# OpenMendel/MendelIHT.jl

Measured on NVIDIA B200. Metric: iht_iterations_per_sec, higher is better.
Workload: dtype f64 (sweep: f32 LUT partials per slab of 640 samples (512 without the ternary copy), f64 across slabs; top-k candidates re-scored in f64)

## Files before the change

### include/ihtb200.h

```cpp
#ifndef IHTB200_H
#define IHTB200_H

#include <stdint.h>

#ifdef __cplusplus
extern "C" {
#endif

#define IHTB_OK          0
#define IHTB_EINVAL     -1
#define IHTB_EDIM       -2
#define IHTB_EDOMAIN    -3
#define IHTB_ENUMERIC   -4
#define IHTB_ECUDA      -5
#define IHTB_ENOMEM     -6
#define IHTB_EUNSUPPORTED -7

enum { IHTB_NORMAL = 0, IHTB_BERNOULLI = 1, IHTB_POISSON = 2, IHTB_NEGBIN = 3 };
enum { IHTB_LINK_IDENTITY = 0, IHTB_LINK_LOGIT = 1, IHTB_LINK_LOG = 2, IHTB_LINK_PROBIT = 3,
       IHTB_LINK_CLOGLOG = 4, IHTB_LINK_CAUCHIT = 5, IHTB_LINK_SQRT = 6, IHTB_LINK_INVERSE = 7,
       IHTB_LINK_INVSQ = 8 };
enum { IHTB_SWEEP_FAST = 0, IHTB_SWEEP_EXACT = 1, IHTB_SWEEP_PAIR = 2 };

typedef struct ihtb_geno ihtb_geno;
typedef struct ihtb_fit ihtb_fit;
typedef struct ihtb_mvfit ihtb_mvfit;
typedef struct ihtb_comm ihtb_comm;

typedef struct ihtb_cfg {
    int32_t dist;
    int32_t link;
    int64_t k;
    double  nb_r;
    double  tol;
    int32_t max_iter;
    int32_t min_iter;
    int32_t max_step;
    int32_t sweep_mode;
    int32_t est_r;
    int32_t debias;
} ihtb_cfg;

typedef struct ihtb_result {
    double  time;
    double  logl;
    int64_t iter;
    double  sigma_g;
    int64_t n_sweeps;
    int64_t n_backtracks;
    double  sweep_seconds;
    int64_t n_launches;
    int64_t n_steps;
} ihtb_result;

typedef struct ihtb_iter_trace {
    double  logl;
    double  tol;
    double  eta;
    int32_t backtracks;
    int32_t n_candidates;
} ihtb_iter_trace;

int32_t ihtb_version(void);
int32_t ihtb_last_error(char* buf, int64_t cap);
int32_t ihtb_device_count(int32_t* count);
int32_t ihtb_set_device(int32_t device);
int32_t ihtb_launch_count(int64_t* count);

int32_t ihtb_geno_create(const uint8_t* bed_cols, int64_t n, int64_t p, int64_t col_stride_bytes,
                         int32_t center, int32_t scale, int32_t impute, ihtb_geno** out);
int32_t ihtb_geno_create_empty(int64_t n, int64_t p, int32_t center, int32_t scale, int32_t impute, ihtb_geno** out);
int32_t ihtb_geno_load_columns(ihtb_geno* g, const uint8_t* bed_cols, int64_t col_stride_bytes, int64_t j_first,
                               int64_t ncols);
int32_t ihtb_geno_finalize(ihtb_geno* g);
int32_t ihtb_geno_create_synthetic(int64_t n, int64_t p_local, int64_t j0, uint64_t seed, double missing_rate,
                                   ihtb_geno** out);
int32_t ihtb_synth_host(int64_t n, int64_t ncols, int64_t j0, uint64_t seed, double missing_rate, uint8_t* out);
int32_t ihtb_geno_dims(const ihtb_geno* g, int64_t* n, int64_t* p);
int32_t ihtb_geno_stats(const ihtb_geno* g, double* mu, double* sigma_inv, int64_t* n_missing);
int32_t ihtb_geno_counts(const ihtb_geno* g, int64_t* counts_4_by_p);
int32_t ihtb_geno_maf(const ihtb_geno* g, double* maf);
int32_t ihtb_geno_decode(const ihtb_geno* g, int64_t i0, int64_t i1, int64_t j0, int64_t j1, double* out_colmajor);
int32_t ihtb_geno_packed(const ihtb_geno* g, int64_t j0, int64_t j1, uint8_t* out);
int32_t ihtb_xt_v(const ihtb_geno* g, const double* V, int64_t m, double* out, int32_t sweep_mode);
int32_t ihtb_x_support(const ihtb_geno* g, const int64_t* idx, int64_t k, const double* coef, int64_t m, double* out);
int32_t ihtb_sweep_bench(const ihtb_geno* g, int32_t sweep_mode, int32_t warmup, int32_t reps, double* ms_kernel,
                         double* ms_total);
int32_t ihtb_geno_sweep_stream_bytes(const ihtb_geno* g, int64_t* bytes, int32_t* ternary);
int32_t ihtb_geno_ternary_tiles(const ihtb_geno* g, uint8_t* out, int64_t out_bytes);
int32_t ihtb_gather_bench(const ihtb_geno* g, int64_t ncols, int32_t reps, double* ms_per_call, double* max_rel_diff);
int32_t ihtb_geno_destroy(ihtb_geno* g);

enum { IHTB_DENSE_F64 = 0, IHTB_DENSE_F32 = 1 };
int32_t ihtb_geno_create_dense(const void* x, int32_t dtype, int64_t n, int64_t p, int64_t ld, int32_t standardize,
                               ihtb_geno** out);
int32_t ihtb_geno_create_dense_empty(int64_t n, int64_t p, int32_t dtype, int32_t standardize, ihtb_geno** out);
int32_t ihtb_geno_load_dense_columns(ihtb_geno* g, const void* x, int64_t ld, int64_t j_first, int64_t ncols);

int32_t ihtb_fit_create(const ihtb_geno* g, const double* y, const double* z, int64_t q, const uint8_t* zkeep,
                        const ihtb_cfg* cfg, ihtb_fit** out);
int32_t ihtb_fit_create_sharded(const ihtb_geno* g, ihtb_comm* comm, int64_t p_global, const double* y,
                                const double* z, int64_t q, const uint8_t* zkeep, const ihtb_cfg* cfg, ihtb_fit** out);
int32_t ihtb_fit_set_weights(ihtb_fit* f, const double* weight);
int32_t ihtb_fit_set_groups(ihtb_fit* f, const int32_t* group, int32_t J, const int64_t* ks, int64_t n_groups);
int32_t ihtb_fit_set_k(ihtb_fit* f, int64_t k);
int32_t ihtb_fit_init(ihtb_fit* f, const uint8_t* train_mask);
int32_t ihtb_fit_init_beta(ihtb_fit* f, const uint8_t* train_mask);
int32_t ihtb_fit_run(ihtb_fit* f, ihtb_result* result, ihtb_iter_trace* trace, int64_t trace_cap);
int32_t ihtb_fit_get(const ihtb_fit* f, double* beta, double* c, double* mu, double* xb);
int32_t ihtb_fit_get_sparse(const ihtb_fit* f, int64_t* idx, double* val, int64_t cap, int64_t* nnz);
int32_t ihtb_fit_predict(ihtb_fit* f, const uint8_t* test_mask, double* deviance);
int32_t ihtb_fit_timer(ihtb_fit* f, int32_t which, double* ms);
int32_t ihtb_fit_phase_times(const ihtb_fit* f, double* out4);
int32_t ihtb_fit_destroy(ihtb_fit* f);

int32_t ihtb_mvfit_create(const ihtb_geno* g, const double* Y, int64_t r, const double* z, int64_t q,
                          const ihtb_cfg* cfg, ihtb_mvfit** out);
int32_t ihtb_mvfit_create_sharded(const ihtb_geno* g, ihtb_comm* comm, int64_t p_global, const double* Y, int64_t r,
                                  const double* z, int64_t q, const ihtb_cfg* cfg, ihtb_mvfit** out);
int32_t ihtb_mvfit_set_k(ihtb_mvfit* f, int64_t k);
int32_t ihtb_mvfit_init(ihtb_mvfit* f, const uint8_t* train_mask);
int32_t ihtb_mvfit_init_beta(ihtb_mvfit* f, const uint8_t* train_mask);
int32_t ihtb_mvfit_run(ihtb_mvfit* f, ihtb_result* result, ihtb_iter_trace* trace, int64_t trace_cap);
int32_t ihtb_mvfit_get(const ihtb_mvfit* f, double* beta, double* c, double* Sigma, double* sigma_g);
int32_t ihtb_mvfit_predict(ihtb_mvfit* f, const uint8_t* test_mask, double* mse);
int32_t ihtb_mvfit_destroy(ihtb_mvfit* f);

int32_t ihtb_cv_run(const ihtb_geno* g, const double* y, const double* z, int64_t q, const uint8_t* zkeep,
                    const ihtb_cfg* cfg, const int32_t* folds, int32_t nfolds, const int64_t* path, int64_t npath,
                    const double* weight, double* mses, int64_t* iters);

enum { IHTB_MULTI_SHARD = 0, IHTB_MULTI_REPLICATE = 1 };
typedef struct ihtb_mgeno ihtb_mgeno;
typedef struct ihtb_mfit ihtb_mfit;
int32_t ihtb_mgeno_create(const uint8_t* bed_cols, int64_t n, int64_t p, int64_t col_stride_bytes, int32_t center,
                          int32_t scale, int32_t impute, int32_t ngpu, const int32_t* devices, int32_t mode,
                          ihtb_mgeno** out);
int32_t ihtb_mgeno_create_synthetic(int64_t n, int64_t p, uint64_t seed, double missing_rate, int32_t ngpu,
                                    const int32_t* devices, int32_t mode, ihtb_mgeno** out);
int32_t ihtb_mgeno_info(const ihtb_mgeno* g, int32_t* ngpu, int32_t* mode, int64_t* n, int64_t* p);
int32_t ihtb_mgeno_part(const ihtb_mgeno* g, int32_t i, ihtb_geno** part, int32_t* device, int64_t* j0);
int32_t ihtb_mgeno_destroy(ihtb_mgeno* g);
int32_t ihtb_mfit_create(const ihtb_mgeno* g, const double* y, const double* z, int64_t q, const uint8_t* zkeep,
                         const ihtb_cfg* cfg, ihtb_mfit** out);
int32_t ihtb_mfit_set_weights(ihtb_mfit* f, const double* weight);
int32_t ihtb_mfit_set_groups(ihtb_mfit* f, const int32_t* group, int32_t J, const int64_t* ks, int64_t n_groups);
int32_t ihtb_mfit_set_k(ihtb_mfit* f, int64_t k);
int32_t ihtb_mfit_init(ihtb_mfit* f, const uint8_t* train_mask, int32_t init_beta);
int32_t ihtb_mfit_run(ihtb_mfit* f, ihtb_result* result, ihtb_iter_trace* trace, int64_t trace_cap);
int32_t ihtb_mfit_get(const ihtb_mfit* f, double* beta, double* c, double* mu, double* xb);
int32_t ihtb_mfit_get_sparse(const ihtb_mfit* f, int64_t* idx, double* val, int64_t cap, int64_t* nnz);
int32_t ihtb_mfit_predict(ihtb_mfit* f, const uint8_t* test_mask, double* deviance);
int32_t ihtb_mfit_timer(ihtb_mfit* f, int32_t which, double* ms);
int32_t ihtb_mfit_destroy(ihtb_mfit* f);
typedef struct ihtb_mmvfit ihtb_mmvfit;
int32_t ihtb_mmvfit_create(const ihtb_mgeno* g, const double* Y, int64_t r, const double* z, int64_t q,
                           const ihtb_cfg* cfg, ihtb_mmvfit** out);
int32_t ihtb_mmvfit_set_k(ihtb_mmvfit* f, int64_t k);
int32_t ihtb_mmvfit_init(ihtb_mmvfit* f, const uint8_t* train_mask, int32_t init_beta);
int32_t ihtb_mmvfit_run(ihtb_mmvfit* f, ihtb_result* result, ihtb_iter_trace* trace, int64_t trace_cap);
int32_t ihtb_mmvfit_get(const ihtb_mmvfit* f, double* beta, double* c, double* Sigma, double* sigma_g);
int32_t ihtb_mmvfit_predict(ihtb_mmvfit* f, const uint8_t* test_mask, double* mse);
int32_t ihtb_mmvfit_destroy(ihtb_mmvfit* f);
int32_t ihtb_mcv_run(const ihtb_mgeno* g, const double* y, const double* z, int64_t q, const uint8_t* zkeep,
                     const ihtb_cfg* cfg, const int32_t* folds, int32_t nfolds, const int64_t* path, int64_t npath,
                     const double* weight, double* mses, int64_t* iters, double* busy_seconds);

int32_t ihtb_comm_unique_id(const char* nccl_lib_path, uint8_t* out128);
int32_t ihtb_comm_create(const char* nccl_lib_path, const uint8_t* id128, int32_t rank, int32_t nranks, ihtb_comm** out);
int32_t ihtb_comm_destroy(ihtb_comm* c);
int32_t ihtb_comm_stats(const ihtb_comm* c, int64_t* peer_memory_collectives, int64_t* nccl_calls);
int32_t ihtb_comm_allreduce_bench(ihtb_comm* c, int64_t n, int32_t reps, int32_t use_p2p, double* us_per_op);
int32_t ihtb_geno_set_offset(ihtb_geno* g, int64_t j0);

#ifdef __cplusplus
}
#endif
#endif
```

### mendeliht.jl_b200/__init__.py

```python
from . import _lib, synth
from ._lib import (SWEEP_EXACT, SWEEP_FAST, SWEEP_PAIR, CudaError, DimensionMismatch, IHTBError, NumericError, device_count,
                   launch_count, load)
from .api import (BERNOULLI, NEGBIN, NORMAL, POISSON, B200DenseLinAlg, B200MultiSnpLinAlg, B200SnpLinAlg, IHTResult, IHTVariable, mIHTResult, mIHTVariable,
                  is_multivariate, allocate_fold_and_k,
                  canonicallink, cross_validate, cv_iht, cv_run, fit_iht, iht, maf_weights, meanloss, parse_covariates)

__all__ = ["B200SnpLinAlg", "B200DenseLinAlg", "B200MultiSnpLinAlg", "IHTResult", "IHTVariable", "fit_iht", "cv_iht", "cv_run", "allocate_fold_and_k", "meanloss",
           "canonicallink", "maf_weights", "iht", "cross_validate", "parse_covariates", "NORMAL", "BERNOULLI", "POISSON", "NEGBIN", "SWEEP_FAST", "SWEEP_EXACT", "SWEEP_PAIR", "load",
           "device_count", "launch_count", "IHTBError", "DimensionMismatch", "NumericError", "CudaError", "synth"]
```

### mendeliht.jl_b200/_lib.py

```python
from __future__ import annotations

import ctypes as C
import os

import numpy as np

HERE = os.path.dirname(os.path.abspath(__file__))
LIB_PATH = os.path.join(HERE, "libihtb200.so")

IHTB_OK, IHTB_EINVAL, IHTB_EDIM, IHTB_EDOMAIN, IHTB_ENUMERIC, IHTB_ECUDA, IHTB_ENOMEM, IHTB_EUNSUPPORTED = (
    0, -1, -2, -3, -4, -5, -6, -7)
SWEEP_FAST, SWEEP_EXACT, SWEEP_PAIR = 0, 1, 2
DENSE_F64, DENSE_F32 = 0, 1


class IHTBError(RuntimeError):
    def __init__(self, code, msg):
        super().__init__(msg)
        self.code = code


class DimensionMismatch(IHTBError, ValueError):
    pass


class NumericError(IHTBError, FloatingPointError):
    pass


class CudaError(IHTBError):
    pass


_EXC = {IHTB_EINVAL: IHTBError, IHTB_EDIM: DimensionMismatch, IHTB_EDOMAIN: IHTBError, IHTB_ENUMERIC: NumericError,
        IHTB_ECUDA: CudaError, IHTB_ENOMEM: IHTBError, IHTB_EUNSUPPORTED: IHTBError}


class Cfg(C.Structure):
    _fields_ = [("dist", C.c_int32), ("link", C.c_int32), ("k", C.c_int64), ("nb_r", C.c_double),
                ("tol", C.c_double), ("max_iter", C.c_int32), ("min_iter", C.c_int32), ("max_step", C.c_int32),
                ("sweep_mode", C.c_int32), ("est_r", C.c_int32), ("debias", C.c_int32)]


class Result(C.Structure):
    _fields_ = [("time", C.c_double), ("logl", C.c_double), ("iter", C.c_int64), ("sigma_g", C.c_double),
                ("n_sweeps", C.c_int64), ("n_backtracks", C.c_int64), ("sweep_seconds", C.c_double),
                ("n_launches", C.c_int64), ("n_steps", C.c_int64)]


class IterTrace(C.Structure):
    _fields_ = [("logl", C.c_double), ("tol", C.c_double), ("eta", C.c_double), ("backtracks", C.c_int32),
                ("n_candidates", C.c_int32)]


_p = C.c_void_p
_pp = C.POINTER(C.c_void_p)
_f64 = C.POINTER(C.c_double)
_i64 = C.POINTER(C.c_int64)
_u8 = C.POINTER(C.c_uint8)

SIGNATURES = {
    "ihtb_version": [],
    "ihtb_last_error": [C.c_char_p, C.c_int64],
    "ihtb_device_count": [C.POINTER(C.c_int32)],
    "ihtb_set_device": [C.c_int32],
    "ihtb_launch_count": [_i64],
    "ihtb_geno_create": [_u8, C.c_int64, C.c_int64, C.c_int64, C.c_int32, C.c_int32, C.c_int32, _pp],
    "ihtb_geno_create_empty": [C.c_int64, C.c_int64, C.c_int32, C.c_int32, C.c_int32, _pp],
    "ihtb_geno_load_columns": [_p, _u8, C.c_int64, C.c_int64, C.c_int64],
    "ihtb_geno_finalize": [_p],
    "ihtb_geno_counts": [_p, _i64],
    "ihtb_geno_maf": [_p, _f64],
    "ihtb_geno_create_synthetic": [C.c_int64, C.c_int64, C.c_int64, C.c_uint64, C.c_double, _pp],
    "ihtb_synth_host": [C.c_int64, C.c_int64, C.c_int64, C.c_uint64, C.c_double, _u8],
    "ihtb_geno_dims": [_p, _i64, _i64],
    "ihtb_geno_stats": [_p, _f64, _f64, _i64],
    "ihtb_geno_decode": [_p, C.c_int64, C.c_int64, C.c_int64, C.c_int64, _f64],
    "ihtb_geno_packed": [_p, C.c_int64, C.c_int64, _u8],
    "ihtb_xt_v": [_p, _f64, C.c_int64, _f64, C.c_int32],
    "ihtb_x_support": [_p, _i64, C.c_int64, _f64, C.c_int64, _f64],
    "ihtb_sweep_bench": [_p, C.c_int32, C.c_int32, C.c_int32, _f64, _f64],
    "ihtb_geno_sweep_stream_bytes": [_p, C.POINTER(C.c_int64), C.POINTER(C.c_int32)],
    "ihtb_gather_bench": [_p, C.c_int64, C.c_int32, _f64, _f64],
    "ihtb_geno_ternary_tiles": [_p, _u8, C.c_int64],
    "ihtb_geno_destroy": [_p],
    "ihtb_geno_create_dense": [_p, C.c_int32, C.c_int64, C.c_int64, C.c_int64, C.c_int32, _pp],
    "ihtb_geno_create_dense_empty": [C.c_int64, C.c_int64, C.c_int32, C.c_int32, _pp],
    "ihtb_geno_load_dense_columns": [_p, _p, C.c_int64, C.c_int64, C.c_int64],
    "ihtb_fit_create": [_p, _f64, _f64, C.c_int64, _u8, C.POINTER(Cfg), _pp],
    "ihtb_fit_create_sharded": [_p, _p, C.c_int64, _f64, _f64, C.c_int64, _u8, C.POINTER(Cfg), _pp],
    "ihtb_fit_set_weights": [_p, _f64],
    "ihtb_fit_set_groups": [_p, C.POINTER(C.c_int32), C.c_int32, _i64, C.c_int64],
    "ihtb_fit_set_k": [_p, C.c_int64],
    "ihtb_fit_init": [_p, _u8],
    "ihtb_fit_init_beta": [_p, _u8],
    "ihtb_fit_run": [_p, C.POINTER(Result), C.POINTER(IterTrace), C.c_int64],
    "ihtb_fit_get": [_p, _f64, _f64, _f64, _f64],
    "ihtb_fit_get_sparse": [_p, C.POINTER(C.c_int64), _f64, C.c_int64, C.POINTER(C.c_int64)],
    "ihtb_fit_predict": [_p, _u8, _f64],
    "ihtb_fit_timer": [_p, C.c_int32, _f64],
    "ihtb_fit_phase_times": [_p, _f64],
    "ihtb_fit_destroy": [_p],
    "ihtb_cv_run": [_p, _f64, _f64, C.c_int64, _u8, C.POINTER(Cfg), C.POINTER(C.c_int32), C.c_int32, _i64, C.c_int64,
                    _f64, _f64, _i64],
    "ihtb_mvfit_create": [_p, _f64, C.c_int64, _f64, C.c_int64, C.POINTER(Cfg), _pp],
    "ihtb_mvfit_create_sharded": [_p, _p, C.c_int64, _f64, C.c_int64, _f64, C.c_int64, C.POINTER(Cfg), _pp],
    "ihtb_mvfit_set_k": [_p, C.c_int64],
    "ihtb_mvfit_init": [_p, _u8],
    "ihtb_mvfit_init_beta": [_p, _u8],
    "ihtb_mvfit_run": [_p, C.POINTER(Result), C.POINTER(IterTrace), C.c_int64],
    "ihtb_mvfit_get": [_p, _f64, _f64, _f64, _f64],
    "ihtb_mvfit_predict": [_p, _u8, _f64],
    "ihtb_mvfit_destroy": [_p],
    "ihtb_comm_unique_id": [C.c_char_p, _u8],
    "ihtb_comm_create": [C.c_char_p, _u8, C.c_int32, C.c_int32, _pp],
    "ihtb_comm_destroy": [_p],
    "ihtb_comm_stats": [_p, _i64, _i64],
    "ihtb_comm_allreduce_bench": [_p, C.c_int64, C.c_int32, C.c_int32, _f64],
    "ihtb_geno_set_offset": [_p, C.c_int64],
    "ihtb_mgeno_create": [_u8, C.c_int64, C.c_int64, C.c_int64, C.c_int32, C.c_int32, C.c_int32, C.c_int32,
                          C.POINTER(C.c_int32), C.c_int32, _pp],
    "ihtb_mgeno_create_synthetic": [C.c_int64, C.c_int64, C.c_uint64, C.c_double, C.c_int32, C.POINTER(C.c_int32),
                                    C.c_int32, _pp],
    "ihtb_mgeno_info": [_p, C.POINTER(C.c_int32), C.POINTER(C.c_int32), _i64, _i64],
    "ihtb_mgeno_part": [_p, C.c_int32, _pp, C.POINTER(C.c_int32), _i64],
    "ihtb_mgeno_destroy": [_p],
    "ihtb_mfit_create": [_p, _f64, _f64, C.c_int64, _u8, C.POINTER(Cfg), _pp],
    "ihtb_mfit_set_weights": [_p, _f64],
    "ihtb_mfit_set_groups": [_p, C.POINTER(C.c_int32), C.c_int32, _i64, C.c_int64],
    "ihtb_mfit_set_k": [_p, C.c_int64],
    "ihtb_mfit_init": [_p, _u8, C.c_int32],
    "ihtb_mfit_run": [_p, C.POINTER(Result), C.POINTER(IterTrace), C.c_int64],
    "ihtb_mfit_get": [_p, _f64, _f64, _f64, _f64],
    "ihtb_mfit_get_sparse": [_p, C.POINTER(C.c_int64), _f64, C.c_int64, C.POINTER(C.c_int64)],
    "ihtb_mfit_predict": [_p, _u8, _f64],
    "ihtb_mfit_timer": [_p, C.c_int32, _f64],
    "ihtb_mfit_destroy": [_p],
    "ihtb_mmvfit_create": [_p, _f64, C.c_int64, _f64, C.c_int64, C.POINTER(Cfg), _pp],
    "ihtb_mmvfit_set_k": [_p, C.c_int64],
    "ihtb_mmvfit_init": [_p, _u8, C.c_int32],
    "ihtb_mmvfit_run": [_p, C.POINTER(Result), C.POINTER(IterTrace), C.c_int64],
    "ihtb_mmvfit_get": [_p, _f64, _f64, _f64, _f64],
    "ihtb_mmvfit_predict": [_p, _u8, _f64],
    "ihtb_mmvfit_destroy": [_p],
    "ihtb_mcv_run": [_p, _f64, _f64, C.c_int64, _u8, C.POINTER(Cfg), C.POINTER(C.c_int32), C.c_int32, _i64, C.c_int64,
                     _f64, _f64, _i64, _f64],
}

_lib = None


def load() -> C.CDLL:
    global _lib
    if _lib is None:
        if not os.path.exists(LIB_PATH):
            raise ImportError(
                f"{LIB_PATH} is missing: the CUDA extension has not been built. "
                "Run `python -c 'import __graft_entry__ as g; g.build()'` (needs nvcc). "
                "mendeliht.jl_b200 has no CPU fallback.")
        lib = C.CDLL(LIB_PATH)
        for name, args in SIGNATURES.items():
            fn = getattr(lib, name)
            fn.argtypes = args
            fn.restype = C.c_int32
        _lib = lib
    return _lib


def last_error() -> str:
    buf = C.create_string_buffer(1024)
    load().ihtb_last_error(buf, 1024)
    return buf.value.decode("utf-8", "replace")


def check(status: int) -> None:
    if status != IHTB_OK:
        raise _EXC.get(status, IHTBError)(status, last_error())


def f64(a) -> np.ndarray:
    return np.ascontiguousarray(a, dtype=np.float64)


def ptr(a: np.ndarray, ctype):
    return a.ctypes.data_as(C.POINTER(ctype)) if a is not None else None


def device_count() -> int:
    n = C.c_int32(0)
    load().ihtb_device_count(C.byref(n))
    return int(n.value)


def launch_count() -> int:
    n = C.c_int64(0)
    check(load().ihtb_launch_count(C.byref(n)))
    return int(n.value)
```

### mendeliht.jl_b200/csrc/common.cuh

```cuda
#pragma once
#include <cuda_runtime.h>
#include <stdint.h>
#include <stdio.h>
#include <string>
#include <vector>
#include <stdexcept>
#include "../../include/ihtb200.h"

namespace ihtb {

struct Error : std::runtime_error {
    int code;
    Error(int c, const std::string& m) : std::runtime_error(m), code(c) {}
};
void set_last_error(const std::string& m);
const std::string& last_error();
struct LaunchCounter {
    int64_t v = 0;
    LaunchCounter& operator++(int) { __atomic_fetch_add(&v, 1, __ATOMIC_RELAXED); return *this; }
    operator int64_t() const { return __atomic_load_n(&v, __ATOMIC_RELAXED); }
};
LaunchCounter& launch_counter();
bool debug_sync();

#define IHTB_CUDA(call)                                                                      \
    do {                                                                                     \
        cudaError_t e__ = (call);                                                            \
        if (e__ != cudaSuccess)                                                              \
            throw ::ihtb::Error(IHTB_ECUDA, std::string(#call) + ": " + cudaGetErrorString(e__)); \
    } while (0)

#define IHTB_CHECK(cond, code, msg)                                  \
    do {                                                             \
        if (!(cond)) throw ::ihtb::Error((code), (msg));             \
    } while (0)

#define IHTB_LAUNCH(kernel, grid, block, smem, stream, ...)          \
    do {                                                             \
        kernel<<<(grid), (block), (smem), (stream)>>>(__VA_ARGS__);  \
        ::ihtb::launch_counter()++;                                  \
        IHTB_CUDA(cudaGetLastError());                               \
        if (::ihtb::debug_sync()) {                                  \
            cudaError_t e2__ = cudaStreamSynchronize(stream);        \
            if (e2__ != cudaSuccess)                                 \
                throw ::ihtb::Error(IHTB_ECUDA, std::string("kernel " #kernel " failed: ") + cudaGetErrorString(e2__)); \
        }                                                            \
    } while (0)

template <typename F>
static inline int32_t guard(F&& f) {
    try {
        f();
        return IHTB_OK;
    } catch (const Error& e) {
        set_last_error(e.what());
        return e.code;
    } catch (const std::bad_alloc&) {
        set_last_error("out of host memory");
        return IHTB_ENOMEM;
    } catch (const std::exception& e) {
        set_last_error(e.what());
        return IHTB_EINVAL;
    }
}

template <typename T>
struct DBuf {
    T* p = nullptr;
    size_t n = 0;
    DBuf() = default;
    explicit DBuf(size_t count) { alloc(count); }
    DBuf(const DBuf&) = delete;
    DBuf& operator=(const DBuf&) = delete;
    ~DBuf() { release(); }
    void alloc(size_t count) {
        release();
        n = count;
        if (count) {
            cudaError_t e = cudaMalloc((void**)&p, count * sizeof(T));
            if (e != cudaSuccess) {
                p = nullptr; n = 0;
                throw Error(IHTB_ENOMEM, std::string("cudaMalloc of ") + std::to_string(count * sizeof(T)) +
                                             " bytes failed: " + cudaGetErrorString(e));
            }
        }
    }
    void release() {
        if (p) cudaFree(p);
        p = nullptr; n = 0;
    }
    void zero(cudaStream_t s) { if (n) IHTB_CUDA(cudaMemsetAsync(p, 0, n * sizeof(T), s)); }
};

template <typename T>
struct HBuf {
    T* p = nullptr;
    size_t n = 0;
    HBuf() = default;
    HBuf(const HBuf&) = delete;
    HBuf& operator=(const HBuf&) = delete;
    ~HBuf() { if (p) cudaFreeHost(p); }
    void alloc(size_t count) {
        if (p) cudaFreeHost(p);
        p = nullptr; n = count;
        if (count) IHTB_CUDA(cudaMallocHost((void**)&p, count * sizeof(T)));
    }
};

static inline int64_t ceil_div(int64_t a, int64_t b) { return (a + b - 1) / b; }

bool smem_attr_needed(const void* kernel, int device);
template <typename K>
static inline void ensure_dynamic_smem(K kernel, int bytes) {
    int dev = 0;
    IHTB_CUDA(cudaGetDevice(&dev));
    if (!smem_attr_needed(reinterpret_cast<const void*>(kernel), dev)) return;
    IHTB_CUDA(cudaFuncSetAttribute(kernel, cudaFuncAttributeMaxDynamicSharedMemorySize, bytes));
}

struct TopkFuse;
ihtb_geno* dense_new_handle(int64_t n, int64_t p, int dtype, int standardize);
void dense_upload(ihtb_geno* g, const void* x, int64_t ld_host, int64_t j_dst, int64_t ncols);
void dense_finalize(ihtb_geno* g);
int64_t dense_stream_bytes(const ihtb_geno* g);
void dense_decode_block(const ihtb_geno* g, int64_t i0, int64_t i1, int64_t j0, int64_t j1, double* d_out);
void dense_xt_v(const ihtb_geno* g, const double* dV, int64_t m, double* dOut, cudaStream_t s, DBuf<double>* part,
                const TopkFuse* tf);
void dense_sweep_kernel_only(const ihtb_geno* g, const double* dV, DBuf<double>* part, cudaStream_t s);
void dense_x_support(const ihtb_geno* g, const int64_t* d_idx, int64_t k, const double* d_coef, int64_t m,
                     double* d_out, cudaStream_t s);
void dense_xt_gather2(const ihtb_geno* g, const int64_t* d_cols_a, int64_t n_a, const int64_t* d_cols_b, int64_t n_b,
                      const double* d_v, int64_t m, double* d_out, cudaStream_t s);
void dense_init_beta_moments(const ihtb_geno* g, const double* d_w, const double* d_wy, double* d_sx, double* d_sxx,
                             double* d_sxy, cudaStream_t s);
void dense_decode_cols(const ihtb_geno* g, const int64_t* d_cols, int64_t k, double* d_out, cudaStream_t s);
const double* geno_bound_scale(const ihtb_geno* g);
double geno_bound_coef(const ihtb_geno* g, double plink_coef);

}

enum { GENO_PLINK = 0, GENO_DENSE = 1 };

struct ihtb_geno {
    int kind = 0;
    int device = 0;
    int64_t n = 0;
    int64_t p = 0;
    int64_t j0 = 0;
    int64_t nbytes = 0;
    int64_t stride = 0;
    int64_t cs_j = 0, cs_s = 0;
    int quad = 0;
    int64_t p4 = 0;
    int center = 1, scale = 1, impute = 1;
    int sm_count = 148;
    ihtb::DBuf<uint8_t> bed;
    ihtb::DBuf<uint8_t> tern;
    int64_t tern_slabs = 0;
    ihtb::DBuf<double> mu, sinv;
    ihtb::DBuf<double> sgn;
    ihtb::DBuf<int32_t> nmiss;
    ihtb::DBuf<int64_t> miss_ptr;
    ihtb::DBuf<int32_t> miss_idx;
    int64_t total_missing = 0;
    bool ready = false;
    int dtype = 0;
    int standardize = 0;
    int64_t ld = 0;
    ihtb::DBuf<uint8_t> dense;
    ihtb::DBuf<double> dscale;
    double dcoef = 0.0;
};
static inline bool geno_is_dense(const ihtb_geno* g) { return g->kind == GENO_DENSE; }

static inline void geno_require_ready(const ihtb_geno* g) {
    IHTB_CHECK(g && g->ready, IHTB_EINVAL, "genotype handle is not finalized (ihtb_geno_finalize)");
}

struct GenoView {
    const uint8_t* bed;
    int64_t cs_j, cs_s, nbytes, stride, n, p;
    int quad;
    const double* mu;
    const double* sinv;
    const int32_t* nmiss;
    int impute;
};
static inline GenoView geno_view(const ihtb_geno* g) {
    return GenoView{g->bed.p, g->cs_j, g->cs_s, g->nbytes, g->stride, g->n, g->p, g->quad, g->mu.p, g->sinv.p,
                    g->nmiss.p, g->impute};
}
__device__ __forceinline__ const uint8_t* gv_ptr(const GenoView& g, int64_t j, int64_t b) {
    if (g.quad)
        return g.bed + (b >> 7) * g.cs_s + (j >> 2) * 512 + ((b & 127) >> 2) * 16 + (j & 3) * 4 + (b & 3);
    return g.bed + j * g.cs_j + (b >> 7) * g.cs_s + (b & 127);
}

namespace ihtb {

__device__ __forceinline__ double warp_sum(double v) {
#pragma unroll
    for (int o = 16; o > 0; o >>= 1) v += __shfl_xor_sync(0xffffffffu, v, o);
    return v;
}
__device__ __forceinline__ float warp_sum(float v) {
#pragma unroll
    for (int o = 16; o > 0; o >>= 1) v += __shfl_xor_sync(0xffffffffu, v, o);
    return v;
}
__device__ __forceinline__ int warp_sum(int v) {
#pragma unroll
    for (int o = 16; o > 0; o >>= 1) v += __shfl_xor_sync(0xffffffffu, v, o);
    return v;
}

__device__ __forceinline__ double block_sum(double v, double* sh) {
    v = warp_sum(v);
    int lane = threadIdx.x & 31, w = threadIdx.x >> 5;
    __syncthreads();
    if (lane == 0) sh[w] = v;
    __syncthreads();
    int nw = (blockDim.x + 31) >> 5;
    v = (threadIdx.x < nw) ? sh[threadIdx.x] : 0.0;
    if (w == 0) v = warp_sum(v);
    return v;
}

void sweep_xt_v(const ihtb_geno* g, const double* dV, int64_t m, double* dOut, int mode, cudaStream_t s,
                double* sweep_seconds);
void x_support(const ihtb_geno* g, const int64_t* d_idx_local, int64_t k, const double* d_coef, int64_t m,
               double* d_out, cudaStream_t s);
void xt_gather(const ihtb_geno* g, const int64_t* d_cols_local, int64_t ncols, const double* d_v, int64_t m,
               const double* d_vsum , double* d_out , cudaStream_t s);
void xt_gather2(const ihtb_geno* g, const int64_t* d_cols_a, int64_t n_a, const int64_t* d_cols_b, int64_t n_b,
                const double* d_v, int64_t m, const double* d_vsum, double* d_out, cudaStream_t s, bool blocked = false);

struct TopkFuse;
void dense_xt_v(const ihtb_geno* g, const double* dV, int64_t m, double* dOut, cudaStream_t s, void* scratch_any,
                const TopkFuse* tf);
void dense_x_support(const ihtb_geno* g, const int64_t* d_idx, int64_t k, const double* d_coef, int64_t m,
                     double* d_out, cudaStream_t s);
void dense_xt_gather2(const ihtb_geno* g, const int64_t* d_cols_a, int64_t n_a, const int64_t* d_cols_b, int64_t n_b,
                      const double* d_v, int64_t m, double* d_out, cudaStream_t s);
void dense_init_beta_moments(const ihtb_geno* g, const double* d_w, const double* d_wy, double* d_sx, double* d_sxx,
                             double* d_sxy, cudaStream_t s, void* scratch_any);
void dense_decode_cols(const ihtb_geno* g, const int64_t* d_cols, int64_t k, double* d_out, cudaStream_t s);
const double* geno_bound_scale(const ihtb_geno* g);
double geno_bound_coef(const ihtb_geno* g, double plink_coef);

}
```

### mendeliht.jl_b200/csrc/fit.cu

```cuda
#include "glm.cuh"
#include "topk.cuh"
#include "comm.cuh"
#include "debias.cuh"
#include "groups.cuh"
#include "pairer.cuh"
#include <algorithm>
#include <chrono>
#include <cmath>
#include <memory>
#include <mutex>
#include <string.h>
#include <unordered_map>

namespace ihtb {
void sweep_xt_v_with_means(const ihtb_geno* g, const double* dV, const double* vbar_host, int64_t m, double* dOut,
                           int mode, cudaStream_t s, void* scratch_any, float* sweep_ms, double* d_l2 = nullptr,
                           const TopkFuse* tf = nullptr);
void* sweep_scratch_create();
void sweep_scratch_destroy(void* p);
void sweep_class_sums(const ihtb_geno* g, const double* d_v, double* d_w1, double* d_w2, double* d_wm, cudaStream_t s,
                      void* scratch_any);
}

using namespace ihtb;

static const double kFastBound = 1.0 / 262144.0;
static const double kExactBound = 1e-13;
static const double kPairBound = 3.1 / 2048.0;

struct ihtb_fit {
    const ihtb_geno* g = nullptr;
    int device = 0;
    int64_t n = 0, p = 0, q = 0;
    ihtb_comm* comm = nullptr;
    int64_t j0 = 0, p_global = 0;
    std::vector<int64_t> shard_j0;
    DBuf<int64_t> d_selall, d_pack, d_packall;
    HBuf<int64_t> h_selall, h_packall;
    int capx = 512;
    ihtb_cfg cfg{};
    cudaStream_t s = nullptr;
    std::vector<uint8_t> zkeep;
    int zkeepn = 0;
    int cap = 4096;

    DBuf<unsigned> d_done;
    DBuf<double> d_y, d_z, d_w, d_xb, d_zc, d_mu, d_r, d_xs, d_dfa, d_part, d_scal, d_small, d_coef, d_gout,
        d_vbar;
    DBuf<uint8_t> d_mask;
    DBuf<uint32_t> d_keyL, d_keyU;
    DBuf<int> d_hist;
    DBuf<int64_t> d_sel;
    DBuf<int64_t> d_idx, d_cols;
    HBuf<double> h_scal, h_gout;
    HBuf<int64_t> h_sel;
    void* sweep_scratch = nullptr;
    cudaEvent_t ev0 = nullptr, ev1 = nullptr, tm0 = nullptr, tm1 = nullptr;
    bool sweep_pending = false;
    struct FusedStep {
        std::vector<int64_t> uni_loc;
        size_t maxsupp = 0;
        int M = 0;
        int winner = -1;
    };
    FusedStep* fz = nullptr;
    DBuf<double> d_pick;
    HBuf<double> h_pick;
    SweepPairer* pairer = nullptr;
    int pair_slot = 0;
    double sweep_coef = kFastBound;
    GlmCtx glm{};
    TopkCtx tk{};

    std::vector<int64_t> idx, idx0, best_idx;
    std::vector<double> b, b0, best_b;
    std::vector<double> c, c0, best_c, df2, h_y, h_mu;
    std::vector<uint8_t> idc, idc0;
    std::unordered_map<int64_t, double> df_exact;
    std::vector<double> wt;
    DBuf<double> d_wt;
    double w_at(int64_t j) const { return wt.empty() ? 1.0 : wt[(size_t)j]; }
    void set_weights(const double* w) {
        if (!w) { wt.clear(); tk.wt = nullptr; return; }
        for (int64_t j = 0; j < p_global; ++j)
            IHTB_CHECK(w[j] > 0.0 && std::isfinite(w[j]), IHTB_EDOMAIN, "weights must be positive and finite");
        wt.assign(w, w + p_global);
        if (d_wt.n < (size_t)p) d_wt.alloc((size_t)p);
        IHTB_CUDA(cudaMemcpyAsync(d_wt.p, wt.data() + j0, (size_t)p * sizeof(double), cudaMemcpyHostToDevice, s));
        sync();
        tk.wt = d_wt.p;
    }
    std::vector<int64_t> cand_cache;
    bool df_sparse = false;
    std::vector<int64_t> dfs_idx;
    std::vector<double> dfs_val;
    double rbar = 0.0, bound = 0.0, sum_w = 0.0, sum_wy = 0.0, last_dev = 0.0, denom_next = 0.0;
    bool denom_ready = false;
    bool inited = false;

    int64_t n_sweeps = 0, n_backtracks = 0, n_cand_iter = 0, n_pair_overflow = 0;
    int last_count = 0;
    double sweep_ms_total = 0.0;
    double pve = 0.0;

    ~ihtb_fit() {
        if (sweep_scratch) sweep_scratch_destroy(sweep_scratch);
        if (ev0) cudaEventDestroy(ev0);
        if (ev1) cudaEventDestroy(ev1);
        if (tm0) cudaEventDestroy(tm0);
        if (tm1) cudaEventDestroy(tm1);
        if (s) cudaStreamDestroy(s);
    }

    void sync() { IHTB_CUDA(cudaStreamSynchronize(s)); }
    void readback_scal(int nv) {
        IHTB_CUDA(cudaMemcpyAsync(h_scal.p, d_scal.p, nv * sizeof(double), cudaMemcpyDeviceToHost, s));
        sync();
    }
    template <typename T>
    void upload(T* dst, const T* src, size_t count) {
        if (count) IHTB_CUDA(cudaMemcpyAsync(dst, src, count * sizeof(T), cudaMemcpyHostToDevice, s));
    }

    bool is_local(int64_t j) const { return j >= j0 && j < j0 + p; }
    int nranks() const { return comm ? comm->nranks : 1; }

    void support_matvec(const std::vector<int64_t>& cols, const std::vector<double>& coef, double* d_out) {
        std::vector<int64_t> ii; std::vector<double> vv;
        for (size_t t = 0; t < cols.size(); ++t)
            if (coef[t] != 0.0 && is_local(cols[t])) { ii.push_back(cols[t] - j0); vv.push_back(coef[t]); }
        if (!ii.empty()) {
            upload(d_idx.p, ii.data(), ii.size());
            upload(d_coef.p, vv.data(), vv.size());
        }
        support_matvec_dev(ii.empty() ? nullptr : d_idx.p, (int64_t)ii.size(), d_coef.p, d_out);
    }

    void support_matvec_dev(const int64_t* d_idx_loc, int64_t k_loc, const double* d_coef_loc, double* d_out) {
        support_matvec_dev_m(d_idx_loc, k_loc, d_coef_loc, 1, d_out);
    }
    void support_matvec_dev_m(const int64_t* d_idx_loc, int64_t k_loc, const double* d_coef_loc, int m, double* d_out) {
        const size_t cnt = (size_t)n * (size_t)m;
        if (!comm) {
            if (k_loc > 0) x_support(g, d_idx_loc, k_loc, d_coef_loc, m, d_out, s);
            else IHTB_CUDA(cudaMemsetAsync(d_out, 0, cnt * sizeof(double), s));
            return;
        }
        if (m == 1 && p2p_pushall_ok(comm, cnt)) {
            if (k_loc > 0) x_support_push(g, d_idx_loc, k_loc, d_coef_loc, comm, s);
            else p2p_push(comm, nullptr, cnt, s);
            p2p_reduce(comm, d_out, cnt, s);
            return;
        }
        if (p2p_mapped(comm) && cnt <= comm->red_cap) {
            double* part = p2p_partial_ptr(comm);
            if (k_loc > 0) x_support(g, d_idx_loc, k_loc, d_coef_loc, m, part, s);
            else IHTB_CUDA(cudaMemsetAsync(part, 0, cnt * sizeof(double), s));
            p2p_allreduce_2phase(comm, cnt, d_out, s);
            return;
        }
        if (k_loc > 0) x_support(g, d_idx_loc, k_loc, d_coef_loc, m, d_out, s);
        else IHTB_CUDA(cudaMemsetAsync(d_out, 0, cnt * sizeof(double), s));
        comm_allreduce_sum_f64(comm, d_out, cnt, s);
    }

    void update_xb() { support_matvec(idx, b, d_xb.p); }

    double glm_update(int add_zc) {
        upload(d_small.p, c.data(), (size_t)q);
        glm_mu(glm, d_small.p, add_zc, s);
        readback_scal(3);
        double dev = h_scal.p[0], lp = h_scal.p[1], sw = h_scal.p[2];
        last_dev = dev;
        if (cfg.dist == IHTB_NORMAL) {
            double phi = dev / (double)n;
            double sigma = std::sqrt(phi);
            return -0.5 * (dev / phi) - sw * (0.5 * std::log(2.0 * M_PI) + std::log(sigma));
        }
        return lp;
    }

    static double digamma(double x) {
        double r = 0.0;
        while (x < 6.0) { r -= 1.0 / x; x += 1.0; }
        double f = 1.0 / (x * x);
        return r + std::log(x) - 0.5 / x -
               f * (1.0 / 12 - f * (1.0 / 120 - f * (1.0 / 252 - f * (1.0 / 240 - f * (1.0 / 132)))));
    }
    static double trigamma(double x) {
        double r = 0.0;
        while (x < 6.0) { r += 1.0 / (x * x); x += 1.0; }
        double f = 1.0 / (x * x);
        return r + 1.0 / x + f / 2 + f / x * (1.0 / 6 - f * (1.0 / 30 - f * (1.0 / 42 - f * (1.0 / 30))));
    }
    void fetch_mu() {
        h_mu.resize((size_t)n);
        IHTB_CUDA(cudaMemcpyAsync(h_mu.data(), d_mu.p, n * sizeof(double), cudaMemcpyDeviceToHost, s));
        sync();
    }
    double nb_logl(double r) {
        glm.nb_r = r;
        return glm_update(1);
    }
    void mle_for_r() {
        fetch_mu();
        const std::vector<double>& y = h_y;
        double r = glm.nb_r;
        if (cfg.est_r == 1) {
            double num = 0.0, den = 0.0;
            for (int64_t i = 0; i < n; ++i) {
                for (int64_t j = 0; j <= (int64_t)y[i] - 1; ++j) num += r / (r + (double)j);
                den += std::log(r / (r + h_mu[i]));
            }
            glm.nb_r = -num / den;
            return;
        }
        auto d1 = [&](double rr) {
            double a = 0.0;
            for (int64_t i = 0; i < n; ++i)
                a += -(y[i] + rr) / (h_mu[i] + rr) - std::log(h_mu[i] + rr) + 1.0 + std::log(rr) + digamma(rr + y[i]) -
                     digamma(rr);
            return a;
        };
        auto d2 = [&](double rr) {
            double a = 0.0;
            for (int64_t i = 0; i < n; ++i)
                a += (y[i] + rr) / ((h_mu[i] + rr) * (h_mu[i] + rr)) - 2.0 / (h_mu[i] + rr) + 1.0 / rr +
                     trigamma(rr + y[i]) - trigamma(rr);
            return a;
        };
        double new_r = 1.0, stepsize = 1.0;
        for (int it = 0; it < 100; ++it) {
            double dx = d1(r), dx2 = d2(r);
            double increment = dx2 < 0 ? dx / dx2 : dx;
            new_r = r - stepsize * increment;
            double old_logl = nb_logl(r);
            for (int j = 0; j < 20; ++j) {
                if (new_r <= 0) {
                    stepsize /= 2; new_r = r - stepsize * increment;
                } else {
                    double new_logl = nb_logl(new_r);
                    if (old_logl >= new_logl) { stepsize /= 2; new_r = r - stepsize * increment; }
                    else break;
                }
            }
            if (std::fabs(r - new_r) <= 1e-6) { glm.nb_r = new_r; return; }
            r = new_r;
        }
        glm.nb_r = r;
    }
    double mu_r_logl() {
        double l = glm_update(1);
        if (cfg.est_r != 0) {
            mle_for_r();
            l = glm_update(1);
        }
        return l;
    }

    void exact_df(const std::vector<int64_t>& cols, bool exchange = true) {
        std::vector<int64_t> need;
        for (int64_t j : cols)
            if (!df_exact.count(j) && (exchange || is_local(j))) need.push_back(j);
        if (need.empty()) { if (!exchange) sync(); return; }
        IHTB_CHECK((int64_t)need.size() <= (int64_t)d_cols.n, IHTB_ENUMERIC, "too many columns to re-score");
        std::vector<int64_t> loc(need.size());
        for (size_t t = 0; t < need.size(); ++t) loc[t] = is_local(need[t]) ? need[t] - j0 : -1;
        upload(d_cols.p, loc.data(), loc.size());
        xt_gather2(g, d_cols.p, (int64_t)need.size(), nullptr, 0, d_r.p, 1, d_vbar.p, d_gout.p, s,
                   false);
        if (exchange) comm_allreduce_sum_f64(comm, d_gout.p, need.size(), s);
        IHTB_CUDA(cudaMemcpyAsync(h_gout.p, d_gout.p, need.size() * sizeof(double), cudaMemcpyDeviceToHost, s));
        sync();
        for (size_t t = 0; t < need.size(); ++t) df_exact[need[t]] = h_gout.p[t];
        n_cand_iter += (int64_t)need.size();
    }

    void score_and_sweep() {
        glm_score(glm, s, d_vbar.p);
        IHTB_CUDA(cudaMemcpyAsync(h_scal.p, d_scal.p, (2 + q) * sizeof(double), cudaMemcpyDeviceToHost, s));
        IHTB_CUDA(cudaEventRecord(ev0, s));
        sweep_coef = geno_bound_coef(g, cfg.sweep_mode == IHTB_SWEEP_FAST ? kFastBound : kExactBound);
        const double t_sw = now();
        if (pairer && cfg.sweep_mode == IHTB_SWEEP_FAST) {
            IHTB_CHECK(!grouped() && !comm, IHTB_EUNSUPPORTED, "paired sweeps serve plain single-device fits only");
            if (pairer->sweep(pair_slot, g, d_r.p, d_vbar.p, d_dfa.p, s, sweep_scratch)) {
                sweep_coef = kPairBound;
                IHTB_CUDA(cudaMemcpyAsync(h_scal.p + 3 + q, pairer->d_l2 + pair_slot, sizeof(double), cudaMemcpyDeviceToHost, s));
            }
        } else if (cfg.k > 0 && !(grouped() && !init_plain)) {
            const TopkFuse tf = topk_absdf_fuse_begin(tk, geno_bound_scale(g), d_scal.p, sweep_coef);
            sweep_xt_v_with_means(g, d_r.p, d_vbar.p, 1, d_dfa.p, cfg.sweep_mode, s, sweep_scratch, nullptr, nullptr, &tf);
        } else {
            sweep_xt_v_with_means(g, d_r.p, d_vbar.p, 1, d_dfa.p, cfg.sweep_mode, s, sweep_scratch, nullptr);
        }
        IHTB_CUDA(cudaEventRecord(ev1, s));
        ++n_sweeps;
        const double t_sel = now();
        dbg[0] += t_sel - t_sw;
        select_rescore(false);
        dbg[1] += now() - t_sel;
    }

    void select_rescore(bool rerun) {
        if (grouped() && !init_plain) {
            select_groups(rerun);
            if (!rerun) finish_sweep_scalars(sweep_coef);
            return;
        }
        df_exact.clear(); cand_cache.clear();
        df_sparse = false;
        const double coef = sweep_coef;
        std::vector<std::pair<int64_t, double>> cvals;
        const bool fused = fz != nullptr && !rerun;
        std::vector<int64_t> supp_loc;
        if (fused) supp_loc = fz->uni_loc;
        else
            for (int64_t j : idx)
                if (is_local(j)) supp_loc.push_back(j - j0);
        const int nsupp = (int)supp_loc.size();
        const int64_t* d_supp = fused ? d_idx.p : d_cols.p;
        int glaunch = 0;
        if (cfg.k > 0) {
            const int64_t ksel = cfg.k + (int64_t)(fused ? fz->maxsupp : idx.size());
            const bool paired = coef == kPairBound;
            if (tk.fused_hist) topk_candidates_absdf_finish(tk, ksel, s);
            else
                topk_candidates_absdf(tk, d_dfa.p, paired ? g->sgn.p : geno_bound_scale(g), rerun ? nullptr : d_scal.p, coef, ksel, s,
                                      bound, (paired && !rerun) ? pairer->d_l2 + pair_slot : nullptr);
            const int64_t want = sweep_coef == kPairBound ? std::max<int64_t>(ksel + 1024, last_count + last_count / 4 + 256)
                                                          : ksel + 64;
            glaunch = (int)std::min<int64_t>(comm ? capx / 2 : cap, want);
        }
        if (nsupp && !fused) upload(d_cols.p, supp_loc.data(), supp_loc.size());
        xt_gather2(g, tk.cand, glaunch, d_supp, nsupp, d_r.p, 1, d_vbar.p, d_gout.p, s);
        denom_ready = false;
        if (!rerun) {
            if (fused) {
                glm_winner_coef(d_pick.p, d_coefM.p, nsupp, d_gout.p + glaunch, d_coef.p, d_cM.p, q, d_small.p + q, s);
                support_matvec_dev(d_supp, nsupp, d_coef.p, d_xs.p);
                IHTB_CUDA(cudaMemcpyAsync(h_pick.p, d_pick.p, (size_t)(1 + fz->M) * sizeof(double), cudaMemcpyDeviceToHost, s));
                IHTB_CUDA(cudaMemcpyAsync(h_scalM.p, d_scalM.p, (size_t)(3 * fz->M) * sizeof(double), cudaMemcpyDeviceToHost, s));
            } else {
                support_matvec_dev(d_supp, nsupp, d_gout.p + glaunch, d_xs.p);
                std::vector<double> mask((size_t)q);
                for (int64_t l = 0; l < q; ++l) mask[l] = idc[l] ? 1.0 : 0.0;
                upload(d_small.p + q, mask.data(), (size_t)q);
            }
            glm_stepsize(glm, d_scal.p + 2, d_xs.p, s, d_small.p + q, d_scal.p + 2 + q);
            IHTB_CUDA(cudaMemcpyAsync(h_scal.p + 2 + q, d_scal.p + 2 + q, sizeof(double), cudaMemcpyDeviceToHost, s));
            denom_ready = true;
        }
        if (!comm) {
            IHTB_CUDA(cudaMemcpyAsync(h_sel.p, d_sel.p, (2 + glaunch) * sizeof(int64_t), cudaMemcpyDeviceToHost, s));
            IHTB_CUDA(cudaMemcpyAsync(h_gout.p, d_gout.p, (glaunch + nsupp) * sizeof(double), cudaMemcpyDeviceToHost, s));
            sync();
            const double t_host = now();
            struct Acc { double& a; double t0; ~Acc() { a += now() - t0; } } acc_host{dbg[2], t_host};
            if (fused) adopt_winner();
            const TopkState* st = reinterpret_cast<const TopkState*>(h_sel.p);
            const int count = cfg.k > 0 ? st->count : 0;
            dbg[3] += (double)std::min(count, glaunch);
            if (count > cap && coef == kPairBound && !rerun) {
                ++n_pair_overflow;
                sweep_coef = kFastBound;
                sweep_xt_v_with_means(g, d_r.p, d_vbar.p, 1, d_dfa.p, IHTB_SWEEP_FAST, s, sweep_scratch, nullptr);
                IHTB_CUDA(cudaEventRecord(ev1, s));
                select_rescore(false);
                return;
            }
            IHTB_CHECK(count <= cap, IHTB_ENUMERIC,
                       "degenerate projection: more than " + std::to_string(cap) +
                           " entries lie within the sweep error bound of the k-th largest |gradient|");
            last_count = count;
            cvals.reserve((size_t)count);
            for (int t = 0; t < std::min(count, glaunch); ++t) cvals.push_back({h_sel.p[2 + t], h_gout.p[t]});
            for (int t = 0; t < nsupp; ++t) df_exact[supp_loc[t] + j0] = h_gout.p[glaunch + t];
            if (count > glaunch) {
                IHTB_CUDA(cudaMemcpyAsync(h_sel.p, d_sel.p, (2 + count) * sizeof(int64_t), cudaMemcpyDeviceToHost, s));
                sync();
                std::vector<int64_t> rest(h_sel.p + 2 + glaunch, h_sel.p + 2 + count);
                exact_df(rest);
                for (int64_t j : rest) cvals.push_back({j, df_exact.at(j)});
            }
        } else {
            const int nr = nranks();
            const size_t blk = 2 + 2 * (size_t)capx;
            IHTB_CHECK(nsupp <= capx / 2, IHTB_ENUMERIC, "support too large for the sharded candidate exchange");
            pack_sweep_candidates(d_pack.p, reinterpret_cast<const TopkState*>(d_sel.p), tk.cand, glaunch, d_gout.p,
                                  d_supp, nsupp, d_gout.p + glaunch, j0, capx, s);
            comm_allgather_i64(comm, d_pack.p, d_packall.p, blk, s);
            IHTB_CUDA(cudaMemcpyAsync(h_packall.p, d_packall.p, nr * blk * sizeof(int64_t), cudaMemcpyDeviceToHost, s));
            sync();
            if (fused) adopt_winner();
            for (int r = 0; r < nr; ++r) {
                const int64_t* b_ = h_packall.p + (size_t)r * blk;
                IHTB_CHECK(b_[0] <= glaunch, IHTB_ENUMERIC,
                           "degenerate projection: too many local candidates within the sweep error bound");
                const int half = capx / 2;
                auto take = [&](int t, bool is_cand) {
                    const int64_t j = b_[2 + t];
                    if (j < 0) return;
                    double v;
                    memcpy(&v, &b_[2 + capx + t], sizeof(double));
                    if (is_cand) cvals.push_back({j, v});
                    else df_exact[j] = v;
                };
                for (int t = 0; t < (int)b_[0]; ++t) take(t, true);
                for (int t = 0; t < (int)b_[1]; ++t) take(half + t, false);
            }
        }
        std::sort(cvals.begin(), cvals.end());
        cvals.erase(std::unique(cvals.begin(), cvals.end(), [](const std::pair<int64_t, double>& x, const std::pair<int64_t, double>& y) {
                        return x.first == y.first; }), cvals.end());
        n_cand_iter += (int64_t)cvals.size();
        std::vector<char> keep(cvals.size(), 1);
        if ((int64_t)cvals.size() > cfg.k) {
            std::vector<std::pair<double, size_t>> outside;
            outside.reserve(cvals.size());
            for (size_t t = 0; t < cvals.size(); ++t)
                if (!std::binary_search(idx.begin(), idx.end(), cvals[t].first))
                    outside.push_back({std::fabs(cvals[t].second) * w_at(cvals[t].first), t});
            if ((int64_t)outside.size() > cfg.k) {
                std::nth_element(outside.begin(), outside.begin() + (cfg.k - 1), outside.end(),
                                 [](const std::pair<double, size_t>& x, const std::pair<double, size_t>& y) {
                                     return x.first > y.first;
                                 });
                const double thr = outside[(size_t)cfg.k - 1].first * (1.0 - 1e-12);
                std::fill(keep.begin(), keep.end(), 0);
                for (const auto& e : outside)
                    if (e.first >= thr) keep[e.second] = 1;
            }
        }
        for (size_t t = 0; t < cvals.size(); ++t)
            if (keep[t]) {
                cand_cache.push_back(cvals[t].first);
                df_exact[cvals[t].first] = cvals[t].second;
            }
        if (rerun) return;
        finish_sweep_scalars(coef);
    }

    void finish_sweep_scalars(double coef) {
        float ms = 0.f;
        IHTB_CUDA(cudaEventElapsedTime(&ms, ev0, ev1));
        sweep_ms_total += ms;
        double rsum = h_scal.p[0], rl1 = h_scal.p[1];
        for (int64_t l = 0; l < q; ++l) df2[l] = h_scal.p[2 + l];
        denom_next = h_scal.p[2 + q];
        rbar = rsum / (double)n;
        bound = coef == kPairBound ? coef * h_scal.p[3 + q]
                                   : coef * (rl1 + std::fabs(rsum));
    }

    double df_at(int64_t j) const {
        if (df_sparse) {
            auto it = std::lower_bound(dfs_idx.begin(), dfs_idx.end(), j);
            return (it != dfs_idx.end() && *it == j) ? dfs_val[it - dfs_idx.begin()] : 0.0;
        }
        return df_exact.at(j);
    }

    double stepsize() {
        std::vector<double> coef(idx.size());
        double numer = 0.0;
        for (size_t t = 0; t < idx.size(); ++t) { coef[t] = df_at(idx[t]); numer += coef[t] * coef[t]; }
        if (denom_ready && !df_sparse) {
            denom_ready = false;
            for (int64_t l = 0; l < q; ++l)
                if (idc[l]) numer += df2[l] * df2[l];
            double eta = numer / denom_next;
            if (std::isinf(eta) || std::isnan(eta)) eta = 1e-8;
            return eta;
        }
        denom_ready = false;
        support_matvec(idx, coef, d_xs.p);
        std::vector<double> d2((size_t)q);
        for (int64_t l = 0; l < q; ++l) {
            d2[l] = idc[l] ? df2[l] : 0.0;
            if (idc[l]) numer += df2[l] * df2[l];
        }
        upload(d_small.p + q, d2.data(), (size_t)q);
        glm_stepsize(glm, d_small.p + q, d_xs.p, s);
        readback_scal(1);
        double denom = h_scal.p[0];
        double eta = numer / denom;
        if (std::isinf(eta) || std::isnan(eta)) eta = 1e-8;
        return eta;
    }

    static double b_lookup(const std::vector<int64_t>& ii, const std::vector<double>& vv, int64_t j) {
        auto it = std::lower_bound(ii.begin(), ii.end(), j);
        return (it != ii.end() && *it == j) ? vv[it - ii.begin()] : 0.0;
    }

    void gradstep(double eta) {
        if (grouped()) { gradstep_group(eta); return; }
        std::vector<int64_t> cand;
        cand = df_sparse ? dfs_idx : cand_cache;
        cand.insert(cand.end(), idx0.begin(), idx0.end());
        std::sort(cand.begin(), cand.end());
        cand.erase(std::unique(cand.begin(), cand.end()), cand.end());

        struct Item { double a; int64_t pos; double v; };
        std::vector<Item> items;
        items.reserve(cand.size() + (size_t)q);
        for (int64_t j : cand) {
            double v = b_lookup(idx0, b0, j) + eta * df_at(j);
            if (!wt.empty()) {
                const double w = wt[(size_t)j], a = v * w;
                items.push_back({std::fabs(a), j, a / w});
            } else {
                items.push_back({std::fabs(v), j, v});
            }
        }
        for (int64_t l = 0; l < q; ++l) {
            c[l] = c0[l] + eta * df2[l];
            if (!zkeep[l]) items.push_back({std::fabs(c[l]), p_global + l, c[l]});
        }
        int64_t k = cfg.k;
        std::sort(items.begin(), items.end(), [](const Item& x, const Item& y) {
            return x.a > y.a || (x.a == y.a && x.pos < y.pos);
        });
        idx.clear(); b.clear();
        const double thr = project_threshold(items, k);
        std::vector<std::pair<int64_t, double>> keep;
        for (size_t t = 0; t < items.size(); ++t) {
            const bool kept = items[t].a >= thr;
            if (items[t].pos >= p_global) {
                if (!kept) c[items[t].pos - p_global] = 0.0;
            } else if (kept && items[t].v != 0.0) {
                keep.push_back({items[t].pos, items[t].v});
            }
        }
        for (int64_t l = 0; l < q; ++l) idc[l] = c[l] != 0.0;
        choose_prune(keep);
        std::sort(keep.begin(), keep.end());
        for (auto& kv : keep) { idx.push_back(kv.first); b.push_back(kv.second); }
    }

    template <typename ItemT>
    static double project_threshold(const std::vector<ItemT>& sorted_items, int64_t k) {
        if (k <= 0) return INFINITY;
        return (int64_t)sorted_items.size() >= k ? sorted_items[(size_t)k - 1].a : 0.0;
    }
    void choose_prune(std::vector<std::pair<int64_t, double>>& keep) const {
        int64_t nonzero = (int64_t)keep.size() - zkeepn;
        for (int64_t l = 0; l < q; ++l) nonzero += idc[l] ? 1 : 0;
        const int64_t limit = cfg.k + zkeepn;
        if (nonzero <= limit) return;
        std::vector<std::pair<int64_t, double>> byabs = keep;
        std::sort(byabs.begin(), byabs.end(), [](const std::pair<int64_t, double>& x, const std::pair<int64_t, double>& y) {
            return std::fabs(x.second) < std::fabs(y.second) || (std::fabs(x.second) == std::fabs(y.second) && x.first > y.first);
        });
        const size_t excess = std::min<size_t>((size_t)(nonzero - limit), byabs.size());
        for (size_t t = 0; t < excess; ++t) keep.erase(std::find(keep.begin(), keep.end(), byabs[t]));
    }

    std::unique_ptr<GroupCtx> grpctx;
    bool init_plain = false;
    bool grouped() const { return (bool)grpctx; }
    void set_groups(const int32_t* group1, int J, const int64_t* ks, int64_t n_groups) {
        if (!group1) { grpctx.reset(); return; }
        IHTB_CHECK(J >= 0, IHTB_EINVAL, "Value of J (max number of groups) must be nonnegative!");
        std::unique_ptr<GroupCtx> gc(new GroupCtx());
        std::vector<double> h_sinv((size_t)p);
        IHTB_CUDA(cudaMemcpy(h_sinv.data(), geno_bound_scale(g), (size_t)p * sizeof(double), cudaMemcpyDeviceToHost));
        gc->build(p, j0, p_global, group1, J, ks, n_groups, cfg.k, h_sinv.data());
        grpctx = std::move(gc);
    }

    void select_groups(bool rerun) {
        GroupCtx& gc = *grpctx;
        df_exact.clear(); cand_cache.clear();
        df_sparse = false; denom_ready = false;
        const double coef = sweep_coef;
        group_topk(gc, d_dfa.p, geno_bound_scale(g), rerun ? nullptr : d_scal.p, coef, bound, cfg.k, s);
        const size_t G = (size_t)gc.G, nT = 2 * G + 1;
        const int nr = nranks();
        std::vector<double> TL(G), TU(G);
        bool overflow = false;
        if (comm) {
            if (gc.d_Tall.n < nT * (size_t)nr) { gc.d_Tall.alloc(nT * (size_t)nr); gc.h_Tall.alloc(nT * (size_t)nr); }
            comm_allgather_i64(comm, reinterpret_cast<const int64_t*>(gc.d_gT.p), gc.d_Tall.p, nT, s);
            IHTB_CUDA(cudaMemcpyAsync(gc.h_Tall.p, gc.d_Tall.p, nT * (size_t)nr * sizeof(int64_t), cudaMemcpyDeviceToHost, s));
            sync();
            std::fill(TL.begin(), TL.end(), 0.0); std::fill(TU.begin(), TU.end(), 0.0);
            for (int rk = 0; rk < nr; ++rk) {
                const double* T = reinterpret_cast<const double*>(gc.h_Tall.p) + (size_t)rk * nT;
                for (size_t gi = 0; gi < G; ++gi) { TL[gi] = std::max(TL[gi], T[gi]); TU[gi] += T[G + gi]; }
                overflow = overflow || T[2 * G] != 0.0;
            }
        } else {
            IHTB_CUDA(cudaMemcpyAsync(gc.h_gT.p, gc.d_gT.p, nT * sizeof(double), cudaMemcpyDeviceToHost, s));
            sync();
            for (size_t gi = 0; gi < G; ++gi) { TL[gi] = gc.h_gT.p[gi]; TU[gi] = gc.h_gT.p[G + gi]; }
            overflow = gc.h_gT.p[2 * G] != 0.0;
        }
        IHTB_CHECK(!overflow, IHTB_ENUMERIC,
                   "degenerate group projection: too many entries of one group lie within the sweep error bound of its "
                   "2k-th largest |gradient|");
        std::vector<char> has(G, 0);
        for (int64_t j : idx) has[(size_t)gc.grp[(size_t)j]] = 1;
        std::vector<int32_t> chosen;
        std::vector<double> lows;
        for (size_t gi = 0; gi < G; ++gi) {
            if (has[gi]) chosen.push_back((int32_t)gi);
            else lows.push_back(TL[gi]);
        }
        if (gc.J > 0 && !lows.empty()) {
            const size_t need = std::min<size_t>((size_t)gc.J, lows.size());
            std::nth_element(lows.begin(), lows.begin() + (need - 1), lows.end(), std::greater<double>());
            const double thr = lows[need - 1];
            for (size_t gi = 0; gi < G; ++gi)
                if (!has[gi] && TU[gi] >= thr) chosen.push_back((int32_t)gi);
        }
        IHTB_CHECK(chosen.size() <= 65536, IHTB_ENUMERIC, "degenerate group projection: too many groups tie at the J-th norm");
        std::sort(chosen.begin(), chosen.end());
        const int nc = (int)chosen.size();
        const int64_t nsupp = (int64_t)idx.size();
        const int64_t list_slots = (int64_t)nc * gc.lcap, slots = list_slots + nsupp;
        if (slots == 0) return;
        gc.ensure_chosen(std::max(nc, 1));
        if (gc.d_oidx.n < (size_t)slots) {
            gc.d_oidx.alloc((size_t)slots); gc.d_oval.alloc((size_t)slots);
            gc.h_oidx.alloc((size_t)slots); gc.h_oval.alloc((size_t)slots);
        }
        if (nc) {
            IHTB_CUDA(cudaMemcpyAsync(gc.d_chosen.p, chosen.data(), (size_t)nc * sizeof(int32_t), cudaMemcpyHostToDevice, s));
            group_take(gc, nc, s);
        }
        std::vector<int64_t> supp_loc((size_t)nsupp);
        for (int64_t t = 0; t < nsupp; ++t) supp_loc[(size_t)t] = is_local(idx[(size_t)t]) ? idx[(size_t)t] - j0 : -1;
        upload(gc.d_oidx.p + list_slots, supp_loc.data(), (size_t)nsupp);
        xt_gather(g, gc.d_oidx.p, slots, d_r.p, 1, d_vbar.p, gc.d_oval.p, s);
        auto take = [&](int64_t t, int64_t j, double v) {
            if (j < 0) return;
            df_exact[j] = v;
            if (t < list_slots) cand_cache.push_back(j);
        };
        if (comm) {
            const size_t blk = 2 * (size_t)slots;
            if (gc.d_blk.n < blk) gc.d_blk.alloc(blk);
            if (gc.d_blkall.n < blk * (size_t)nr) { gc.d_blkall.alloc(blk * (size_t)nr); gc.h_blkall.alloc(blk * (size_t)nr); }
            group_pack(gc.d_oidx.p, gc.d_oval.p, slots, j0, gc.d_blk.p, s);
            comm_allgather_i64(comm, gc.d_blk.p, gc.d_blkall.p, blk, s);
            IHTB_CUDA(cudaMemcpyAsync(gc.h_blkall.p, gc.d_blkall.p, blk * (size_t)nr * sizeof(int64_t), cudaMemcpyDeviceToHost, s));
            sync();
            for (int rk = 0; rk < nr; ++rk) {
                const int64_t* b_ = gc.h_blkall.p + (size_t)rk * blk;
                for (int64_t t = 0; t < slots; ++t) {
                    double v;
                    memcpy(&v, &b_[slots + t], sizeof(double));
                    take(t, b_[t], v);
                }
            }
        } else {
            IHTB_CUDA(cudaMemcpyAsync(gc.h_oidx.p, gc.d_oidx.p, (size_t)slots * sizeof(int64_t), cudaMemcpyDeviceToHost, s));
            IHTB_CUDA(cudaMemcpyAsync(gc.h_oval.p, gc.d_oval.p, (size_t)slots * sizeof(double), cudaMemcpyDeviceToHost, s));
            sync();
            for (int64_t t = 0; t < slots; ++t) take(t, gc.h_oidx.p[t], gc.h_oval.p[t]);
        }
        std::sort(cand_cache.begin(), cand_cache.end());
        cand_cache.erase(std::unique(cand_cache.begin(), cand_cache.end()), cand_cache.end());
        n_cand_iter += (int64_t)cand_cache.size();
    }

    struct GItem { double a; int64_t j; double v; int g; };
    std::vector<std::pair<int64_t, double>> project_groups(std::vector<GItem>& items) const {
        const GroupCtx& gc = *grpctx;
        std::sort(items.begin(), items.end(), [](const GItem& x, const GItem& y) { return x.a > y.a || (x.a == y.a && x.j < y.j); });
        std::unordered_map<int, std::pair<int64_t, double>> acc;
        for (const GItem& it : items) {
            auto& e = acc[it.g];
            if (e.first < gc.k_of(it.g, cfg.k)) { e.second += it.v * it.v; ++e.first; }
        }
        std::vector<std::pair<double, int>> order;
        for (const auto& kv : acc) order.push_back({kv.second.second, kv.first});
        std::sort(order.begin(), order.end(), [](const std::pair<double, int>& x, const std::pair<double, int>& y) {
            return x.first > y.first || (x.first == y.first && x.second < y.second);
        });
        std::unordered_map<int, int> rank;
        for (size_t i = 0; i < order.size(); ++i) rank[order[i].second] = (int)i + 1;
        std::unordered_map<int, int64_t> cnt;
        std::vector<std::pair<int64_t, double>> keep;
        for (const GItem& it : items) {
            int64_t& c_ = cnt[it.g];
            if (rank[it.g] > gc.J || c_ >= gc.k_of(it.g, cfg.k)) continue;
            ++c_;
            if (it.v != 0.0) keep.push_back({it.j, it.v});
        }
        std::sort(keep.begin(), keep.end());
        return keep;
    }

    void gradstep_group(double eta) {
        const GroupCtx& gc = *grpctx;
        std::vector<int64_t> cand = df_sparse ? dfs_idx : cand_cache;
        cand.insert(cand.end(), idx0.begin(), idx0.end());
        std::sort(cand.begin(), cand.end());
        cand.erase(std::unique(cand.begin(), cand.end()), cand.end());
        std::vector<GItem> items;
        items.reserve(cand.size());
        for (int64_t j : cand) {
            const double v = b_lookup(idx0, b0, j) + eta * df_at(j);
            items.push_back({std::fabs(v), j, v, gc.grp[(size_t)j]});
        }
        for (int64_t l = 0; l < q; ++l) c[l] = c0[l] + eta * df2[l];
        auto keep = project_groups(items);
        for (int64_t l = 0; l < q; ++l) idc[l] = c[l] != 0.0;
        if (!gc.ks_vector) {
            int64_t nonzero = (int64_t)keep.size() - zkeepn;
            for (int64_t l = 0; l < q; ++l) nonzero += idc[l] ? 1 : 0;
            const int64_t limit = (int64_t)(gc.J == 0 ? 1 : gc.J) * (cfg.k + zkeepn);
            if (nonzero > limit) {
                std::vector<std::pair<int64_t, double>> byabs = keep;
                std::sort(byabs.begin(), byabs.end(), [](const std::pair<int64_t, double>& x, const std::pair<int64_t, double>& y) {
                    return std::fabs(x.second) < std::fabs(y.second) || (std::fabs(x.second) == std::fabs(y.second) && x.first > y.first);
                });
                const size_t excess = std::min<size_t>((size_t)(nonzero - limit), byabs.size());
                for (size_t t = 0; t < excess; ++t)
                    keep.erase(std::find(keep.begin(), keep.end(), byabs[t]));
            }
        }
        idx.clear(); b.clear();
        for (auto& kv : keep) { idx.push_back(kv.first); b.push_back(kv.second); }
    }

    DebiasWs debias_ws;
    void debias() {
        if (idx.empty()) return;
        std::vector<int64_t> loc(idx.size());
        for (size_t t = 0; t < idx.size(); ++t) loc[t] = is_local(idx[t]) ? idx[t] - j0 : -1;
        upload(d_cols.p, loc.data(), loc.size());
        debias_irls(g, d_y.p, cfg.dist, cfg.link, glm.nb_r, d_cols.p, (int)idx.size(), b.data(), debias_ws, s, comm);
        ++n_debias;
    }
    int64_t n_debias = 0;

    double save_prev(double cur, double best) {
        idx0 = idx; b0 = b; c0 = c; idc0 = idc;
        if (cur > best) { best_idx = idx; best_b = b; best_c = c; }
        return std::max(cur, best);
    }

    double check_convergence() const {
        double the_norm = 0.0, b0max = 0.0;
        size_t i = 0, j = 0;
        while (i < idx.size() || j < idx0.size()) {
            double x = 0.0, y = 0.0;
            if (j >= idx0.size() || (i < idx.size() && idx[i] < idx0[j])) x = b[i++];
            else if (i >= idx.size() || idx0[j] < idx[i]) y = b0[j++];
            else { x = b[i++]; y = b0[j++]; }
            the_norm = std::max(the_norm, std::fabs(x - y));
            b0max = std::max(b0max, std::fabs(y));
        }
        for (int64_t l = 0; l < q; ++l) {
            the_norm = std::max(the_norm, std::fabs(c[l] - c0[l]));
            b0max = std::max(b0max, std::fabs(c0[l]));
        }
        return the_norm / (b0max + 1.0);
    }

    void save_best_model() {
        idx.clear(); b.clear();
        for (size_t t = 0; t < best_idx.size(); ++t)
            if (best_b[t] != 0.0) { idx.push_back(best_idx[t]); b.push_back(best_b[t]); }
        c = best_c;
        for (int64_t l = 0; l < q; ++l) idc[l] = c[l] != 0.0;
        update_xb();
        glm_update(0);
    }

    void compute_pve() {
        glm_sum2(glm, d_mu.p, d_y.p, s);
        readback_scal(2);
        double mm = h_scal.p[0] / (double)n, my = h_scal.p[1] / (double)n;
        glm_ssq2(glm, d_mu.p, mm, d_y.p, my, s);
        readback_scal(2);
        pve = h_scal.p[0] / h_scal.p[1];
    }

    void do_init_beta() {
        IHTB_CHECK(cfg.dist == IHTB_NORMAL, IHTB_EINVAL, "Intializing beta values only work for Gaussian phenotypes! Sorry!");
        DBuf<double> cls((size_t)(7 * p));
        double *W1 = cls.p, *W2 = W1 + p, *Wm = W2 + p, *Y1 = Wm + p, *Y2 = Y1 + p, *Ym = Y2 + p, *bd = Ym + p;
        init_beta_products(glm, d_xs.p, s);
        if (geno_is_dense(g)) {
            dense_init_beta_moments(g, d_w.p, d_xs.p, W1, W2, Wm, s);
            n_sweeps += 1;
            init_beta_solve_moments(glm, p, W1, W2, Wm, sum_w, sum_wy, bd, s);
        } else {
            sweep_class_sums(g, d_w.p, W1, W2, Wm, s, sweep_scratch);
            sweep_class_sums(g, d_xs.p, Y1, Y2, Ym, s, sweep_scratch);
            n_sweeps += 2;
            init_beta_solve(glm, p, W1, W2, Wm, Y1, Y2, Ym, sum_w, sum_wy, g->mu.p, g->sinv.p, g->impute, bd, s);
        }
        if (comm) comm_allreduce_sum_f64(comm, d_scal.p, 1, s);
        readback_scal(1);
        double c0sum = h_scal.p[0];
        std::fill(c.begin(), c.end(), 0.0);
        if (q > 1) {
            init_beta_cov_sums(glm, s);
            readback_scal(3 * ((int)q - 1));
            for (int64_t l = 1; l < q; ++l) {
                double sx = h_scal.p[3 * (l - 1)], sxx = h_scal.p[3 * (l - 1) + 1], sxy = h_scal.p[3 * (l - 1) + 2];
                double icpt = sum_wy, slope = sxy;
                double u11 = std::sqrt(sum_w), u12 = sx / u11, dd = sxx - u12 * u12;
                if (sum_w > 0 && dd > 0) {
                    double u22 = std::sqrt(dd), t1 = sum_wy / u11, t2 = (sxy - u12 * t1) / u22;
                    slope = t2 / u22; icpt = (t1 - u12 * slope) / u11;
                }
                c0sum += icpt;
                c[l] = std::min(std::max(slope, -2.0), 2.0);
            }
        }
        c[0] = std::min(std::max(c0sum / (double)(p_global + q - 1), -2.0), 2.0);
        std::vector<int64_t> cand;
        if (cfg.k > 0) {
            topk_candidates(tk, bd, nullptr, g->sinv.p, 1.0, 0.0, cfg.k, s);
            IHTB_CUDA(cudaMemcpyAsync(h_sel.p, d_sel.p, (2 + cap) * sizeof(int64_t), cudaMemcpyDeviceToHost, s));
            sync();
            const TopkState* st = reinterpret_cast<const TopkState*>(h_sel.p);
            IHTB_CHECK(st->count <= cap, IHTB_ENUMERIC, "degenerate projection of the initial beta (too many ties)");
            cand.assign(h_sel.p + 2, h_sel.p + 2 + st->count);
            std::sort(cand.begin(), cand.end());
        }
        std::vector<double> vals(cand.size());
        if (!cand.empty()) {
            upload(d_cols.p, cand.data(), cand.size());
            take_values(bd, d_cols.p, (int64_t)cand.size(), d_gout.p, s);
            IHTB_CUDA(cudaMemcpyAsync(vals.data(), d_gout.p, cand.size() * sizeof(double), cudaMemcpyDeviceToHost, s));
            sync();
        }
        if (comm) {
            const size_t blk = 2 + 2 * (size_t)capx;
            IHTB_CHECK((int64_t)cand.size() <= capx, IHTB_ENUMERIC, "degenerate projection of the initial beta (too many ties)");
            std::vector<int64_t> mine(blk, 0);
            mine[0] = (int64_t)cand.size();
            for (size_t t = 0; t < cand.size(); ++t) {
                mine[2 + t] = cand[t] + j0;
                memcpy(&mine[2 + capx + t], &vals[t], sizeof(double));
            }
            upload(d_pack.p, mine.data(), blk);
            comm_allgather_i64(comm, d_pack.p, d_packall.p, blk, s);
            const int nr = nranks();
            IHTB_CUDA(cudaMemcpyAsync(h_packall.p, d_packall.p, nr * blk * sizeof(int64_t), cudaMemcpyDeviceToHost, s));
            sync();
            cand.clear(); vals.clear();
            for (int rk = 0; rk < nr; ++rk) {
                const int64_t* b_ = h_packall.p + (size_t)rk * blk;
                for (int64_t t = 0; t < b_[0]; ++t) {
                    double v;
                    memcpy(&v, &b_[2 + capx + t], sizeof(double));
                    cand.push_back(b_[2 + t]);
                    vals.push_back(v);
                }
            }
        }
        struct Item { double a; int64_t pos; double v; };
        std::vector<Item> items;
        for (size_t t = 0; t < cand.size(); ++t) {
            const double w = w_at(cand[t]), a = vals[t] * w;
            items.push_back({std::fabs(a), cand[t], wt.empty() ? vals[t] : a / w});
        }
        for (int64_t l = 0; l < q; ++l)
            if (!zkeep[l]) items.push_back({std::fabs(c[l]), p_global + l, c[l]});
        std::sort(items.begin(), items.end(), [](const Item& x, const Item& y) {
            return x.a > y.a || (x.a == y.a && x.pos < y.pos);
        });
        const double thr = project_threshold(items, cfg.k);
        std::vector<std::pair<int64_t, double>> keep;
        for (size_t t = 0; t < items.size(); ++t) {
            const bool kept = items[t].a >= thr;
            if (items[t].pos >= p_global) {
                if (!kept) c[items[t].pos - p_global] = 0.0;
            } else if (kept && items[t].v != 0.0) {
                keep.push_back({items[t].pos, items[t].v});
            }
        }
        std::sort(keep.begin(), keep.end());
        idx.clear(); b.clear();
        for (auto& kv : keep) { idx.push_back(kv.first); b.push_back(kv.second); }
        for (int64_t l = 0; l < q; ++l) idc[l] = c[l] != 0.0;
        select_rescore(true);
    }

    void init(const uint8_t* train_mask, bool init_beta = false) {
        idx.clear(); b.clear(); idx0.clear(); b0.clear(); best_idx.clear(); best_b.clear();
        c.assign((size_t)q, 0.0); c0 = c; best_c = c; df2.assign((size_t)q, 0.0);
        idc.assign(zkeep.begin(), zkeep.end()); idc0 = idc;
        df_exact.clear(); dfs_idx.clear(); dfs_val.clear(); df_sparse = false;
        last_bt = kMaxBatch;
        d_xb.zero(s);
        const uint8_t* dm = nullptr;
        if (train_mask) {
            upload(d_mask.p, train_mask, (size_t)n);
            dm = d_mask.p;
        }
        glm_set_weights(glm, dm, s);
        readback_scal(2);
        sum_w = h_scal.p[0];
        sum_wy = h_scal.p[1];
        double ybar = h_scal.p[1] / sum_w;
        for (int it = 0; it < 20; ++it) {
            double g1 = glm_linkinv(cfg.link, c[0]);
            double g2 = glm_mueta(cfg.link, c[0]);
            double step = (g1 - ybar) / g2;
            step = std::min(std::max(step, -1.0), 1.0);
            c[0] = c[0] - step;
            if (std::fabs(g1 - ybar) < 1e-10) break;
        }
        glm_update(1);
        init_plain = grouped() && !grpctx->ks_vector && !init_beta;
        score_and_sweep();
        init_plain = false;
        if (grouped() && grpctx->ks_vector && !init_beta) {
            std::vector<GItem> items;
            for (int64_t j : cand_cache) { double v = df_exact.at(j); items.push_back({std::fabs(v), j, v, grpctx->grp[(size_t)j]}); }
            auto keep = project_groups(items);
            for (auto& kv : keep) { dfs_idx.push_back(kv.first); dfs_val.push_back(kv.second); }
            df_sparse = true;
            idx.clear(); b.clear();
            for (int64_t l = 0; l < q; ++l) idc[l] = 1;
            inited = true;
            return;
        }
        if (init_beta) {
            do_init_beta();
            inited = true;
            return;
        }
        std::vector<int64_t> cand = cand_cache;
        struct Item { double a; int64_t pos; double v; };
        std::vector<Item> items;
        for (int64_t j : cand) {
            double v = df_exact.at(j);
            const double w = w_at(j), a = v * w;
            items.push_back({std::fabs(a), j, wt.empty() ? v : a / w});
        }
        for (int64_t l = 0; l < q; ++l)
            if (!zkeep[l]) items.push_back({std::fabs(df2[l]), p_global + l, df2[l]});
        std::sort(items.begin(), items.end(), [](const Item& x, const Item& y) {
            return x.a > y.a || (x.a == y.a && x.pos < y.pos);
        });
        const double thr = project_threshold(items, cfg.k);
        std::vector<std::pair<int64_t, double>> keep;
        for (size_t t = 0; t < items.size(); ++t) {
            const bool kept = items[t].a >= thr;
            if (items[t].pos >= p_global) {
                if (!kept) df2[items[t].pos - p_global] = 0.0;
            } else if (kept && items[t].v != 0.0) {
                keep.push_back({items[t].pos, items[t].v});
            }
        }
        std::sort(keep.begin(), keep.end());
        for (auto& kv : keep) { dfs_idx.push_back(kv.first); dfs_val.push_back(kv.second); }
        df_sparse = true;
        for (int64_t l = 0; l < q; ++l) idc[l] = zkeep[l];
        choose_prune(keep);
        std::sort(keep.begin(), keep.end());
        idx.clear();
        for (auto& kv : keep) idx.push_back(kv.first);
        b.assign(idx.size(), 0.0);
        inited = true;
    }

    double phase[4] = {0, 0, 0, 0};
    double dbg[6] = {0, 0, 0, 0, 0, 0};
    static double now() {
        return std::chrono::duration<double>(std::chrono::steady_clock::now().time_since_epoch()).count();
    }
    static constexpr int kMaxBatch = 4;
    static constexpr int64_t kAdaptiveBatchN = 131072;
    int last_bt = kMaxBatch;
    DBuf<double> d_xbM, d_zcM, d_muM, d_partM, d_scalM, d_cM, d_coefM;
    HBuf<double> h_scalM;
    bool batch_ok() const {
        static const bool off = [] { const char* e = getenv("IHTB_NO_BATCH"); return e && *e == '1'; }();
        return !off && cfg.est_r == 0 && cfg.max_step >= 1 && cfg.max_step + 1 <= kMaxBatch;
    }
    struct StepModel { double eta; std::vector<int64_t> idx; std::vector<double> b, c; std::vector<uint8_t> idc; };
    std::vector<StepModel> step_models;
    void ensure_batch_buffers() {
        if (d_xbM.n < (size_t)(kMaxBatch * n)) {
            d_xbM.alloc((size_t)(kMaxBatch * n)); d_zcM.alloc((size_t)(kMaxBatch * n)); d_muM.alloc((size_t)(kMaxBatch * n));
            d_partM.alloc((size_t)kMaxBatch * GLM_MAX_BLOCKS * 3); d_scalM.alloc(kMaxBatch * 3); h_scalM.alloc(kMaxBatch * 3);
            d_cM.alloc((size_t)(kMaxBatch * q)); d_coefM.alloc((size_t)kMaxBatch * (size_t)cap);
            d_pick.alloc(1 + kMaxBatch); h_pick.alloc(1 + kMaxBatch);
        }
    }
    struct StepPlan { int M; int m0; std::vector<int64_t> uni, loc; size_t UL; };
    StepPlan plan_step(double eta0, int m0 = 0, int m1 = -1) {
        const int Mtot = cfg.max_step + 1;
        if (m1 < 0) m1 = Mtot;
        if (m0 == 0) step_models.assign((size_t)Mtot, StepModel{});
        for (int m = m0; m < m1; ++m) {
            double e = eta0;
            for (int i = 0; i < m; ++i) e /= 2;
            if (m) { idx = idx0; b = b0; c = c0; }
            gradstep(e);
            step_models[(size_t)m] = StepModel{e, idx, b, c, idc};
        }
        const int M = m1 - m0;
        StepPlan pl; pl.M = M; pl.m0 = m0;
        for (int m = m0; m < m1; ++m) {
            const StepModel& md = step_models[(size_t)m];
            pl.uni.insert(pl.uni.end(), md.idx.begin(), md.idx.end());
        }
        std::sort(pl.uni.begin(), pl.uni.end());
        pl.uni.erase(std::unique(pl.uni.begin(), pl.uni.end()), pl.uni.end());
        const size_t U = pl.uni.size();
        IHTB_CHECK(U * (size_t)M <= d_coefM.n && U <= d_idx.n, IHTB_ENUMERIC, "support union too large for the batched step");
        std::vector<size_t> keep_pos;
        for (size_t t = 0; t < U; ++t)
            if (is_local(pl.uni[t])) { pl.loc.push_back(pl.uni[t] - j0); keep_pos.push_back(t); }
        pl.UL = pl.loc.size();
        std::vector<double> coefL(pl.UL * (size_t)M, 0.0), cM((size_t)(M * q));
        for (int m = 0; m < M; ++m) {
            const StepModel& md = step_models[(size_t)(m0 + m)];
            size_t u = 0;
            for (size_t t = 0; t < md.idx.size(); ++t) {
                if (!is_local(md.idx[t])) continue;
                const int64_t lj = md.idx[t] - j0;
                while (pl.loc[u] != lj) ++u;
                coefL[u + (size_t)m * pl.UL] = md.b[t];
            }
            for (int64_t l = 0; l < q; ++l) cM[(size_t)(m * q + l)] = md.c[(size_t)l];
        }
        if (pl.UL) {
            upload(d_idx.p, pl.loc.data(), pl.UL);
            upload(d_coefM.p, coefL.data(), coefL.size());
        }
        upload(d_cM.p, cM.data(), cM.size());
        return pl;
    }
    void adopt_model(int m) {
        const StepModel& win = step_models[(size_t)m];
        idx = win.idx; b = win.b; c = win.c; idc = win.idc;
    }
    double logl_from_sums(const double* s3) const {
        if (cfg.dist == IHTB_NORMAL) {
            const double dev = s3[0], sw = s3[2], phi = dev / (double)n, sigma = std::sqrt(phi);
            return -0.5 * (dev / phi) - sw * (0.5 * std::log(2.0 * M_PI) + std::log(sigma));
        }
        return s3[1];
    }

    void one_step_batched(double old_logl, double& eta, int& eta_step, double& new_logl) {
        ensure_batch_buffers();
        double t0 = now();
        const double eta0 = stepsize();
        double t1 = now(); phase[0] += t1 - t0;
        const int Mtot = cfg.max_step + 1;
        int first = Mtot;
        if (n >= kAdaptiveBatchN) first = std::min(Mtot, last_bt + 1 + (last_bt > 0 ? 1 : 0));
        const StepPlan pl = plan_step(eta0, 0, first);
        double t2 = now(); phase[1] += t2 - t1;
        finish_batched(pl, eta0, t2, old_logl, eta, eta_step, new_logl);
    }
    void finish_batched(const StepPlan& pl, double eta0, double t2, double old_logl, double& eta, int& eta_step,
                        double& new_logl) {
        const int Mtot = cfg.max_step + 1;
        auto eval = [&](const StepPlan& P) {
            const size_t off = (size_t)P.m0 * (size_t)n;
            support_matvec_dev_m(P.UL ? d_idx.p : nullptr, (int64_t)P.UL, d_coefM.p, P.M, d_xbM.p + off);
            glm_mu_batched(glm, d_cM.p, P.M, d_xbM.p + off, d_zcM.p + off, d_muM.p + off, d_partM.p, d_scalM.p + 3 * P.m0, s);
            IHTB_CUDA(cudaMemcpyAsync(h_scalM.p + 3 * P.m0, d_scalM.p + 3 * P.m0, (size_t)(3 * P.M) * sizeof(double),
                                      cudaMemcpyDeviceToHost, s));
            sync();
        };
        int have = pl.M;
        eval(pl);
        int sidx = 0;
        new_logl = logl_from_sums(h_scalM.p);
        while (old_logl > new_logl && sidx < cfg.max_step) {
            ++sidx;
            if (sidx >= have) { eval(plan_step(eta0, have, Mtot)); have = Mtot; }
            new_logl = logl_from_sums(h_scalM.p + 3 * sidx);
            ++n_backtracks;
        }
        last_bt = sidx;
        adopt_model(sidx);
        eta = step_models[(size_t)sidx].eta; eta_step = sidx;
        last_dev = h_scalM.p[3 * sidx];
        const size_t nb = (size_t)n * sizeof(double);
        IHTB_CUDA(cudaMemcpyAsync(d_xb.p, d_xbM.p + (size_t)sidx * n, nb, cudaMemcpyDeviceToDevice, s));
        IHTB_CUDA(cudaMemcpyAsync(d_zc.p, d_zcM.p + (size_t)sidx * n, nb, cudaMemcpyDeviceToDevice, s));
        IHTB_CUDA(cudaMemcpyAsync(d_mu.p, d_muM.p + (size_t)sidx * n, nb, cudaMemcpyDeviceToDevice, s));
        double t3 = now(); phase[2] += t3 - t2;
        score_and_sweep();
        phase[3] += now() - t3;
        IHTB_CHECK(!std::isnan(new_logl), IHTB_ENUMERIC, "Loglikelihood function is NaN, aborting...");
        IHTB_CHECK(!std::isinf(new_logl), IHTB_ENUMERIC, "Loglikelihood function is Inf, aborting...");
    }

    bool fuse_ok() const {
        const char* e = getenv("IHTB_FUSE");
        return e && *e == '1' && !grouped() && denom_ready && !df_sparse;
    }
    void adopt_winner() {
        fz->winner = (int)h_pick.p[0];
        adopt_model(fz->winner);
    }
    void one_step_fused(double old_logl, double& eta, int& eta_step, double& new_logl) {
        ensure_batch_buffers();
        double t0 = now();
        const double eta0 = stepsize();
        double t1 = now(); phase[0] += t1 - t0;
        const StepPlan pl = plan_step(eta0);
        const int M = pl.M;
        double t2 = now(); phase[1] += t2 - t1;
        if (comm && pl.UL > (size_t)capx / 2) {
            finish_batched(pl, eta0, t2, old_logl, eta, eta_step, new_logl);
            return;
        }
        support_matvec_dev_m(pl.UL ? d_idx.p : nullptr, (int64_t)pl.UL, d_coefM.p, M, d_xbM.p);
        glm_mu_batched(glm, d_cM.p, M, d_xbM.p, d_zcM.p, d_muM.p, d_partM.p, d_scalM.p, s);
        glm_pick_model(glm, d_scalM.p, M, old_logl, cfg.max_step, d_pick.p, d_xbM.p, d_zcM.p, d_muM.p, s);
        FusedStep ctx;
        ctx.uni_loc = pl.loc; ctx.M = M;
        for (const StepModel& md : step_models) ctx.maxsupp = std::max(ctx.maxsupp, md.idx.size());
        double t3 = now(); phase[2] += t3 - t2;
        fz = &ctx;
        try {
            score_and_sweep();
        } catch (...) {
            fz = nullptr;
            throw;
        }
        fz = nullptr;
        phase[3] += now() - t3;
        const int w = ctx.winner;
        n_backtracks += w;
        eta = step_models[(size_t)w].eta; eta_step = w;
        new_logl = h_pick.p[1 + w];
        last_dev = h_scalM.p[3 * w];
        IHTB_CHECK(!std::isnan(new_logl), IHTB_ENUMERIC, "Loglikelihood function is NaN, aborting...");
        IHTB_CHECK(!std::isinf(new_logl), IHTB_ENUMERIC, "Loglikelihood function is Inf, aborting...");
    }

    void one_step(double old_logl, double& eta, int& eta_step, double& new_logl) {
        if (batch_ok()) {
            if (fuse_ok()) one_step_fused(old_logl, eta, eta_step, new_logl);
            else one_step_batched(old_logl, eta, eta_step, new_logl);
            return;
        }
        double t0 = now();
        eta = stepsize();
        double t1 = now(); phase[0] += t1 - t0;
        gradstep(eta);
        double t2 = now(); phase[1] += t2 - t1;
        update_xb();
        new_logl = mu_r_logl();
        double t3 = now(); phase[2] += t3 - t2;
        eta_step = 0;
        while (old_logl > new_logl && eta_step < cfg.max_step) {
            eta /= 2;
            idx = idx0; b = b0; c = c0;
            double u0 = now();
            gradstep(eta);
            double u1 = now(); phase[1] += u1 - u0;
            update_xb();
            new_logl = mu_r_logl();
            phase[2] += now() - u1;
            ++eta_step;
            ++n_backtracks;
        }
        double t4 = now();
        score_and_sweep();
        phase[3] += now() - t4;
        IHTB_CHECK(!std::isnan(new_logl), IHTB_ENUMERIC, "Loglikelihood function is NaN, aborting...");
        IHTB_CHECK(!std::isinf(new_logl), IHTB_ENUMERIC, "Loglikelihood function is Inf, aborting...");
    }

    void run(ihtb_result* res, ihtb_iter_trace* trace, int64_t trace_cap) {
        IHTB_CHECK(inited, IHTB_EINVAL, "ihtb_fit_init must be called before ihtb_fit_run");
        auto t0 = std::chrono::steady_clock::now();
        int64_t launches0 = launch_counter();
        int64_t mm_iter = 0, n_steps = 0;
        double next_logl = -INFINITY, best_logl = -INFINITY;
        n_backtracks = 0;
        int64_t sweeps0 = n_sweeps;
        double sweep_ms0 = sweep_ms_total;
        for (int64_t iter = 1; iter <= cfg.max_iter; ++iter) {
            if (iter >= cfg.max_iter) {
                best_logl = save_prev(next_logl, best_logl);
                save_best_model();
                mm_iter = iter;
                break;
            }
            best_logl = save_prev(next_logl, best_logl);
            double eta; int eta_step;
            n_cand_iter = 0;
            one_step(next_logl, eta, eta_step, next_logl);
            ++n_steps;
            if (cfg.debias && iter >= 5 && idx == idx0) debias();
            double scaled_norm = check_convergence();
            if (trace && iter - 1 < trace_cap)
                trace[iter - 1] = ihtb_iter_trace{next_logl, scaled_norm, eta, eta_step, (int32_t)n_cand_iter};
            if (iter >= cfg.min_iter && scaled_norm < cfg.tol) {
                best_logl = save_prev(next_logl, best_logl);
                save_best_model();
                mm_iter = iter;
                break;
            }
        }
        compute_pve();
        IHTB_CHECK(!p2p_failed(comm), IHTB_ECUDA, "peer-memory all-reduce timed out waiting for another rank");
        inited = false;
        if (res) {
            res->time = std::chrono::duration<double>(std::chrono::steady_clock::now() - t0).count();
            res->logl = best_logl;
            res->iter = mm_iter;
            res->sigma_g = pve;
            res->n_sweeps = n_sweeps - sweeps0 + 1;
            res->n_backtracks = n_backtracks;
            res->sweep_seconds = (sweep_ms_total - sweep_ms0) * 1e-3;
            res->n_launches = launch_counter() - launches0;
            res->n_steps = n_steps;
        }
    }
};

extern "C" {

static std::mutex g_cache_mu;
static std::vector<ihtb_fit*> g_cache;
static const size_t kCacheMax = 16;

static ihtb_fit* cache_take(int device, int64_t n, int64_t p, int64_t q, int cap) {
    std::lock_guard<std::mutex> lk(g_cache_mu);
    for (size_t i = 0; i < g_cache.size(); ++i) {
        ihtb_fit* f = g_cache[i];
        if (f->device == device && f->n == n && f->p == p && f->q == q && f->cap == cap) {
            g_cache.erase(g_cache.begin() + i);
            return f;
        }
    }
    return nullptr;
}

void ihtb_internal_fit_cache_clear(int device) {
    std::vector<ihtb_fit*> drop;
    {
        std::lock_guard<std::mutex> lk(g_cache_mu);
        for (size_t i = 0; i < g_cache.size();) {
            if (device < 0 || g_cache[i]->device == device) { drop.push_back(g_cache[i]); g_cache.erase(g_cache.begin() + i); }
            else ++i;
        }
    }
    for (ihtb_fit* f : drop) { cudaSetDevice(f->device); delete f; }
}

static thread_local int t_min_cap = 0;
void ihtb_internal_next_fit_min_cap(int cap) { t_min_cap = cap; }

static ihtb_fit* fit_allocate(const ihtb_geno* g, int64_t q, int cap) {
    std::unique_ptr<ihtb_fit> f(new ihtb_fit());
    int64_t n = g->n, p = g->p;
    f->device = g->device; f->n = n; f->p = p; f->q = q; f->cap = cap;
    IHTB_CUDA(cudaStreamCreateWithFlags(&f->s, cudaStreamNonBlocking));
    IHTB_CUDA(cudaEventCreate(&f->ev0));
    IHTB_CUDA(cudaEventCreate(&f->ev1));
    f->d_y.alloc(n); f->d_z.alloc(n * q); f->d_w.alloc(n); f->d_xb.alloc(n); f->d_zc.alloc(n); f->d_mu.alloc(n);
    f->d_r.alloc(n); f->d_xs.alloc(n + 2 * (size_t)cap + 64); f->d_dfa.alloc(p); f->d_mask.alloc(n);
    f->d_part.alloc((size_t)GLM_MAX_BLOCKS * (2 + q)); f->d_scal.alloc(2 + q + 8); f->d_small.alloc(2 * q);
    size_t cols_cap = 2 * (size_t)cap + 64;
    f->d_coef.alloc(cols_cap); f->d_gout.alloc(cols_cap); f->d_vbar.alloc(1);
    f->d_idx.alloc(cols_cap); f->d_cols.alloc(cols_cap);
    f->d_keyL.alloc(p); f->d_keyU.alloc(p); f->d_hist.alloc(2 * 3 * 2048); f->d_sel.alloc(2 + cap);
    f->h_scal.alloc(2 + q + 8); f->h_gout.alloc(cols_cap); f->h_sel.alloc(2 + cap);
    f->sweep_scratch = sweep_scratch_create();
    f->d_hist.zero(f->s);
    return f.release();
}

int32_t ihtb_fit_create_sharded(const ihtb_geno* g, ihtb_comm* comm, int64_t p_global, const double* y,
                                const double* z, int64_t q, const uint8_t* zkeep, const ihtb_cfg* cfg, ihtb_fit** out);

int32_t ihtb_fit_create(const ihtb_geno* g, const double* y, const double* z, int64_t q, const uint8_t* zkeep,
                        const ihtb_cfg* cfg, ihtb_fit** out) {
    return ihtb_fit_create_sharded(g, nullptr, g ? g->p : 0, y, z, q, zkeep, cfg, out);
}

int32_t ihtb_fit_create_sharded(const ihtb_geno* g, ihtb_comm* comm, int64_t p_global, const double* y,
                                const double* z, int64_t q, const uint8_t* zkeep, const ihtb_cfg* cfg, ihtb_fit** out) {
    return guard([&] {
        IHTB_CHECK(g && y && z && cfg && out, IHTB_EINVAL, "NULL argument");
        IHTB_CHECK(p_global >= g->p, IHTB_EDIM, "p_global is smaller than the local shard");
        geno_require_ready(g);
        IHTB_CHECK(!(geno_is_dense(g) && comm && comm->nranks > 1), IHTB_EUNSUPPORTED,
                   "SNP-sharded fits need PLINK handles: a dense matrix is fitted on one device");
        IHTB_CHECK(q >= 1, IHTB_EDIM, "z must have at least the intercept column");
        IHTB_CHECK(cfg->k >= 0, IHTB_EINVAL, "Value of k (max predictors per group) must be nonnegative!");
        IHTB_CHECK(cfg->max_iter >= 0, IHTB_EINVAL, "Value of max_iter must be nonnegative!");
        IHTB_CHECK(cfg->max_step >= 0, IHTB_EINVAL, "Value of max_step must be nonnegative!");
        IHTB_CHECK(cfg->tol > 2.220446049250313e-16, IHTB_EINVAL, "Value of global tol must exceed machine precision!");
        IHTB_CHECK(cfg->dist >= IHTB_NORMAL && cfg->dist <= IHTB_NEGBIN, IHTB_EINVAL, "unknown distribution");
        IHTB_CHECK(cfg->link >= IHTB_LINK_IDENTITY && cfg->link <= IHTB_LINK_INVSQ, IHTB_EINVAL, "unknown link");
        IHTB_CHECK(cfg->sweep_mode == IHTB_SWEEP_FAST || cfg->sweep_mode == IHTB_SWEEP_EXACT, IHTB_EINVAL,
                   "bad sweep_mode");
        IHTB_CHECK(cfg->k <= p_global, IHTB_EINVAL, "k cannot exceed the number of SNPs");
        IHTB_CUDA(cudaSetDevice(g->device));
        int cap = (int)std::max<int64_t>(4096, 4 * cfg->k + 1024);
        if (t_min_cap > cap) cap = t_min_cap;
        t_min_cap = 0;
        std::unique_ptr<ihtb_fit> f(cache_take(g->device, g->n, g->p, q, cap));
        if (!f) f.reset(fit_allocate(g, q, cap));
        int64_t n = g->n, p = g->p;
        f->g = g; f->cfg = *cfg;
        f->comm = (comm && comm->nranks > 1) ? comm : nullptr;
        f->j0 = f->comm ? g->j0 : 0;
        f->p_global = f->comm ? p_global : g->p;
        f->shard_j0.clear();
        if (f->comm) {
            const int nr = comm->nranks;
            p2p_setup(comm, (size_t)ihtb_fit::kMaxBatch * (size_t)n,
                      (size_t)(2 + 2 * std::max<int64_t>(1024, 2 * (2 * cfg->k + 64 + 64))), f->s);
            if (f->d_selall.n < (size_t)nr * (2 + cap)) {
                f->d_selall.alloc((size_t)nr * (2 + cap));
                f->h_selall.alloc((size_t)nr * (2 + cap));
            }
            f->capx = (int)std::max<int64_t>(1024, 2 * (2 * cfg->k + 64 + 64));
            const size_t blk = 2 + 2 * (size_t)f->capx;
            if (f->d_packall.n < (size_t)nr * blk) {
                f->d_pack.alloc(blk);
                f->d_packall.alloc((size_t)nr * blk);
                f->h_packall.alloc((size_t)nr * blk);
            }
            int64_t mine = g->j0;
            IHTB_CUDA(cudaMemcpyAsync(f->d_sel.p, &mine, sizeof(int64_t), cudaMemcpyHostToDevice, f->s));
            comm_allgather_i64(comm, f->d_sel.p, f->d_selall.p, 1, f->s);
            f->shard_j0.resize(nr);
            IHTB_CUDA(cudaMemcpyAsync(f->shard_j0.data(), f->d_selall.p, nr * sizeof(int64_t), cudaMemcpyDeviceToHost,
                                      f->s));
            IHTB_CUDA(cudaStreamSynchronize(f->s));

        }
        f->zkeep.assign((size_t)q, 1);
        if (zkeep) for (int64_t l = 0; l < q; ++l) f->zkeep[l] = zkeep[l] ? 1 : 0;
        f->zkeepn = 0;
        for (auto v : f->zkeep) f->zkeepn += v;
        f->d_hist.zero(f->s);
        f->inited = false; f->sweep_pending = false; f->denom_ready = false;
        f->n_sweeps = 0; f->n_backtracks = 0; f->sweep_ms_total = 0.0;
        for (int i = 0; i < 4; ++i) f->phase[i] = 0.0;
        IHTB_CHECK(cfg->est_r == 0 || cfg->dist == IHTB_NEGBIN, IHTB_EINVAL,
                   "Only negative binomial regression currently supports nuisance parameter estimation");
        IHTB_CHECK(cfg->est_r >= 0 && cfg->est_r <= 2, IHTB_EINVAL, "Only support method is Newton or MM");
        if (cfg->est_r != 0) f->h_y.assign(y, y + n); else f->h_y.clear();
        IHTB_CUDA(cudaMemcpyAsync(f->d_y.p, y, n * sizeof(double), cudaMemcpyHostToDevice, f->s));
        IHTB_CUDA(cudaMemcpyAsync(f->d_z.p, z, n * q * sizeof(double), cudaMemcpyHostToDevice, f->s));
        f->d_xb.zero(f->s); f->d_zc.zero(f->s);
        f->glm = GlmCtx{n, q, f->d_z.p, f->d_y.p, f->d_w.p, f->d_xb.p, f->d_zc.p, f->d_mu.p, f->d_r.p, f->d_part.p,
                        f->d_scal.p, cfg->dist, cfg->link, cfg->nb_r};
        if (f->d_done.n < 8) { f->d_done.alloc(8); }
        IHTB_CUDA(cudaMemsetAsync(f->d_done.p, 0, 8 * sizeof(unsigned), f->s));
        f->glm.done = f->d_done.p;
        f->tk = TopkCtx{p, f->d_keyL.p, f->d_keyU.p, f->d_hist.p, reinterpret_cast<TopkState*>(f->d_sel.p),
                        f->d_sel.p + 2, f->cap};
        f->wt.clear();
        f->grpctx.reset();
        f->init_plain = false;
        f->sync();
        *out = f.release();
    });
}

int32_t ihtb_fit_set_weights(ihtb_fit* f, const double* weight) {
    return guard([&] {
        IHTB_CHECK(f, IHTB_EINVAL, "NULL fit handle");
        IHTB_CUDA(cudaSetDevice(f->g->device));
        f->set_weights(weight);
    });
}

int32_t ihtb_fit_set_groups(ihtb_fit* f, const int32_t* group, int32_t J, const int64_t* ks, int64_t n_groups) {
    return guard([&] {
        IHTB_CHECK(f, IHTB_EINVAL, "NULL fit handle");
        IHTB_CUDA(cudaSetDevice(f->g->device));
        f->set_groups(group, J, ks, n_groups);
    });
}

int32_t ihtb_fit_set_k(ihtb_fit* f, int64_t k) {
    return guard([&] {
        IHTB_CHECK(f, IHTB_EINVAL, "NULL fit handle");
        IHTB_CHECK(k >= 0 && k <= f->p, IHTB_EINVAL, "Sparsity level cannot be larger than total number of variables");
        IHTB_CHECK(4 * k + 1024 <= f->cap, IHTB_EINVAL,
                   "k exceeds the candidate capacity this fit handle was created with (create it with the largest k)");
        IHTB_CHECK(!f->grouped() || f->grpctx->ks_vector || k <= f->grpctx->kcap, IHTB_EINVAL,
                   "k exceeds the group candidate capacity (create the fit with the largest k of the path)");
        f->cfg.k = k;
    });
}

int32_t ihtb_fit_init(ihtb_fit* f, const uint8_t* train_mask) {
    return guard([&] {
        IHTB_CHECK(f, IHTB_EINVAL, "NULL fit handle");
        IHTB_CUDA(cudaSetDevice(f->g->device));
        f->init(train_mask);
    });
}

int32_t ihtb_fit_init_beta(ihtb_fit* f, const uint8_t* train_mask) {
    return guard([&] {
        IHTB_CHECK(f, IHTB_EINVAL, "NULL fit handle");
        IHTB_CUDA(cudaSetDevice(f->g->device));
        f->init(train_mask, true);
    });
}

int32_t ihtb_fit_run(ihtb_fit* f, ihtb_result* result, ihtb_iter_trace* trace, int64_t trace_cap) {
    return guard([&] {
        IHTB_CHECK(f, IHTB_EINVAL, "NULL fit handle");
        IHTB_CUDA(cudaSetDevice(f->g->device));
        f->run(result, trace, trace_cap);
    });
}

int32_t ihtb_fit_get(const ihtb_fit* f, double* beta, double* c, double* mu, double* xb) {
    return guard([&] {
        IHTB_CHECK(f, IHTB_EINVAL, "NULL fit handle");
        IHTB_CUDA(cudaSetDevice(f->g->device));
        if (beta) {
            std::fill(beta, beta + f->p_global, 0.0);
            for (size_t t = 0; t < f->best_idx.size(); ++t) beta[f->best_idx[t]] = f->best_b[t];
        }
        if (c) std::copy(f->best_c.begin(), f->best_c.end(), c);
        if (mu) IHTB_CUDA(cudaMemcpy(mu, f->d_mu.p, f->n * sizeof(double), cudaMemcpyDeviceToHost));
        if (xb) IHTB_CUDA(cudaMemcpy(xb, f->d_xb.p, f->n * sizeof(double), cudaMemcpyDeviceToHost));
    });
}

int32_t ihtb_fit_get_sparse(const ihtb_fit* f, int64_t* idx, double* val, int64_t cap, int64_t* nnz) {
    return guard([&] {
        IHTB_CHECK(f && nnz, IHTB_EINVAL, "NULL argument");
        *nnz = (int64_t)f->best_idx.size();
        for (size_t t = 0; t < f->best_idx.size() && (int64_t)t < cap; ++t) {
            if (idx) idx[t] = f->best_idx[t];
            if (val) val[t] = f->best_b[t];
        }
    });
}

int32_t ihtb_fit_predict(ihtb_fit* f, const uint8_t* test_mask, double* deviance) {
    return guard([&] {
        IHTB_CHECK(f && deviance, IHTB_EINVAL, "NULL argument");
        IHTB_CUDA(cudaSetDevice(f->g->device));
        const uint8_t* dm = nullptr;
        if (test_mask) {
            f->upload(f->d_mask.p, test_mask, (size_t)f->n);
            dm = f->d_mask.p;
        }
        glm_set_weights(f->glm, dm, f->s);
        f->update_xb();
        f->glm_update(1);
        *deviance = f->last_dev;
    });
}

int32_t ihtb_fit_timer(ihtb_fit* f, int32_t which, double* ms) {
    return guard([&] {
        IHTB_CHECK(f, IHTB_EINVAL, "NULL fit handle");
        IHTB_CUDA(cudaSetDevice(f->g->device));
        if (!f->tm0) { IHTB_CUDA(cudaEventCreate(&f->tm0)); IHTB_CUDA(cudaEventCreate(&f->tm1)); }
        if (which == 0) {
            IHTB_CUDA(cudaStreamSynchronize(f->s));
            IHTB_CUDA(cudaEventRecord(f->tm0, f->s));
        } else {
            IHTB_CUDA(cudaEventRecord(f->tm1, f->s));
            IHTB_CUDA(cudaEventSynchronize(f->tm1));
            float t = 0.f;
            IHTB_CUDA(cudaEventElapsedTime(&t, f->tm0, f->tm1));
            if (ms) *ms = t;
        }
    });
}

int32_t ihtb_fit_phase_times(const ihtb_fit* f, double* out4) {
    return guard([&] {
        IHTB_CHECK(f && out4, IHTB_EINVAL, "NULL argument");
        for (int i = 0; i < 4; ++i) out4[i] = f->phase[i];
    });
}

void ihtb_internal_fit_debug(const ihtb_fit* f, double* out8) {
    for (int i = 0; i < 6; ++i) out8[i] = f->dbg[i];
    out8[6] = f->sweep_ms_total * 1e-3;
    out8[7] = (double)f->n_sweeps;
}

void ihtb_internal_fit_set_pairer(ihtb_fit* f, void* pairer, int slot) {
    f->pairer = reinterpret_cast<ihtb::SweepPairer*>(pairer);
    f->pair_slot = slot;
}

int32_t ihtb_fit_destroy(ihtb_fit* f) {
    return guard([&] {
        if (!f) return;
        cudaSetDevice(f->device);
        cudaStreamSynchronize(f->s);
        f->g = nullptr;
        f->pairer = nullptr;
        {
            std::lock_guard<std::mutex> lk(g_cache_mu);
            if (g_cache.size() < kCacheMax) { g_cache.push_back(f); return; }
        }
        delete f;
    });
}

}
```

### mendeliht.jl_b200/csrc/geno.cu

```cuda
#include "common.cuh"
#include "synth.cuh"
#include <mutex>
#include <thread>
#include <stdlib.h>
#include <string.h>

extern "C" void ihtb_internal_fit_cache_clear(int device);

namespace ihtb {

static thread_local std::string t_last_error;
void set_last_error(const std::string& m) { t_last_error = m; }
const std::string& last_error() { return t_last_error; }
LaunchCounter& launch_counter() {
    static LaunchCounter c;
    return c;
}
bool smem_attr_needed(const void* kernel, int device) {
    static std::mutex mu;
    static std::vector<std::pair<const void*, int>> done;
    std::lock_guard<std::mutex> lk(mu);
    for (const auto& e : done)
        if (e.first == kernel && e.second == device) return false;
    done.push_back({kernel, device});
    return true;
}
bool debug_sync() {
    static int v = -1;
    if (v < 0) { const char* e = getenv("IHTB_DEBUG_SYNC"); v = (e && *e == '1') ? 1 : 0; }
    return v == 1;
}


__global__ void k_mask_tail(GenoView g, int n_rem) {
    int64_t j = blockIdx.x * (int64_t)blockDim.x + threadIdx.x;
    if (j >= g.p) return;
    uint8_t mask = (uint8_t)((1u << (2 * n_rem)) - 1u);
    *const_cast<uint8_t*>(gv_ptr(g, j, g.nbytes - 1)) &= mask;
}

__global__ void k_repack(const uint8_t* __restrict__ staging, int64_t pitch, int64_t j0, int64_t ncols, GenoView g) {
    int64_t vec_per_col = (g.nbytes + 15) >> 4;
    int64_t t = blockIdx.x * (int64_t)blockDim.x + threadIdx.x;
    if (t >= ncols * vec_per_col) return;
    int64_t c = t / vec_per_col, v = t % vec_per_col;
    const uint8_t* src = staging + c * pitch + 16 * v;
    uint8_t tmp[16];
#pragma unroll
    for (int k = 0; k < 16; ++k) tmp[k] = (16 * v + k < g.nbytes) ? src[k] : (uint8_t)0;
    uint32_t q[4];
    memcpy(q, tmp, 16);
#pragma unroll
    for (int k = 0; k < 4; ++k)
        *reinterpret_cast<uint32_t*>(const_cast<uint8_t*>(gv_ptr(g, j0 + c, 16 * v + 4 * k))) = q[k];
}

__global__ void k_export(GenoView g, int64_t j0, int64_t ncols, uint8_t* __restrict__ out) {
    int64_t t = blockIdx.x * (int64_t)blockDim.x + threadIdx.x;
    if (t >= ncols * g.nbytes) return;
    int64_t c = t / g.nbytes, b = t % g.nbytes;
    out[t] = *gv_ptr(g, j0 + c, b);
}

__global__ void k_col_stats(GenoView g, int scale, double* __restrict__ mu, double* __restrict__ sinv,
                            int32_t* __restrict__ nmiss, double* __restrict__ sgn) {
    int64_t j = (blockIdx.x * (int64_t)blockDim.x + threadIdx.x) >> 5;
    int lane = threadIdx.x & 31;
    if (j >= g.p) return;
    const int64_t n = g.n;
    int64_t nvec = g.stride >> 4;
    int c1 = 0, c2 = 0, cm = 0;
    for (int64_t v = lane; v < nvec; v += 32) {
        uint32_t w[4];
#pragma unroll
        for (int t = 0; t < 4; ++t) w[t] = *reinterpret_cast<const uint32_t*>(gv_ptr(g, j, 16 * v + 4 * t));
#pragma unroll
        for (int t = 0; t < 4; ++t) {
            uint32_t lo = w[t] & 0x55555555u, hi = (w[t] >> 1) & 0x55555555u;
            cm += __popc(lo & ~hi);
            c1 += __popc(hi & ~lo);
            c2 += __popc(hi & lo);
        }
    }
    c1 = warp_sum(c1); c2 = warp_sum(c2); cm = warp_sum(cm);
    if (lane == 0) {
        double nobs = (double)(n - cm);
        double m = (double)((int64_t)c1 + 2 * (int64_t)c2) / nobs;
        double s = sqrt(__dmul_rn(m, __dsub_rn(1.0, m / 2.0)));
        mu[j] = m;
        const double si = (scale && s > 0.0) ? 1.0 / s : 1.0;
        sinv[j] = si;
        nmiss[j] = cm;
        const double g2 = sqrt((double)((int64_t)c1 + 4 * (int64_t)c2));
        sgn[j] = si * (g2 > 1.0 ? g2 : 1.0);
    }
}

__global__ void k_col_counts(GenoView g, int64_t* __restrict__ out ) {
    int64_t j = (blockIdx.x * (int64_t)blockDim.x + threadIdx.x) >> 5;
    int lane = threadIdx.x & 31;
    if (j >= g.p) return;
    int64_t nvec = g.stride >> 4;
    int c1 = 0, c2 = 0, cm = 0;
    for (int64_t v = lane; v < nvec; v += 32) {
        uint32_t w[4];
#pragma unroll
        for (int t = 0; t < 4; ++t) w[t] = *reinterpret_cast<const uint32_t*>(gv_ptr(g, j, 16 * v + 4 * t));
#pragma unroll
        for (int t = 0; t < 4; ++t) {
            uint32_t lo = w[t] & 0x55555555u, hi = (w[t] >> 1) & 0x55555555u;
            cm += __popc(lo & ~hi);
            c1 += __popc(hi & ~lo);
            c2 += __popc(hi & lo);
        }
    }
    c1 = warp_sum(c1); c2 = warp_sum(c2); cm = warp_sum(cm);
    if (lane == 0) {
        out[4 * j + 0] = g.n - c1 - c2 - cm;
        out[4 * j + 1] = cm;
        out[4 * j + 2] = c1;
        out[4 * j + 3] = c2;
    }
}

__global__ void k_fill_missing(GenoView g, const int64_t* __restrict__ ptr, int32_t* __restrict__ idx) {
    int64_t j = (blockIdx.x * (int64_t)blockDim.x + threadIdx.x) >> 5;
    int lane = threadIdx.x & 31;
    if (j >= g.p) return;
    int64_t base = ptr[j];
    if (ptr[j + 1] == base) return;
    const int64_t nbytes = g.nbytes;
    int64_t off = 0;
    for (int64_t b0 = 0; b0 < nbytes; b0 += 32) {
        int64_t b = b0 + lane;
        uint32_t byte = (b < nbytes) ? *gv_ptr(g, j, b) : 0u;
        uint32_t lo = byte & 0x55u, hi = (byte >> 1) & 0x55u;
        uint32_t mm = lo & ~hi;
        int cnt = __popc(mm);
        int pre = cnt;
#pragma unroll
        for (int o = 1; o < 32; o <<= 1) {
            int t = __shfl_up_sync(0xffffffffu, pre, o);
            if (lane >= o) pre += t;
        }
        int total = __shfl_sync(0xffffffffu, pre, 31);
        pre -= cnt;
        int w = 0;
#pragma unroll
        for (int t = 0; t < 4; ++t)
            if (mm & (1u << (2 * t))) idx[base + off + pre + (w++)] = (int32_t)(4 * b + t);
        off += total;
    }
}

__global__ void k_decode(GenoView gv, int center, int64_t i0, int64_t i1, int64_t j0, int64_t j1,
                         double* __restrict__ out) {
    int64_t ni = i1 - i0;
    int64_t t = blockIdx.x * (int64_t)blockDim.x + threadIdx.x;
    if (t >= ni * (j1 - j0)) return;
    int64_t j = j0 + t / ni, i = i0 + t % ni;
    uint32_t code = (*gv_ptr(gv, j, i >> 2) >> (2 * (i & 3))) & 3u;
    double m = gv.mu[j];
    double g = (code == 2) ? 1.0 : (code == 3) ? 2.0 : (code == 1) ? (gv.impute ? m : 0.0) : 0.0;
    if (center) g = __dsub_rn(g, m);
    out[t] = __dmul_rn(g, gv.sinv[j]);
}

__global__ void k_synth(GenoView g, int64_t j0, uint64_t seed, uint32_t miss_thr) {
    const int64_t n = g.n;
    int64_t words = g.stride >> 2;
    int64_t t = blockIdx.x * (int64_t)blockDim.x + threadIdx.x;
    if (t >= g.p * words) return;
    int64_t j = t / words, w = t % words;
    uint64_t key = synth_col_key(seed, (uint64_t)(j0 + j));
    uint64_t thr = synth_maf_threshold(key);
    uint32_t out = 0;
#pragma unroll
    for (int s = 0; s < 16; ++s) {
        int64_t i = 16 * w + s;
        if (i < n) out |= synth_code(key, thr, miss_thr, (uint64_t)i) << (2 * s);
    }
    *reinterpret_cast<uint32_t*>(const_cast<uint8_t*>(gv_ptr(g, j, 4 * w))) = out;
}

__global__ void k_make_tern(GenoView g, int64_t p4, int64_t tern_slabs, uint32_t* __restrict__ out) {
    const int64_t idx = blockIdx.x * (int64_t)blockDim.x + threadIdx.x;
    const int64_t total = tern_slabs * p4 * 32;
    if (idx >= total) return;
    const int cj = (int)(idx & 3), w = (int)((idx >> 2) & 31);
    const int64_t sq = idx >> 7, nquads = p4 >> 2;
    const int64_t slab = sq / nquads, j = (sq % nquads) * 4 + (cj ^ (w & 3));
    uint32_t word = 0;
    if (j < g.p) {
        const int64_t b0 = slab * 160 + 5 * w;
        uint32_t code[20];
#pragma unroll
        for (int t = 0; t < 5; ++t) {
            const int64_t b = b0 + t;
            const uint32_t byte = b < g.stride ? *gv_ptr(g, j, b) : 0u;
#pragma unroll
            for (int s = 0; s < 4; ++s) code[4 * t + s] = (byte >> (2 * s)) & 3u;
        }
#pragma unroll
        for (int t = 0; t < 4; ++t) {
            uint32_t v = 0;
#pragma unroll
            for (int d = 4; d >= 0; --d) {
                const uint32_t c = code[5 * t + d];
                v = 3u * v + ((c >> 1) * (1u + (c & 1u)));
            }
            word |= v << (8 * t);
        }
    }
    out[idx] = word;
}

static void build_tern(ihtb_geno* g, cudaStream_t s) {
    g->tern.release();
    g->tern_slabs = 0;
    if (!g->quad) return;
    const char* e = getenv("IHTB_TERN");
    if (e && *e == '0') return;
    const int64_t slabs = ceil_div(g->n, 640);
    const size_t bytes = (size_t)slabs * (size_t)g->p4 * 128;
    if (!(e && *e == '1')) {
        size_t free_b = 0, total_b = 0;
        IHTB_CUDA(cudaMemGetInfo(&free_b, &total_b));
        if (bytes > free_b / 2) return;
    }
    g->tern.alloc(bytes);
    g->tern_slabs = slabs;
    const int64_t words = slabs * g->p4 * 32;
    IHTB_LAUNCH(k_make_tern, (unsigned)ceil_div(words, 256), 256, 0, s, geno_view(g), g->p4, slabs,
                reinterpret_cast<uint32_t*>(g->tern.p));
}

static void finish_handle(ihtb_geno* g) {
    cudaStream_t s = 0;
    g->mu.alloc(g->p); g->sinv.alloc(g->p); g->nmiss.alloc(g->p); g->sgn.alloc(g->p);
    int64_t threads = g->p * 32;
    IHTB_LAUNCH(k_col_stats, (unsigned)ceil_div(threads, 256), 256, 0, s, geno_view(g), g->scale, g->mu.p, g->sinv.p,
                g->nmiss.p, g->sgn.p);
    g->miss_ptr.alloc(g->p + 1);
    int64_t total = 0;
    {
        std::vector<int32_t> hn((size_t)g->p);
        std::vector<int64_t> hp((size_t)g->p + 1);
        IHTB_CUDA(cudaMemcpy(hn.data(), g->nmiss.p, g->p * sizeof(int32_t), cudaMemcpyDeviceToHost));
        for (int64_t j = 0; j < g->p; ++j) { hp[j] = total; total += hn[j]; }
        hp[g->p] = total;
        IHTB_CUDA(cudaMemcpy(g->miss_ptr.p, hp.data(), (g->p + 1) * sizeof(int64_t), cudaMemcpyHostToDevice));
    }
    g->total_missing = total;
    if (total > 0) {
        g->miss_idx.alloc(total);
        IHTB_LAUNCH(k_fill_missing, (unsigned)ceil_div(threads, 256), 256, 0, s, geno_view(g), g->miss_ptr.p,
                    g->miss_idx.p);
    }
    build_tern(g, s);
    IHTB_CUDA(cudaStreamSynchronize(s));
}

static ihtb_geno* new_handle(int64_t n, int64_t p, int center, int scale, int impute) {
    IHTB_CHECK(n > 0 && p > 0, IHTB_EDIM, "genotype matrix must have n > 0 and p > 0");
    IHTB_CHECK(n < (int64_t(1) << 31), IHTB_EDIM, "n must be < 2^31");
    IHTB_CHECK(center == 1, IHTB_EUNSUPPORTED,
               "x is not centered! Please construct SnpLinAlg{Float64}(::SnpArray, center=true, scale=true)");
    int ndev = 0;
    cudaError_t e = cudaGetDeviceCount(&ndev);
    if (e != cudaSuccess || ndev == 0)
        throw Error(IHTB_ECUDA, "no CUDA device available (libihtb200 has no CPU fallback)");
    ihtb_geno* g = new ihtb_geno();
    IHTB_CUDA(cudaGetDevice(&g->device));
    IHTB_CUDA(cudaDeviceGetAttribute(&g->sm_count, cudaDevAttrMultiProcessorCount, g->device));
    g->n = n; g->p = p;
    g->nbytes = (n + 3) / 4;
    g->stride = ceil_div(g->nbytes, 128) * 128;
    const char* lay = getenv("IHTB_LAYOUT");
    g->p4 = (p + 3) / 4 * 4;
    if (lay && std::string(lay) == "colmajor") { g->cs_j = g->stride; g->cs_s = 128; g->p4 = p; }
    else if (lay && std::string(lay) == "tiled") { g->cs_j = 128; g->cs_s = g->p * 128; g->p4 = p; }
    else { g->quad = 1; g->cs_j = 128; g->cs_s = g->p4 * 128; }
    g->center = center; g->scale = scale; g->impute = impute;
    try {
        g->bed.alloc((size_t)(g->p4 * g->stride));
        if (g->p4 != g->p) IHTB_CUDA(cudaMemset(g->bed.p, 0, (size_t)(g->p4 * g->stride)));
    } catch (...) {
        delete g;
        throw;
    }
    return g;
}

}

using namespace ihtb;

extern "C" {

int32_t ihtb_version(void) { return 100; }

int32_t ihtb_last_error(char* buf, int64_t cap) {
    if (!buf || cap <= 0) return IHTB_EINVAL;
    const std::string& m = ihtb::last_error();
    int64_t k = (int64_t)m.size() < cap - 1 ? (int64_t)m.size() : cap - 1;
    memcpy(buf, m.data(), (size_t)k);
    buf[k] = 0;
    return IHTB_OK;
}

int32_t ihtb_device_count(int32_t* count) {
    return guard([&] {
        IHTB_CHECK(count, IHTB_EINVAL, "count is NULL");
        int n = 0;
        cudaError_t e = cudaGetDeviceCount(&n);
        *count = (e == cudaSuccess) ? n : 0;
        if (e != cudaSuccess) cudaGetLastError();
    });
}

int32_t ihtb_set_device(int32_t device) {
    return guard([&] { IHTB_CUDA(cudaSetDevice(device)); });
}

int32_t ihtb_launch_count(int64_t* count) {
    return guard([&] {
        IHTB_CHECK(count, IHTB_EINVAL, "count is NULL");
        *count = launch_counter();
    });
}

static void upload_columns(ihtb_geno* g, const uint8_t* bed_cols, int64_t col_stride_bytes, int64_t j_dst, int64_t ncols) {
    const int64_t pitch = ceil_div(g->nbytes, 16) * 16;
    int64_t cols_per = (int64_t(64) << 20) / pitch;
    if (cols_per < 1) cols_per = 1;
    if (cols_per > ncols) cols_per = ncols;
    const int NB = 2;
    HBuf<uint8_t> hbuf[NB];
    DBuf<uint8_t> dbuf[NB];
    cudaEvent_t done[NB];
    cudaStream_t st;
    IHTB_CUDA(cudaStreamCreateWithFlags(&st, cudaStreamNonBlocking));
    for (int b = 0; b < NB; ++b) {
        hbuf[b].alloc((size_t)(cols_per * pitch));
        dbuf[b].alloc((size_t)(cols_per * pitch));
        IHTB_CUDA(cudaEventCreateWithFlags(&done[b], cudaEventDisableTiming));
    }
    unsigned nt = std::thread::hardware_concurrency();
    if (nt == 0) nt = 1;
    if (nt > 16) nt = 16;
    const GenoView gv = geno_view(g);
    const int64_t vec_per_col = (g->nbytes + 15) >> 4;
    const int64_t nbytes = g->nbytes;
    int b = 0;
    try {
        for (int64_t j = 0; j < ncols; j += cols_per, b ^= 1) {
            const int64_t h = (ncols - j < cols_per) ? ncols - j : cols_per;
            IHTB_CUDA(cudaEventSynchronize(done[b]));
            uint8_t* dst = hbuf[b].p;
            const uint8_t* src = bed_cols + j * col_stride_bytes;
            const unsigned use = (unsigned)std::min<int64_t>(nt, h);
            std::vector<std::thread> pool;
            for (unsigned t = 1; t < use; ++t)
                pool.emplace_back([=] {
                    for (int64_t c = h * t / use; c < h * (t + 1) / use; ++c)
                        memcpy(dst + c * pitch, src + c * col_stride_bytes, (size_t)nbytes);
                });
            for (int64_t c = 0; c < h / use; ++c) memcpy(dst + c * pitch, src + c * col_stride_bytes, (size_t)nbytes);
            for (auto& th : pool) th.join();
            IHTB_CUDA(cudaMemcpyAsync(dbuf[b].p, hbuf[b].p, (size_t)(h * pitch), cudaMemcpyHostToDevice, st));
            IHTB_LAUNCH(k_repack, (unsigned)ceil_div(h * vec_per_col, 256), 256, 0, st, dbuf[b].p, pitch, j_dst + j, h, gv);
            IHTB_CUDA(cudaEventRecord(done[b], st));
        }
        IHTB_CUDA(cudaStreamSynchronize(st));
    } catch (...) {
        cudaStreamSynchronize(st);
        for (int i = 0; i < NB; ++i) cudaEventDestroy(done[i]);
        cudaStreamDestroy(st);
        throw;
    }
    for (int i = 0; i < NB; ++i) cudaEventDestroy(done[i]);
    cudaStreamDestroy(st);
}

static void seal_handle(ihtb_geno* g) {
    if (g->n % 4) IHTB_LAUNCH(k_mask_tail, (unsigned)ceil_div(g->p, 256), 256, 0, 0, geno_view(g), (int)(g->n % 4));
    finish_handle(g);
    g->ready = true;
}

int32_t ihtb_geno_create(const uint8_t* bed_cols, int64_t n, int64_t p, int64_t col_stride_bytes, int32_t center,
                         int32_t scale, int32_t impute, ihtb_geno** out) {
    return guard([&] {
        IHTB_CHECK(bed_cols && out, IHTB_EINVAL, "NULL argument");
        IHTB_CHECK(col_stride_bytes >= (n + 3) / 4, IHTB_EDIM, "col_stride_bytes is smaller than ceil(n/4)");
        ihtb_geno* g = new_handle(n, p, center, scale, impute);
        try {
            IHTB_CUDA(cudaMemset(g->bed.p, 0, (size_t)(g->p4 * g->stride)));
            upload_columns(g, bed_cols, col_stride_bytes, 0, p);
            seal_handle(g);
        } catch (...) {
            delete g;
            throw;
        }
        *out = g;
    });
}

int32_t ihtb_geno_create_empty(int64_t n, int64_t p, int32_t center, int32_t scale, int32_t impute, ihtb_geno** out) {
    return guard([&] {
        IHTB_CHECK(out, IHTB_EINVAL, "NULL argument");
        ihtb_geno* g = new_handle(n, p, center, scale, impute);
        try {
            IHTB_CUDA(cudaMemset(g->bed.p, 0, (size_t)(g->p4 * g->stride)));
        } catch (...) {
            delete g;
            throw;
        }
        g->ready = false;
        *out = g;
    });
}

int32_t ihtb_geno_load_columns(ihtb_geno* g, const uint8_t* bed_cols, int64_t col_stride_bytes, int64_t j_first,
                               int64_t ncols) {
    return guard([&] {
        IHTB_CHECK(g && bed_cols, IHTB_EINVAL, "NULL argument");
        IHTB_CHECK(!geno_is_dense(g), IHTB_EINVAL, "a dense handle takes ihtb_geno_load_dense_columns");
        IHTB_CHECK(!g->ready, IHTB_EINVAL, "genotype handle is already finalized");
        IHTB_CHECK(col_stride_bytes >= g->nbytes, IHTB_EDIM, "col_stride_bytes is smaller than ceil(n/4)");
        IHTB_CHECK(j_first >= 0 && ncols >= 0 && j_first + ncols <= g->p, IHTB_EDIM, "column range outside the matrix");
        IHTB_CUDA(cudaSetDevice(g->device));
        if (ncols > 0) upload_columns(g, bed_cols, col_stride_bytes, j_first, ncols);
    });
}

int32_t ihtb_geno_finalize(ihtb_geno* g) {
    return guard([&] {
        IHTB_CHECK(g, IHTB_EINVAL, "NULL argument");
        IHTB_CHECK(!g->ready, IHTB_EINVAL, "genotype handle is already finalized");
        IHTB_CUDA(cudaSetDevice(g->device));
        if (geno_is_dense(g)) {
            dense_finalize(g);
            g->ready = true;
        } else {
            seal_handle(g);
        }
    });
}

int32_t ihtb_geno_create_synthetic(int64_t n, int64_t p_local, int64_t j0, uint64_t seed, double missing_rate,
                                   ihtb_geno** out) {
    return guard([&] {
        IHTB_CHECK(out, IHTB_EINVAL, "NULL argument");
        IHTB_CHECK(missing_rate >= 0.0 && missing_rate < 1.0, IHTB_EINVAL, "missing_rate must be in [0, 1)");
        ihtb_geno* g = new_handle(n, p_local, 1, 1, 1);
        try {
            g->j0 = j0;
            uint32_t miss_thr = synth_missing_threshold(missing_rate);
            int64_t words = g->stride >> 2;
            int64_t total = g->p * words;
            IHTB_LAUNCH(k_synth, (unsigned)ceil_div(total, 256), 256, 0, 0, geno_view(g), j0, seed, miss_thr);
            finish_handle(g);
            g->ready = true;
        } catch (...) {
            delete g;
            throw;
        }
        *out = g;
    });
}

int32_t ihtb_synth_host(int64_t n, int64_t ncols, int64_t j0, uint64_t seed, double missing_rate, uint8_t* out) {
    return guard([&] {
        IHTB_CHECK(out && n > 0 && ncols >= 0, IHTB_EINVAL, "bad argument");
        const int64_t nbytes = (n + 3) / 4;
        const uint32_t miss_thr = synth_missing_threshold(missing_rate);
        unsigned nt = std::thread::hardware_concurrency();
        if (nt == 0) nt = 1;
        if ((int64_t)nt > ncols) nt = (unsigned)(ncols > 0 ? ncols : 1);
        std::vector<std::thread> pool;
        for (unsigned t = 0; t < nt; ++t) {
            pool.emplace_back([=] {
                for (int64_t c = ncols * t / nt; c < ncols * (t + 1) / nt; ++c) {
                    uint64_t key = synth_col_key(seed, (uint64_t)(j0 + c));
                    uint64_t thr = synth_maf_threshold(key);
                    uint8_t* col = out + c * nbytes;
                    for (int64_t b = 0; b < nbytes; ++b) {
                        uint32_t byte = 0;
                        for (int s = 0; s < 4; ++s) {
                            int64_t i = 4 * b + s;
                            if (i < n) byte |= synth_code(key, thr, miss_thr, (uint64_t)i) << (2 * s);
                        }
                        col[b] = (uint8_t)byte;
                    }
                }
            });
        }
        for (auto& th : pool) th.join();
    });
}

int32_t ihtb_geno_sweep_stream_bytes(const ihtb_geno* g, int64_t* bytes, int32_t* ternary) {
    return guard([&] {
        IHTB_CHECK(g, IHTB_EINVAL, "NULL genotype handle");
        geno_require_ready(g);
        if (geno_is_dense(g)) {
            if (bytes) *bytes = dense_stream_bytes(g);
            if (ternary) *ternary = 0;
            return;
        }
        const bool t = g->tern.p != nullptr;
        if (bytes) *bytes = (t ? g->tern_slabs : g->stride / 128) * g->p4 * 128;
        if (ternary) *ternary = t ? 1 : 0;
    });
}

int32_t ihtb_geno_set_offset(ihtb_geno* g, int64_t j0) {
    return guard([&] {
        IHTB_CHECK(g && j0 >= 0, IHTB_EINVAL, "bad argument");
        IHTB_CHECK(!geno_is_dense(g), IHTB_EUNSUPPORTED, "dense handles cannot be SNP shards");
        g->j0 = j0;
    });
}

int32_t ihtb_geno_dims(const ihtb_geno* g, int64_t* n, int64_t* p) {
    return guard([&] {
        IHTB_CHECK(g, IHTB_EINVAL, "NULL genotype handle");
        if (n) *n = g->n;
        if (p) *p = g->p;
    });
}

int32_t ihtb_geno_stats(const ihtb_geno* g, double* mu, double* sigma_inv, int64_t* n_missing) {
    return guard([&] {
        IHTB_CHECK(g, IHTB_EINVAL, "NULL genotype handle");
        geno_require_ready(g);
        IHTB_CUDA(cudaSetDevice(g->device));
        if (mu) IHTB_CUDA(cudaMemcpy(mu, g->mu.p, g->p * sizeof(double), cudaMemcpyDeviceToHost));
        if (sigma_inv) IHTB_CUDA(cudaMemcpy(sigma_inv, g->sinv.p, g->p * sizeof(double), cudaMemcpyDeviceToHost));
        if (n_missing) {
            std::vector<int32_t> tmp(g->p);
            IHTB_CUDA(cudaMemcpy(tmp.data(), g->nmiss.p, g->p * sizeof(int32_t), cudaMemcpyDeviceToHost));
            for (int64_t j = 0; j < g->p; ++j) n_missing[j] = tmp[j];
        }
    });
}

int32_t ihtb_geno_counts(const ihtb_geno* g, int64_t* counts) {
    return guard([&] {
        IHTB_CHECK(g && counts, IHTB_EINVAL, "NULL argument");
        IHTB_CHECK(!geno_is_dense(g), IHTB_EUNSUPPORTED, "genotype counts need a PLINK handle");
        geno_require_ready(g);
        IHTB_CUDA(cudaSetDevice(g->device));
        DBuf<int64_t> d((size_t)(4 * g->p));
        IHTB_LAUNCH(k_col_counts, (unsigned)ceil_div(g->p * 32, 256), 256, 0, 0, geno_view(g), d.p);
        IHTB_CUDA(cudaMemcpy(counts, d.p, (size_t)(4 * g->p) * sizeof(int64_t), cudaMemcpyDeviceToHost));
    });
}

int32_t ihtb_geno_maf(const ihtb_geno* g, double* maf) {
    return guard([&] {
        IHTB_CHECK(g && maf, IHTB_EINVAL, "NULL argument");
        IHTB_CHECK(!geno_is_dense(g), IHTB_EUNSUPPORTED, "maf needs a PLINK handle (SnpArray)");
        geno_require_ready(g);
        IHTB_CUDA(cudaSetDevice(g->device));
        IHTB_CUDA(cudaMemcpy(maf, g->mu.p, g->p * sizeof(double), cudaMemcpyDeviceToHost));
        for (int64_t j = 0; j < g->p; ++j) {
            double f = maf[j] / 2.0;
            maf[j] = f > 0.5 ? 1.0 - f : f;
        }
    });
}

int32_t ihtb_geno_decode(const ihtb_geno* g, int64_t i0, int64_t i1, int64_t j0, int64_t j1, double* out) {
    return guard([&] {
        IHTB_CHECK(g && out, IHTB_EINVAL, "NULL argument");
        IHTB_CHECK(0 <= i0 && i0 <= i1 && i1 <= g->n && 0 <= j0 && j0 <= j1 && j1 <= g->p, IHTB_EDIM,
                   "decode block out of bounds");
        geno_require_ready(g);
        IHTB_CUDA(cudaSetDevice(g->device));
        int64_t total = (i1 - i0) * (j1 - j0);
        if (total == 0) return;
        DBuf<double> d((size_t)total);
        if (geno_is_dense(g)) dense_decode_block(g, i0, i1, j0, j1, d.p);
        else IHTB_LAUNCH(k_decode, (unsigned)ceil_div(total, 256), 256, 0, 0, geno_view(g), g->center, i0, i1, j0, j1, d.p);
        IHTB_CUDA(cudaMemcpy(out, d.p, total * sizeof(double), cudaMemcpyDeviceToHost));
    });
}

int32_t ihtb_geno_packed(const ihtb_geno* g, int64_t j0, int64_t j1, uint8_t* out) {
    return guard([&] {
        IHTB_CHECK(g && out, IHTB_EINVAL, "NULL argument");
        IHTB_CHECK(!geno_is_dense(g), IHTB_EUNSUPPORTED, "a dense handle has no packed genotypes");
        IHTB_CHECK(0 <= j0 && j0 <= j1 && j1 <= g->p, IHTB_EDIM, "column range out of bounds");
        geno_require_ready(g);
        IHTB_CUDA(cudaSetDevice(g->device));
        if (j1 == j0) return;
        int64_t cols_per = (int64_t(256) << 20) / g->nbytes;
        if (cols_per < 1) cols_per = 1;
        if (cols_per > j1 - j0) cols_per = j1 - j0;
        DBuf<uint8_t> staging((size_t)(cols_per * g->nbytes));
        for (int64_t j = j0; j < j1; j += cols_per) {
            int64_t h = (j1 - j < cols_per) ? j1 - j : cols_per;
            IHTB_LAUNCH(k_export, (unsigned)ceil_div(h * g->nbytes, 256), 256, 0, 0, geno_view(g), j, h, staging.p);
            IHTB_CUDA(cudaMemcpy(out + (j - j0) * g->nbytes, staging.p, (size_t)(h * g->nbytes),
                                 cudaMemcpyDeviceToHost));
        }
    });
}

int32_t ihtb_geno_ternary_tiles(const ihtb_geno* g, uint8_t* out, int64_t out_bytes) {
    return guard([&] {
        IHTB_CHECK(g && out, IHTB_EINVAL, "NULL argument");
        IHTB_CHECK(!geno_is_dense(g), IHTB_EUNSUPPORTED, "a dense handle has no ternary copy");
        geno_require_ready(g);
        IHTB_CHECK(g->tern.p != nullptr, IHTB_EINVAL, "this handle holds no ternary copy");
        const int64_t bytes = g->tern_slabs * g->p4 * 128;
        IHTB_CHECK(out_bytes == bytes, IHTB_EDIM, "the ternary copy has " + std::to_string(bytes) + " bytes");
        IHTB_CUDA(cudaSetDevice(g->device));
        IHTB_CUDA(cudaMemcpy(out, g->tern.p, (size_t)bytes, cudaMemcpyDeviceToHost));
    });
}

int32_t ihtb_geno_destroy(ihtb_geno* g) {
    return guard([&] {
        if (g) {
            cudaSetDevice(g->device);
            ihtb_internal_fit_cache_clear(g->device);
            delete g;
        }
    });
}

}
```

### mendeliht.jl_b200/csrc/support.cu

```cuda
#include "common.cuh"
#include "comm.cuh"
#include <algorithm>
#include <memory>
#include <mutex>
#include <unordered_map>

namespace ihtb {

constexpr int XS_CHUNK = 32;

template <int M, bool PUSH>
__global__ void __launch_bounds__(256)
k_x_support(GenoView gv, const int64_t* __restrict__ idx, int64_t k, const double* __restrict__ coef,
            double* __restrict__ out, P2PView pv, unsigned long long seq) {
    const int64_t nbytes = gv.nbytes, n = gv.n;
    const double* __restrict__ mu = gv.mu;
    const double* __restrict__ sinv = gv.sinv;
    const int impute = gv.impute;
    __shared__ double tab[XS_CHUNK][4][M];
    __shared__ int64_t cols[XS_CHUNK];
    int64_t b = blockIdx.x * (int64_t)blockDim.x + threadIdx.x;
    double acc[4][M];
#pragma unroll
    for (int s = 0; s < 4; ++s)
#pragma unroll
        for (int t = 0; t < M; ++t) acc[s][t] = 0.0;

    for (int64_t c0 = 0; c0 < k; c0 += XS_CHUNK) {
        int nc = (int)((k - c0 < XS_CHUNK) ? (k - c0) : XS_CHUNK);
        __syncthreads();
        for (int e = threadIdx.x; e < nc * 4 * M; e += blockDim.x) {
            int c = e / (4 * M), code = (e / M) & 3, t = e % M;
            int64_t j = idx[c0 + c];
            double m = mu[j];
            double g = (code == 2) ? 1.0 : (code == 3) ? 2.0 : (code == 1) ? (impute ? m : 0.0) : 0.0;
            double x = __dmul_rn(__dsub_rn(g, m), sinv[j]);
            tab[c][code][t] = __dmul_rn(x, coef[(c0 + c) + (int64_t)t * k]);
            if (code == 0 && t == 0) cols[c] = j;
        }
        __syncthreads();
        if (b < nbytes) {
            for (int c = 0; c < nc; ++c) {
                uint32_t byte = *gv_ptr(gv, cols[c], b);
#pragma unroll
                for (int s = 0; s < 4; ++s) {
                    uint32_t code = (byte >> (2 * s)) & 3u;
#pragma unroll
                    for (int t = 0; t < M; ++t) acc[s][t] = __dadd_rn(acc[s][t], tab[c][code][t]);
                }
            }
        }
    }
    if (PUSH) {
        __shared__ double stage[PUSH ? 1024 : 1];
        __syncthreads();
#pragma unroll
        for (int s = 0; s < 4; ++s) stage[4 * threadIdx.x + s] = acc[s][0];
        __syncthreads();
        const int64_t base = 1024 * (int64_t)blockIdx.x;
        for (int e = 2 * threadIdx.x; e < 1024; e += 512) {
            const int64_t i = base + e;
            if (i + 1 < n) {
                const double2 x = make_double2(stage[e], stage[e + 1]);
                for (int r = 0; r < pv.nranks; ++r) *reinterpret_cast<double2*>(pv.push_slot[r] + i) = x;
            } else if (i < n) {
                for (int r = 0; r < pv.nranks; ++r) pv.push_slot[r][i] = stage[e];
            }
        }
        p2p_publish(pv, seq);
        return;
    }
    if (b < nbytes) {
#pragma unroll
        for (int s = 0; s < 4; ++s) {
            int64_t i = 4 * b + s;
            if (i < n)
#pragma unroll
                for (int t = 0; t < M; ++t) out[i + (int64_t)t * n] = acc[s][t];
        }
    }
}

template <int M>
static void launch_x_support(const ihtb_geno* g, const int64_t* d_idx, int64_t k, const double* d_coef, double* d_out,
                             cudaStream_t s) {
    IHTB_LAUNCH((k_x_support<M, false>), (unsigned)ceil_div(g->nbytes, 256), 256, 0, s, geno_view(g), d_idx, k, d_coef,
                d_out, P2PView{}, 0ull);
}

void x_support_push(const ihtb_geno* g, const int64_t* d_idx, int64_t k, const double* d_coef, ihtb_comm* c,
                    cudaStream_t s) {
    IHTB_LAUNCH((k_x_support<1, true>), (unsigned)ceil_div(g->nbytes, 256), 256, 0, s, geno_view(g), d_idx, k, d_coef,
                (double*)nullptr, p2p_view(c), (unsigned long long)(c->seq[0] + 1));
}

void x_support(const ihtb_geno* g, const int64_t* d_idx, int64_t k, const double* d_coef, int64_t m, double* d_out,
               cudaStream_t s) {
    if (geno_is_dense(g)) { dense_x_support(g, d_idx, k, d_coef, m, d_out, s); return; }
    for (int64_t t0 = 0; t0 < m;) {
        int64_t mm = m - t0;
        const double* cf = d_coef + t0 * k;
        double* o = d_out + t0 * g->n;
        if (mm >= 4) { launch_x_support<4>(g, d_idx, k, cf, o, s); t0 += 4; }
        else if (mm == 3) { launch_x_support<3>(g, d_idx, k, cf, o, s); t0 += 3; }
        else if (mm == 2) { launch_x_support<2>(g, d_idx, k, cf, o, s); t0 += 2; }
        else { launch_x_support<1>(g, d_idx, k, cf, o, s); t0 += 1; }
    }
}

constexpr int XG_MAX_SPLIT = 64;


template <int M>
__global__ void __launch_bounds__(256)
k_xt_gather(GenoView gv, const int64_t* __restrict__ cols, int64_t n_a, const int64_t* __restrict__ cols_b,
            int64_t split_bytes, const double* __restrict__ v,
            const double* __restrict__ vbar, double* __restrict__ part ) {
    __shared__ double sh[32];
    const int64_t nbytes = gv.nbytes, n = gv.n;
    const int64_t c = blockIdx.x, sp = blockIdx.y;
    const int64_t j = c < n_a ? cols[c] : cols_b[c - n_a];
    if (j < 0) return;
    const int64_t b0 = sp * split_bytes;
    const int64_t b1 = (b0 + split_bytes < nbytes) ? b0 + split_bytes : nbytes;
    double a[M], mm[M], vb[M];
#pragma unroll
    for (int t = 0; t < M; ++t) { a[t] = 0.0; mm[t] = 0.0; vb[t] = vbar[t]; }
    for (int64_t b = b0 + threadIdx.x; b < b1; b += blockDim.x) {
        uint32_t byte = *gv_ptr(gv, j, b);
        if (byte == 0) continue;
#pragma unroll
        for (int s = 0; s < 4; ++s) {
            uint32_t code = (byte >> (2 * s)) & 3u;
            int64_t i = 4 * b + s;
            if (code != 0 && i < n) {
#pragma unroll
                for (int t = 0; t < M; ++t) {
                    double u = __dsub_rn(v[i + (int64_t)t * n], vb[t]);
                    if (code == 1) mm[t] = __dadd_rn(mm[t], u);
                    else a[t] = __dadd_rn(a[t], (code == 3) ? __dadd_rn(u, u) : u);
                }
            }
        }
    }
    double* o = part + (c * gridDim.y + sp) * (2 * M);
#pragma unroll
    for (int t = 0; t < M; ++t) {
        double at = block_sum(a[t], sh);
        double mt = block_sum(mm[t], sh);
        if (threadIdx.x == 0) { o[2 * t] = at; o[2 * t + 1] = mt; }
    }
}

template <int M>
__global__ void k_xt_gather_fin(GenoView gv, const int64_t* __restrict__ cols, int64_t n_a,
                                const int64_t* __restrict__ cols_b, int64_t ncols, int nsplit,
                                const double* __restrict__ vbar, const double* __restrict__ part,
                                double* __restrict__ out) {
    int64_t e = blockIdx.x * (int64_t)blockDim.x + threadIdx.x;
    if (e >= ncols * M) return;
    int64_t c = e / M;
    int t = (int)(e % M);
    const int64_t jc = c < n_a ? cols[c] : cols_b[c - n_a];
    if (jc < 0) { out[c + (int64_t)t * ncols] = 0.0; return; }
    double at = 0.0, mt = 0.0;
    for (int sp = 0; sp < nsplit; ++sp) {
        const double* o = part + (c * nsplit + sp) * (2 * M);
        at = __dadd_rn(at, o[2 * t]);
        mt = __dadd_rn(mt, o[2 * t + 1]);
    }
    int64_t j = jc;
    double corr = gv.impute ? mt : __dmul_rn(-vbar[t], (double)gv.nmiss[j]);
    out[c + (int64_t)t * ncols] = __dmul_rn(gv.sinv[j], __dadd_rn(at, __dmul_rn(gv.mu[j], corr)));
}

constexpr int XN_CHUNK = 512;
__global__ void __launch_bounds__(256)
k_xt_gather_nib(GenoView gv, const int64_t* __restrict__ cols, int64_t n_a, const int64_t* __restrict__ cols_b,
                int64_t ncols, const double* __restrict__ v, const double* __restrict__ vbar,
                double* __restrict__ part ) {
    __shared__ double T[8][16][32];
    const int64_t n = gv.n;
    const int64_t chunk = blockIdx.x, nchunks = gridDim.x;
    const int warp = threadIdx.x >> 5, lane = threadIdx.x & 31;
    {
        const double vb = vbar[0];
        const int64_t i0 = chunk * XN_CHUNK + 16 * lane + 2 * warp;
        const double u0 = (i0 < n) ? __dsub_rn(v[i0], vb) : 0.0;
        const double u1 = (i0 + 1 < n) ? __dsub_rn(v[i0 + 1], vb) : 0.0;
        const double d0[4] = {0.0, 0.0, u0, __dadd_rn(u0, u0)};
        const double d1[4] = {0.0, 0.0, u1, __dadd_rn(u1, u1)};
#pragma unroll
        for (int nib = 0; nib < 16; ++nib) T[warp][nib][lane] = __dadd_rn(d0[nib & 3], d1[nib >> 2]);
    }
    __syncthreads();
    const int64_t w = chunk * (XN_CHUNK / 16) + lane;
    const bool in_col = w < ((gv.nbytes + 3) >> 2);
    for (int64_t c = (int64_t)blockIdx.y * 8 + warp; c < ncols; c += (int64_t)gridDim.y * 8) {
        const int64_t j = c < n_a ? cols[c] : cols_b[c - n_a];
        if (j < 0) continue;
        const uint32_t x = in_col ? *reinterpret_cast<const uint32_t*>(gv_ptr(gv, j, 4 * w)) : 0u;
        double a = 0.0;
#pragma unroll
        for (int k = 0; k < 8; ++k) a = __dadd_rn(a, T[k][(x >> (4 * k)) & 15u][lane]);
        a = warp_sum(a);
        if (lane == 0) part[c * nchunks + chunk] = a;
    }
}

__global__ void __launch_bounds__(128)
k_xt_gather_fin_nib(GenoView gv, const int64_t* __restrict__ miss_ptr, const int32_t* __restrict__ miss_idx,
                    const int64_t* __restrict__ cols, int64_t n_a, const int64_t* __restrict__ cols_b, int64_t ncols,
                    int nchunks, const double* __restrict__ v, const double* __restrict__ vbar,
                    const double* __restrict__ part, double* __restrict__ out) {
    const int64_t c = (blockIdx.x * (int64_t)blockDim.x + threadIdx.x) >> 5;
    const int lane = threadIdx.x & 31;
    if (c >= ncols) return;
    const int64_t jc = c < n_a ? cols[c] : cols_b[c - n_a];
    if (jc < 0) { if (lane == 0) out[c] = 0.0; return; }
    double at = 0.0, mt = 0.0;
    for (int sp = lane; sp < nchunks; sp += 32) at = __dadd_rn(at, part[c * nchunks + sp]);
    const double vb = vbar[0];
    if (gv.impute)
        for (int64_t e = miss_ptr[jc] + lane; e < miss_ptr[jc + 1]; e += 32) mt = __dadd_rn(mt, __dsub_rn(v[miss_idx[e]], vb));
    at = warp_sum(at); mt = warp_sum(mt);
    if (lane == 0) {
        const double corr = gv.impute ? mt : __dmul_rn(-vb, (double)gv.nmiss[jc]);
        out[c] = __dmul_rn(gv.sinv[jc], __dadd_rn(at, __dmul_rn(gv.mu[jc], corr)));
    }
}

static DBuf<double>& gather_scratch(cudaStream_t s) {
    static std::mutex mu;
    static std::unordered_map<cudaStream_t, std::unique_ptr<DBuf<double>>> pool;
    std::lock_guard<std::mutex> lk(mu);
    auto& slot = pool[s];
    if (!slot) slot.reset(new DBuf<double>());
    return *slot;
}

template <int M>
static void launch_xt_gather(const ihtb_geno* g, const int64_t* d_cols, int64_t n_a, const int64_t* d_cols_b,
                             int64_t ncols, const double* d_v, const double* d_vbar, double* d_out, cudaStream_t s,
                             bool blocked) {
    DBuf<double>& sc = gather_scratch(s);
    (void)blocked;
    if (M == 1) {
        const int nchunks = (int)ceil_div(g->n, XN_CHUNK);
        const size_t need_b = (size_t)ncols * nchunks;
        if (sc.n < need_b) {
            IHTB_CUDA(cudaStreamSynchronize(s));
            sc.alloc(need_b < 65536 ? 65536 : need_b);
        }
        int groups = (int)std::max<int64_t>(1, std::min<int64_t>(ceil_div(ncols, 8), (8 * g->sm_count) / nchunks + 1));
        IHTB_LAUNCH(k_xt_gather_nib, dim3((unsigned)nchunks, (unsigned)groups), 256, 0, s, geno_view(g), d_cols, n_a,
                    d_cols_b, ncols, d_v, d_vbar, sc.p);
        IHTB_LAUNCH(k_xt_gather_fin_nib, (unsigned)ceil_div(ncols * 32, 128), 128, 0, s, geno_view(g), g->miss_ptr.p,
                    g->miss_idx.p, d_cols, n_a, d_cols_b, ncols, nchunks, d_v, d_vbar, sc.p, d_out);
        return;
    }
    int64_t split_bytes = ceil_div(ceil_div(g->nbytes, XG_MAX_SPLIT), 256) * 256;
    if (split_bytes < 1024) split_bytes = 1024;
    int nsplit = (int)ceil_div(g->nbytes, split_bytes);
    size_t need = (size_t)ncols * nsplit * 2 * M;
    if (sc.n < need) {
        IHTB_CUDA(cudaStreamSynchronize(s));
        sc.alloc(need < 65536 ? 65536 : need);
    }
    dim3 grid((unsigned)ncols, (unsigned)nsplit);
    IHTB_LAUNCH((k_xt_gather<M>), grid, 256, 0, s, geno_view(g), d_cols, n_a, d_cols_b, split_bytes, d_v, d_vbar, sc.p);
    IHTB_LAUNCH((k_xt_gather_fin<M>), (unsigned)ceil_div(ncols * M, 128), 128, 0, s, geno_view(g), d_cols, n_a, d_cols_b,
                ncols, nsplit, d_vbar, sc.p, d_out);
}

void xt_gather2(const ihtb_geno* g, const int64_t* d_cols_a, int64_t n_a, const int64_t* d_cols_b, int64_t n_b,
                const double* d_v, int64_t m, const double* d_vbar, double* d_out, cudaStream_t s, bool blocked) {
    const int64_t ncols = n_a + n_b;
    if (ncols == 0) return;
    if (geno_is_dense(g)) { dense_xt_gather2(g, d_cols_a, n_a, d_cols_b, n_b, d_v, m, d_out, s); return; }
    for (int64_t t0 = 0; t0 < m;) {
        int64_t mm = m - t0;
        const double* vv = d_v + t0 * g->n;
        const double* vb = d_vbar + t0;
        double* o = d_out + t0 * ncols;
        if (mm >= 4) { launch_xt_gather<4>(g, d_cols_a, n_a, d_cols_b, ncols, vv, vb, o, s, blocked); t0 += 4; }
        else if (mm == 3) { launch_xt_gather<3>(g, d_cols_a, n_a, d_cols_b, ncols, vv, vb, o, s, blocked); t0 += 3; }
        else if (mm == 2) { launch_xt_gather<2>(g, d_cols_a, n_a, d_cols_b, ncols, vv, vb, o, s, blocked); t0 += 2; }
        else { launch_xt_gather<1>(g, d_cols_a, n_a, d_cols_b, ncols, vv, vb, o, s, blocked); t0 += 1; }
    }
}

void xt_gather(const ihtb_geno* g, const int64_t* d_cols, int64_t ncols, const double* d_v, int64_t m,
               const double* d_vbar, double* d_out, cudaStream_t s) {
    xt_gather2(g, d_cols, ncols, nullptr, 0, d_v, m, d_vbar, d_out, s, false);
}

}

using namespace ihtb;

__global__ void k_gb_fill(double* v, int64_t n) {
    int64_t i = blockIdx.x * (int64_t)blockDim.x + threadIdx.x;
    if (i < n) {
        uint64_t h = (uint64_t)i * 0x9E3779B97F4A7C15ull + 12345ull;
        h ^= h >> 31; h *= 0xBF58476D1CE4E5B9ull; h ^= h >> 29;
        v[i] = (double)(h >> 11) * (1.0 / 9007199254740992.0) - 0.4;
        v[i + n] = v[i];
    }
}
extern "C" int32_t ihtb_gather_bench(const ihtb_geno* g, int64_t ncols, int32_t reps, double* ms_per_call,
                                     double* max_rel_diff) {
    return guard([&] {
        IHTB_CHECK(g && ncols >= 1 && reps >= 1, IHTB_EINVAL, "bad argument");
        IHTB_CHECK(!geno_is_dense(g), IHTB_EUNSUPPORTED, "the gather bench times the PLINK re-scoring kernels");
        geno_require_ready(g);
        IHTB_CUDA(cudaSetDevice(g->device));
        cudaStream_t s;
        IHTB_CUDA(cudaStreamCreateWithFlags(&s, cudaStreamNonBlocking));
        std::vector<int64_t> hc((size_t)ncols);
        for (int64_t t = 0; t < ncols; ++t) hc[(size_t)t] = (t * 7919) % g->p;
        DBuf<int64_t> d_cols((size_t)ncols);
        DBuf<double> d_v((size_t)(2 * g->n)), d_mean(2), d_a((size_t)ncols), d_b((size_t)(2 * ncols));
        IHTB_CUDA(cudaMemcpyAsync(d_cols.p, hc.data(), (size_t)ncols * sizeof(int64_t), cudaMemcpyHostToDevice, s));
        IHTB_LAUNCH(k_gb_fill, (unsigned)ceil_div(g->n, 256), 256, 0, s, d_v.p, g->n);
        const double mean[2] = {0.1, 0.1};
        IHTB_CUDA(cudaMemcpyAsync(d_mean.p, mean, sizeof(mean), cudaMemcpyHostToDevice, s));
        xt_gather2(g, d_cols.p, ncols, nullptr, 0, d_v.p, 1, d_mean.p, d_a.p, s);
        cudaEvent_t e0, e1;
        IHTB_CUDA(cudaEventCreate(&e0)); IHTB_CUDA(cudaEventCreate(&e1));
        IHTB_CUDA(cudaEventRecord(e0, s));
        for (int i = 0; i < reps; ++i) xt_gather2(g, d_cols.p, ncols, nullptr, 0, d_v.p, 1, d_mean.p, d_a.p, s);
        IHTB_CUDA(cudaEventRecord(e1, s));
        xt_gather2(g, d_cols.p, ncols, nullptr, 0, d_v.p, 2, d_mean.p, d_b.p, s);
        std::vector<double> ha((size_t)ncols), hb((size_t)(2 * ncols));
        IHTB_CUDA(cudaMemcpyAsync(ha.data(), d_a.p, ha.size() * sizeof(double), cudaMemcpyDeviceToHost, s));
        IHTB_CUDA(cudaMemcpyAsync(hb.data(), d_b.p, hb.size() * sizeof(double), cudaMemcpyDeviceToHost, s));
        IHTB_CUDA(cudaStreamSynchronize(s));
        float ms = 0.f;
        IHTB_CUDA(cudaEventElapsedTime(&ms, e0, e1));
        if (ms_per_call) *ms_per_call = ms / reps;
        double worst = 0.0, scale = 0.0;
        for (int64_t t = 0; t < ncols; ++t) scale = std::max(scale, std::fabs(hb[(size_t)t]));
        for (int64_t t = 0; t < ncols; ++t) worst = std::max(worst, std::fabs(ha[(size_t)t] - hb[(size_t)t]));
        if (max_rel_diff) *max_rel_diff = scale > 0 ? worst / scale : worst;
        cudaEventDestroy(e0); cudaEventDestroy(e1);
        cudaStreamDestroy(s);
    });
}

extern "C" int32_t ihtb_x_support(const ihtb_geno* g, const int64_t* idx, int64_t k, const double* coef, int64_t m,
                                  double* out) {
    return guard([&] {
        IHTB_CHECK(g && out && m >= 1 && k >= 0, IHTB_EINVAL, "bad argument");
        geno_require_ready(g);
        IHTB_CHECK(k == 0 || (idx && coef), IHTB_EINVAL, "NULL idx/coef");
        IHTB_CUDA(cudaSetDevice(g->device));
        for (int64_t c = 0; c < k; ++c)
            IHTB_CHECK(idx[c] >= 0 && idx[c] < g->p, IHTB_EDIM, "support index out of range");
        DBuf<double> d_out((size_t)(g->n * m));
        if (k == 0) {
            d_out.zero(0);
        } else {
            DBuf<int64_t> d_idx((size_t)k);
            DBuf<double> d_coef((size_t)(k * m));
            IHTB_CUDA(cudaMemcpy(d_idx.p, idx, k * sizeof(int64_t), cudaMemcpyHostToDevice));
            IHTB_CUDA(cudaMemcpy(d_coef.p, coef, k * m * sizeof(double), cudaMemcpyHostToDevice));
            x_support(g, d_idx.p, k, d_coef.p, m, d_out.p, 0);
        }
        IHTB_CUDA(cudaMemcpy(out, d_out.p, g->n * m * sizeof(double), cudaMemcpyDeviceToHost));
    });
}
```

Baseline: 916.4.

## Trim host-device copies per iteration and remap x_support to one sample per thread

The support index list and covariate mask are packed into one host buffer and sent early in score_and_sweep, replacing separate per-iteration uploads. Scalar readbacks are merged into a single copy after the stepsize. The k_x_support kernel now gives each thread one sample instead of one packed byte, preloading the chunk's bytes into registers, which raises parallelism but issues four times as many byte loads. A copy counter and API hook are added, and some buffers are redirected through the glm context pointers.

```diff
diff --git a/include/ihtb200.h b/include/ihtb200.h
--- a/include/ihtb200.h
+++ b/include/ihtb200.h
@@ -66,6 +66,7 @@
 int32_t ihtb_device_count(int32_t* count);
 int32_t ihtb_set_device(int32_t device);
 int32_t ihtb_launch_count(int64_t* count);
+int32_t ihtb_copy_count(int64_t* count);
 
 int32_t ihtb_geno_create(const uint8_t* bed_cols, int64_t n, int64_t p, int64_t col_stride_bytes,
                          int32_t center, int32_t scale, int32_t impute, ihtb_geno** out);
diff --git a/mendeliht.jl_b200/__init__.py b/mendeliht.jl_b200/__init__.py
--- a/mendeliht.jl_b200/__init__.py
+++ b/mendeliht.jl_b200/__init__.py
@@ -1,10 +1,10 @@
 from . import _lib, synth
 from ._lib import (SWEEP_EXACT, SWEEP_FAST, SWEEP_PAIR, CudaError, DimensionMismatch, IHTBError, NumericError, device_count,
-                   launch_count, load)
+                   launch_count, copy_count, load)
 from .api import (BERNOULLI, NEGBIN, NORMAL, POISSON, B200DenseLinAlg, B200MultiSnpLinAlg, B200SnpLinAlg, IHTResult, IHTVariable, mIHTResult, mIHTVariable,
                   is_multivariate, allocate_fold_and_k,
                   canonicallink, cross_validate, cv_iht, cv_run, fit_iht, iht, maf_weights, meanloss, parse_covariates)
 
 __all__ = ["B200SnpLinAlg", "B200DenseLinAlg", "B200MultiSnpLinAlg", "IHTResult", "IHTVariable", "fit_iht", "cv_iht", "cv_run", "allocate_fold_and_k", "meanloss",
            "canonicallink", "maf_weights", "iht", "cross_validate", "parse_covariates", "NORMAL", "BERNOULLI", "POISSON", "NEGBIN", "SWEEP_FAST", "SWEEP_EXACT", "SWEEP_PAIR", "load",
-           "device_count", "launch_count", "IHTBError", "DimensionMismatch", "NumericError", "CudaError", "synth"]
+           "device_count", "launch_count", "copy_count", "IHTBError", "DimensionMismatch", "NumericError", "CudaError", "synth"]
diff --git a/mendeliht.jl_b200/_lib.py b/mendeliht.jl_b200/_lib.py
--- a/mendeliht.jl_b200/_lib.py
+++ b/mendeliht.jl_b200/_lib.py
@@ -65,6 +65,7 @@
     "ihtb_device_count": [C.POINTER(C.c_int32)],
     "ihtb_set_device": [C.c_int32],
     "ihtb_launch_count": [_i64],
+    "ihtb_copy_count": [_i64],
     "ihtb_geno_create": [_u8, C.c_int64, C.c_int64, C.c_int64, C.c_int32, C.c_int32, C.c_int32, _pp],
     "ihtb_geno_create_empty": [C.c_int64, C.c_int64, C.c_int32, C.c_int32, C.c_int32, _pp],
     "ihtb_geno_load_columns": [_p, _u8, C.c_int64, C.c_int64, C.c_int64],
@@ -196,3 +197,9 @@
     n = C.c_int64(0)
     check(load().ihtb_launch_count(C.byref(n)))
     return int(n.value)
+
+
+def copy_count() -> int:
+    n = C.c_int64(0)
+    check(load().ihtb_copy_count(C.byref(n)))
+    return int(n.value)
diff --git a/mendeliht.jl_b200/csrc/common.cuh b/mendeliht.jl_b200/csrc/common.cuh
--- a/mendeliht.jl_b200/csrc/common.cuh
+++ b/mendeliht.jl_b200/csrc/common.cuh
@@ -21,6 +21,7 @@
     operator int64_t() const { return __atomic_load_n(&v, __ATOMIC_RELAXED); }
 };
 LaunchCounter& launch_counter();
+LaunchCounter& copy_counter();
 bool debug_sync();
 
 #define IHTB_CUDA(call)                                                                      \
diff --git a/mendeliht.jl_b200/csrc/fit.cu b/mendeliht.jl_b200/csrc/fit.cu
--- a/mendeliht.jl_b200/csrc/fit.cu
+++ b/mendeliht.jl_b200/csrc/fit.cu
@@ -23,6 +23,11 @@
 }
 
 using namespace ihtb;
+
+static void copy_async(void* dst, const void* src, size_t bytes, cudaMemcpyKind kind, cudaStream_t s) {
+    IHTB_CUDA(cudaMemcpyAsync(dst, src, bytes, kind, s));
+    copy_counter()++;
+}
 
 static const double kFastBound = 1.0 / 262144.0;
 static const double kExactBound = 1e-13;
@@ -86,7 +91,7 @@
             IHTB_CHECK(w[j] > 0.0 && std::isfinite(w[j]), IHTB_EDOMAIN, "weights must be positive and finite");
         wt.assign(w, w + p_global);
         if (d_wt.n < (size_t)p) d_wt.alloc((size_t)p);
-        IHTB_CUDA(cudaMemcpyAsync(d_wt.p, wt.data() + j0, (size_t)p * sizeof(double), cudaMemcpyHostToDevice, s));
+        copy_async(d_wt.p, wt.data() + j0, (size_t)p * sizeof(double), cudaMemcpyHostToDevice, s);
         sync();
         tk.wt = d_wt.p;
     }
@@ -114,12 +119,12 @@
 
     void sync() { IHTB_CUDA(cudaStreamSynchronize(s)); }
     void readback_scal(int nv) {
-        IHTB_CUDA(cudaMemcpyAsync(h_scal.p, d_scal.p, nv * sizeof(double), cudaMemcpyDeviceToHost, s));
+        copy_async(h_scal.p, d_scal.p, nv * sizeof(double), cudaMemcpyDeviceToHost, s);
         sync();
     }
     template <typename T>
     void upload(T* dst, const T* src, size_t count) {
-        if (count) IHTB_CUDA(cudaMemcpyAsync(dst, src, count * sizeof(T), cudaMemcpyHostToDevice, s));
+        if (count) copy_async(dst, src, count * sizeof(T), cudaMemcpyHostToDevice, s);
     }
 
     bool is_local(int64_t j) const { return j >= j0 && j < j0 + p; }
@@ -164,7 +169,7 @@
         comm_allreduce_sum_f64(comm, d_out, cnt, s);
     }
 
-    void update_xb() { support_matvec(idx, b, d_xb.p); }
+    void update_xb() { support_matvec(idx, b, glm.xb); }
 
     double glm_update(int add_zc) {
         upload(d_small.p, c.data(), (size_t)q);
@@ -195,7 +200,7 @@
     }
     void fetch_mu() {
         h_mu.resize((size_t)n);
-        IHTB_CUDA(cudaMemcpyAsync(h_mu.data(), d_mu.p, n * sizeof(double), cudaMemcpyDeviceToHost, s));
+        copy_async(h_mu.data(), glm.mu, n * sizeof(double), cudaMemcpyDeviceToHost, s);
         sync();
     }
     double nb_logl(double r) {
@@ -270,15 +275,15 @@
         xt_gather2(g, d_cols.p, (int64_t)need.size(), nullptr, 0, d_r.p, 1, d_vbar.p, d_gout.p, s,
                    false);
         if (exchange) comm_allreduce_sum_f64(comm, d_gout.p, need.size(), s);
-        IHTB_CUDA(cudaMemcpyAsync(h_gout.p, d_gout.p, need.size() * sizeof(double), cudaMemcpyDeviceToHost, s));
+        copy_async(h_gout.p, d_gout.p, need.size() * sizeof(double), cudaMemcpyDeviceToHost, s);
         sync();
         for (size_t t = 0; t < need.size(); ++t) df_exact[need[t]] = h_gout.p[t];
         n_cand_iter += (int64_t)need.size();
     }
 
     void score_and_sweep() {
+        if (fz == nullptr && !(grouped() && !init_plain)) send_support();
         glm_score(glm, s, d_vbar.p);
-        IHTB_CUDA(cudaMemcpyAsync(h_scal.p, d_scal.p, (2 + q) * sizeof(double), cudaMemcpyDeviceToHost, s));
         IHTB_CUDA(cudaEventRecord(ev0, s));
         sweep_coef = geno_bound_coef(g, cfg.sweep_mode == IHTB_SWEEP_FAST ? kFastBound : kExactBound);
         const double t_sw = now();
@@ -286,7 +291,7 @@
             IHTB_CHECK(!grouped() && !comm, IHTB_EUNSUPPORTED, "paired sweeps serve plain single-device fits only");
             if (pairer->sweep(pair_slot, g, d_r.p, d_vbar.p, d_dfa.p, s, sweep_scratch)) {
                 sweep_coef = kPairBound;
-                IHTB_CUDA(cudaMemcpyAsync(h_scal.p + 3 + q, pairer->d_l2 + pair_slot, sizeof(double), cudaMemcpyDeviceToHost, s));
+                copy_async(h_scal.p + 3 + q, pairer->d_l2 + pair_slot, sizeof(double), cudaMemcpyDeviceToHost, s);
             }
         } else if (cfg.k > 0 && !(grouped() && !init_plain)) {
             const TopkFuse tf = topk_absdf_fuse_begin(tk, geno_bound_scale(g), d_scal.p, sweep_coef);
@@ -295,11 +300,28 @@
             sweep_xt_v_with_means(g, d_r.p, d_vbar.p, 1, d_dfa.p, cfg.sweep_mode, s, sweep_scratch, nullptr);
         }
         IHTB_CUDA(cudaEventRecord(ev1, s));
+        if (grouped() && !init_plain) copy_async(h_scal.p, d_scal.p, (2 + q) * sizeof(double), cudaMemcpyDeviceToHost, s);
         ++n_sweeps;
         const double t_sel = now();
         dbg[0] += t_sel - t_sw;
         select_rescore(false);
         dbg[1] += now() - t_sel;
+    }
+
+    HBuf<int64_t> h_sup;
+    DBuf<int64_t> d_sup;
+    const double* sup_mask = nullptr;
+    bool sup_sent = false;
+    void send_support() {
+        IHTB_CHECK(idx.size() + (size_t)q <= h_sup.n, IHTB_ENUMERIC, "support too large to re-score");
+        size_t u = 0;
+        for (int64_t j : idx)
+            if (is_local(j)) h_sup.p[u++] = j - j0;
+        double* mask = reinterpret_cast<double*>(h_sup.p + u);
+        for (int64_t l = 0; l < q; ++l) mask[l] = idc[l] ? 1.0 : 0.0;
+        copy_async(d_sup.p, h_sup.p, (u + (size_t)q) * sizeof(int64_t), cudaMemcpyHostToDevice, s);
+        sup_mask = reinterpret_cast<const double*>(d_sup.p + u);
+        sup_sent = true;
     }
 
     void select_rescore(bool rerun) {
@@ -319,7 +341,9 @@
             for (int64_t j : idx)
                 if (is_local(j)) supp_loc.push_back(j - j0);
         const int nsupp = (int)supp_loc.size();
-        const int64_t* d_supp = fused ? d_idx.p : d_cols.p;
+        if (!fused && !sup_sent) send_support();
+        sup_sent = false;
+        const int64_t* d_supp = fused ? plan_idx : d_sup.p;
         int glaunch = 0;
         if (cfg.k > 0) {
             const int64_t ksel = cfg.k + (int64_t)(fused ? fz->maxsupp : idx.size());
@@ -332,28 +356,24 @@
                                                           : ksel + 64;
             glaunch = (int)std::min<int64_t>(comm ? capx / 2 : cap, want);
         }
-        if (nsupp && !fused) upload(d_cols.p, supp_loc.data(), supp_loc.size());
         xt_gather2(g, tk.cand, glaunch, d_supp, nsupp, d_r.p, 1, d_vbar.p, d_gout.p, s);
         denom_ready = false;
         if (!rerun) {
             if (fused) {
-                glm_winner_coef(d_pick.p, d_coefM.p, nsupp, d_gout.p + glaunch, d_coef.p, d_cM.p, q, d_small.p + q, s);
+                glm_winner_coef(d_pick.p, plan_coef, nsupp, d_gout.p + glaunch, d_coef.p, plan_c, q, d_small.p + q, s);
                 support_matvec_dev(d_supp, nsupp, d_coef.p, d_xs.p);
-                IHTB_CUDA(cudaMemcpyAsync(h_pick.p, d_pick.p, (size_t)(1 + fz->M) * sizeof(double), cudaMemcpyDeviceToHost, s));
-                IHTB_CUDA(cudaMemcpyAsync(h_scalM.p, d_scalM.p, (size_t)(3 * fz->M) * sizeof(double), cudaMemcpyDeviceToHost, s));
+                copy_async(h_pick.p, d_pick.p, (size_t)(1 + fz->M) * sizeof(double), cudaMemcpyDeviceToHost, s);
+                copy_async(h_scalM.p, d_scalM.p, (size_t)(3 * fz->M) * sizeof(double), cudaMemcpyDeviceToHost, s);
             } else {
                 support_matvec_dev(d_supp, nsupp, d_gout.p + glaunch, d_xs.p);
-                std::vector<double> mask((size_t)q);
-                for (int64_t l = 0; l < q; ++l) mask[l] = idc[l] ? 1.0 : 0.0;
-                upload(d_small.p + q, mask.data(), (size_t)q);
-            }
-            glm_stepsize(glm, d_scal.p + 2, d_xs.p, s, d_small.p + q, d_scal.p + 2 + q);
-            IHTB_CUDA(cudaMemcpyAsync(h_scal.p + 2 + q, d_scal.p + 2 + q, sizeof(double), cudaMemcpyDeviceToHost, s));
+            }
+            glm_stepsize(glm, d_scal.p + 2, d_xs.p, s, fused ? d_small.p + q : sup_mask, d_scal.p + 2 + q);
+            copy_async(h_scal.p, d_scal.p, (3 + q) * sizeof(double), cudaMemcpyDeviceToHost, s);
             denom_ready = true;
         }
         if (!comm) {
-            IHTB_CUDA(cudaMemcpyAsync(h_sel.p, d_sel.p, (2 + glaunch) * sizeof(int64_t), cudaMemcpyDeviceToHost, s));
-            IHTB_CUDA(cudaMemcpyAsync(h_gout.p, d_gout.p, (glaunch + nsupp) * sizeof(double), cudaMemcpyDeviceToHost, s));
+            copy_async(h_sel.p, d_sel.p, (2 + glaunch) * sizeof(int64_t), cudaMemcpyDeviceToHost, s);
+            copy_async(h_gout.p, d_gout.p, (glaunch + nsupp) * sizeof(double), cudaMemcpyDeviceToHost, s);
             sync();
             const double t_host = now();
             struct Acc { double& a; double t0; ~Acc() { a += now() - t0; } } acc_host{dbg[2], t_host};
@@ -377,7 +397,7 @@
             for (int t = 0; t < std::min(count, glaunch); ++t) cvals.push_back({h_sel.p[2 + t], h_gout.p[t]});
             for (int t = 0; t < nsupp; ++t) df_exact[supp_loc[t] + j0] = h_gout.p[glaunch + t];
             if (count > glaunch) {
-                IHTB_CUDA(cudaMemcpyAsync(h_sel.p, d_sel.p, (2 + count) * sizeof(int64_t), cudaMemcpyDeviceToHost, s));
+                copy_async(h_sel.p, d_sel.p, (2 + count) * sizeof(int64_t), cudaMemcpyDeviceToHost, s);
                 sync();
                 std::vector<int64_t> rest(h_sel.p + 2 + glaunch, h_sel.p + 2 + count);
                 exact_df(rest);
@@ -390,7 +410,7 @@
             pack_sweep_candidates(d_pack.p, reinterpret_cast<const TopkState*>(d_sel.p), tk.cand, glaunch, d_gout.p,
                                   d_supp, nsupp, d_gout.p + glaunch, j0, capx, s);
             comm_allgather_i64(comm, d_pack.p, d_packall.p, blk, s);
-            IHTB_CUDA(cudaMemcpyAsync(h_packall.p, d_packall.p, nr * blk * sizeof(int64_t), cudaMemcpyDeviceToHost, s));
+            copy_async(h_packall.p, d_packall.p, nr * blk * sizeof(int64_t), cudaMemcpyDeviceToHost, s);
             sync();
             if (fused) adopt_winner();
             for (int r = 0; r < nr; ++r) {
@@ -583,7 +603,7 @@
         if (comm) {
             if (gc.d_Tall.n < nT * (size_t)nr) { gc.d_Tall.alloc(nT * (size_t)nr); gc.h_Tall.alloc(nT * (size_t)nr); }
             comm_allgather_i64(comm, reinterpret_cast<const int64_t*>(gc.d_gT.p), gc.d_Tall.p, nT, s);
-            IHTB_CUDA(cudaMemcpyAsync(gc.h_Tall.p, gc.d_Tall.p, nT * (size_t)nr * sizeof(int64_t), cudaMemcpyDeviceToHost, s));
+            copy_async(gc.h_Tall.p, gc.d_Tall.p, nT * (size_t)nr * sizeof(int64_t), cudaMemcpyDeviceToHost, s);
             sync();
             std::fill(TL.begin(), TL.end(), 0.0); std::fill(TU.begin(), TU.end(), 0.0);
             for (int rk = 0; rk < nr; ++rk) {
@@ -592,7 +612,7 @@
                 overflow = overflow || T[2 * G] != 0.0;
             }
         } else {
-            IHTB_CUDA(cudaMemcpyAsync(gc.h_gT.p, gc.d_gT.p, nT * sizeof(double), cudaMemcpyDeviceToHost, s));
+            copy_async(gc.h_gT.p, gc.d_gT.p, nT * sizeof(double), cudaMemcpyDeviceToHost, s);
             sync();
             for (size_t gi = 0; gi < G; ++gi) { TL[gi] = gc.h_gT.p[gi]; TU[gi] = gc.h_gT.p[G + gi]; }
             overflow = gc.h_gT.p[2 * G] != 0.0;
@@ -627,7 +647,7 @@
             gc.h_oidx.alloc((size_t)slots); gc.h_oval.alloc((size_t)slots);
         }
         if (nc) {
-            IHTB_CUDA(cudaMemcpyAsync(gc.d_chosen.p, chosen.data(), (size_t)nc * sizeof(int32_t), cudaMemcpyHostToDevice, s));
+            copy_async(gc.d_chosen.p, chosen.data(), (size_t)nc * sizeof(int32_t), cudaMemcpyHostToDevice, s);
             group_take(gc, nc, s);
         }
         std::vector<int64_t> supp_loc((size_t)nsupp);
@@ -645,7 +665,7 @@
             if (gc.d_blkall.n < blk * (size_t)nr) { gc.d_blkall.alloc(blk * (size_t)nr); gc.h_blkall.alloc(blk * (size_t)nr); }
             group_pack(gc.d_oidx.p, gc.d_oval.p, slots, j0, gc.d_blk.p, s);
             comm_allgather_i64(comm, gc.d_blk.p, gc.d_blkall.p, blk, s);
-            IHTB_CUDA(cudaMemcpyAsync(gc.h_blkall.p, gc.d_blkall.p, blk * (size_t)nr * sizeof(int64_t), cudaMemcpyDeviceToHost, s));
+            copy_async(gc.h_blkall.p, gc.d_blkall.p, blk * (size_t)nr * sizeof(int64_t), cudaMemcpyDeviceToHost, s);
             sync();
             for (int rk = 0; rk < nr; ++rk) {
                 const int64_t* b_ = gc.h_blkall.p + (size_t)rk * blk;
@@ -656,8 +676,8 @@
                 }
             }
         } else {
-            IHTB_CUDA(cudaMemcpyAsync(gc.h_oidx.p, gc.d_oidx.p, (size_t)slots * sizeof(int64_t), cudaMemcpyDeviceToHost, s));
-            IHTB_CUDA(cudaMemcpyAsync(gc.h_oval.p, gc.d_oval.p, (size_t)slots * sizeof(double), cudaMemcpyDeviceToHost, s));
+            copy_async(gc.h_oidx.p, gc.d_oidx.p, (size_t)slots * sizeof(int64_t), cudaMemcpyDeviceToHost, s);
+            copy_async(gc.h_oval.p, gc.d_oval.p, (size_t)slots * sizeof(double), cudaMemcpyDeviceToHost, s);
             sync();
             for (int64_t t = 0; t < slots; ++t) take(t, gc.h_oidx.p[t], gc.h_oval.p[t]);
         }
@@ -773,10 +793,10 @@
     }
 
     void compute_pve() {
-        glm_sum2(glm, d_mu.p, d_y.p, s);
+        glm_sum2(glm, glm.mu, d_y.p, s);
         readback_scal(2);
         double mm = h_scal.p[0] / (double)n, my = h_scal.p[1] / (double)n;
-        glm_ssq2(glm, d_mu.p, mm, d_y.p, my, s);
+        glm_ssq2(glm, glm.mu, mm, d_y.p, my, s);
         readback_scal(2);
         pve = h_scal.p[0] / h_scal.p[1];
     }
@@ -819,7 +839,7 @@
         std::vector<int64_t> cand;
         if (cfg.k > 0) {
             topk_candidates(tk, bd, nullptr, g->sinv.p, 1.0, 0.0, cfg.k, s);
-            IHTB_CUDA(cudaMemcpyAsync(h_sel.p, d_sel.p, (2 + cap) * sizeof(int64_t), cudaMemcpyDeviceToHost, s));
+            copy_async(h_sel.p, d_sel.p, (2 + cap) * sizeof(int64_t), cudaMemcpyDeviceToHost, s);
             sync();
             const TopkState* st = reinterpret_cast<const TopkState*>(h_sel.p);
             IHTB_CHECK(st->count <= cap, IHTB_ENUMERIC, "degenerate projection of the initial beta (too many ties)");
@@ -830,7 +850,7 @@
         if (!cand.empty()) {
             upload(d_cols.p, cand.data(), cand.size());
             take_values(bd, d_cols.p, (int64_t)cand.size(), d_gout.p, s);
-            IHTB_CUDA(cudaMemcpyAsync(vals.data(), d_gout.p, cand.size() * sizeof(double), cudaMemcpyDeviceToHost, s));
+            copy_async(vals.data(), d_gout.p, cand.size() * sizeof(double), cudaMemcpyDeviceToHost, s);
             sync();
         }
         if (comm) {
@@ -845,7 +865,7 @@
             upload(d_pack.p, mine.data(), blk);
             comm_allgather_i64(comm, d_pack.p, d_packall.p, blk, s);
             const int nr = nranks();
-            IHTB_CUDA(cudaMemcpyAsync(h_packall.p, d_packall.p, nr * blk * sizeof(int64_t), cudaMemcpyDeviceToHost, s));
+            copy_async(h_packall.p, d_packall.p, nr * blk * sizeof(int64_t), cudaMemcpyDeviceToHost, s);
             sync();
             cand.clear(); vals.clear();
             for (int rk = 0; rk < nr; ++rk) {
@@ -892,7 +912,7 @@
         idc.assign(zkeep.begin(), zkeep.end()); idc0 = idc;
         df_exact.clear(); dfs_idx.clear(); dfs_val.clear(); df_sparse = false;
         last_bt = kMaxBatch;
-        d_xb.zero(s);
+        IHTB_CUDA(cudaMemsetAsync(glm.xb, 0, (size_t)n * sizeof(double), s));
         const uint8_t* dm = nullptr;
         if (train_mask) {
             upload(d_mask.p, train_mask, (size_t)n);
@@ -974,7 +994,17 @@
     static constexpr int kMaxBatch = 4;
     static constexpr int64_t kAdaptiveBatchN = 131072;
     int last_bt = kMaxBatch;
-    DBuf<double> d_xbM, d_zcM, d_muM, d_partM, d_scalM, d_cM, d_coefM;
+    DBuf<double> d_xbM, d_zcM, d_muM, d_partM, d_scalM;
+    HBuf<int64_t> h_plan;
+    DBuf<int64_t> d_plan;
+    const int64_t* plan_idx = nullptr;
+    const double *plan_coef = nullptr, *plan_c = nullptr;
+    int area = 0;
+    void pick_area() {
+        const bool in0 = glm.xb >= d_xbM.p && glm.xb < d_xbM.p + (size_t)kMaxBatch * n;
+        area = in0 ? 1 : 0;
+    }
+    double* slot(const DBuf<double>& B, int m) const { return B.p + ((size_t)area * kMaxBatch + (size_t)m) * (size_t)n; }
     HBuf<double> h_scalM;
     bool batch_ok() const {
         static const bool off = [] { const char* e = getenv("IHTB_NO_BATCH"); return e && *e == '1'; }();
@@ -984,9 +1014,11 @@
     std::vector<StepModel> step_models;
     void ensure_batch_buffers() {
         if (d_xbM.n < (size_t)(kMaxBatch * n)) {
-            d_xbM.alloc((size_t)(kMaxBatch * n)); d_zcM.alloc((size_t)(kMaxBatch * n)); d_muM.alloc((size_t)(kMaxBatch * n));
+            d_xbM.alloc((size_t)(2 * kMaxBatch * n)); d_zcM.alloc((size_t)(2 * kMaxBatch * n));
+            d_muM.alloc((size_t)(2 * kMaxBatch * n));
             d_partM.alloc((size_t)kMaxBatch * GLM_MAX_BLOCKS * 3); d_scalM.alloc(kMaxBatch * 3); h_scalM.alloc(kMaxBatch * 3);
-            d_cM.alloc((size_t)(kMaxBatch * q)); d_coefM.alloc((size_t)kMaxBatch * (size_t)cap);
+            const size_t words = d_idx.n + (size_t)kMaxBatch * ((size_t)cap + (size_t)q);
+            h_plan.alloc(words); d_plan.alloc(words);
             d_pick.alloc(1 + kMaxBatch); h_pick.alloc(1 + kMaxBatch);
         }
     }
@@ -1011,7 +1043,7 @@
         std::sort(pl.uni.begin(), pl.uni.end());
         pl.uni.erase(std::unique(pl.uni.begin(), pl.uni.end()), pl.uni.end());
         const size_t U = pl.uni.size();
-        IHTB_CHECK(U * (size_t)M <= d_coefM.n && U <= d_idx.n, IHTB_ENUMERIC, "support union too large for the batched step");
+        IHTB_CHECK(U * (size_t)M <= (size_t)kMaxBatch * cap && U <= d_idx.n, IHTB_ENUMERIC, "support union too large for the batched step");
         std::vector<size_t> keep_pos;
         for (size_t t = 0; t < U; ++t)
             if (is_local(pl.uni[t])) { pl.loc.push_back(pl.uni[t] - j0); keep_pos.push_back(t); }
@@ -1028,11 +1060,14 @@
             }
             for (int64_t l = 0; l < q; ++l) cM[(size_t)(m * q + l)] = md.c[(size_t)l];
         }
-        if (pl.UL) {
-            upload(d_idx.p, pl.loc.data(), pl.UL);
-            upload(d_coefM.p, coefL.data(), coefL.size());
-        }
-        upload(d_cM.p, cM.data(), cM.size());
+        int64_t* h = h_plan.p;
+        memcpy(h, pl.loc.data(), pl.UL * sizeof(int64_t));
+        memcpy(h + pl.UL, coefL.data(), coefL.size() * sizeof(double));
+        memcpy(h + pl.UL + coefL.size(), cM.data(), cM.size() * sizeof(double));
+        copy_async(d_plan.p, h, (pl.UL + coefL.size() + cM.size()) * sizeof(int64_t), cudaMemcpyHostToDevice, s);
+        plan_idx = d_plan.p;
+        plan_coef = reinterpret_cast<const double*>(d_plan.p + pl.UL);
+        plan_c = reinterpret_cast<const double*>(d_plan.p + pl.UL + coefL.size());
         return pl;
     }
     void adopt_model(int m) {
@@ -1062,12 +1097,13 @@
     void finish_batched(const StepPlan& pl, double eta0, double t2, double old_logl, double& eta, int& eta_step,
                         double& new_logl) {
         const int Mtot = cfg.max_step + 1;
+        pick_area();
         auto eval = [&](const StepPlan& P) {
-            const size_t off = (size_t)P.m0 * (size_t)n;
-            support_matvec_dev_m(P.UL ? d_idx.p : nullptr, (int64_t)P.UL, d_coefM.p, P.M, d_xbM.p + off);
-            glm_mu_batched(glm, d_cM.p, P.M, d_xbM.p + off, d_zcM.p + off, d_muM.p + off, d_partM.p, d_scalM.p + 3 * P.m0, s);
-            IHTB_CUDA(cudaMemcpyAsync(h_scalM.p + 3 * P.m0, d_scalM.p + 3 * P.m0, (size_t)(3 * P.M) * sizeof(double),
-                                      cudaMemcpyDeviceToHost, s));
+            support_matvec_dev_m(P.UL ? plan_idx : nullptr, (int64_t)P.UL, plan_coef, P.M, slot(d_xbM, P.m0));
+            glm_mu_batched(glm, plan_c, P.M, slot(d_xbM, P.m0), slot(d_zcM, P.m0), slot(d_muM, P.m0), d_partM.p,
+                           d_scalM.p + 3 * P.m0, s);
+            copy_async(h_scalM.p + 3 * P.m0, d_scalM.p + 3 * P.m0, (size_t)(3 * P.M) * sizeof(double),
+                                      cudaMemcpyDeviceToHost, s);
             sync();
         };
         int have = pl.M;
@@ -1084,10 +1120,7 @@
         adopt_model(sidx);
         eta = step_models[(size_t)sidx].eta; eta_step = sidx;
         last_dev = h_scalM.p[3 * sidx];
-        const size_t nb = (size_t)n * sizeof(double);
-        IHTB_CUDA(cudaMemcpyAsync(d_xb.p, d_xbM.p + (size_t)sidx * n, nb, cudaMemcpyDeviceToDevice, s));
-        IHTB_CUDA(cudaMemcpyAsync(d_zc.p, d_zcM.p + (size_t)sidx * n, nb, cudaMemcpyDeviceToDevice, s));
-        IHTB_CUDA(cudaMemcpyAsync(d_mu.p, d_muM.p + (size_t)sidx * n, nb, cudaMemcpyDeviceToDevice, s));
+        glm.xb = slot(d_xbM, sidx); glm.zc = slot(d_zcM, sidx); glm.mu = slot(d_muM, sidx);
         double t3 = now(); phase[2] += t3 - t2;
         score_and_sweep();
         phase[3] += now() - t3;
@@ -1115,9 +1148,10 @@
             finish_batched(pl, eta0, t2, old_logl, eta, eta_step, new_logl);
             return;
         }
-        support_matvec_dev_m(pl.UL ? d_idx.p : nullptr, (int64_t)pl.UL, d_coefM.p, M, d_xbM.p);
-        glm_mu_batched(glm, d_cM.p, M, d_xbM.p, d_zcM.p, d_muM.p, d_partM.p, d_scalM.p, s);
-        glm_pick_model(glm, d_scalM.p, M, old_logl, cfg.max_step, d_pick.p, d_xbM.p, d_zcM.p, d_muM.p, s);
+        pick_area();
+        support_matvec_dev_m(pl.UL ? plan_idx : nullptr, (int64_t)pl.UL, plan_coef, M, slot(d_xbM, 0));
+        glm_mu_batched(glm, plan_c, M, slot(d_xbM, 0), slot(d_zcM, 0), slot(d_muM, 0), d_partM.p, d_scalM.p, s);
+        glm_pick_model(glm, d_scalM.p, M, old_logl, cfg.max_step, d_pick.p, slot(d_xbM, 0), slot(d_zcM, 0), slot(d_muM, 0), s);
         FusedStep ctx;
         ctx.uni_loc = pl.loc; ctx.M = M;
         for (const StepModel& md : step_models) ctx.maxsupp = std::max(ctx.maxsupp, md.idx.size());
@@ -1269,6 +1303,7 @@
     size_t cols_cap = 2 * (size_t)cap + 64;
     f->d_coef.alloc(cols_cap); f->d_gout.alloc(cols_cap); f->d_vbar.alloc(1);
     f->d_idx.alloc(cols_cap); f->d_cols.alloc(cols_cap);
+    f->h_sup.alloc(cols_cap + (size_t)q); f->d_sup.alloc(cols_cap + (size_t)q);
     f->d_keyL.alloc(p); f->d_keyU.alloc(p); f->d_hist.alloc(2 * 3 * 2048); f->d_sel.alloc(2 + cap);
     f->h_scal.alloc(2 + q + 8); f->h_gout.alloc(cols_cap); f->h_sel.alloc(2 + cap);
     f->sweep_scratch = sweep_scratch_create();
@@ -1330,11 +1365,11 @@
                 f->h_packall.alloc((size_t)nr * blk);
             }
             int64_t mine = g->j0;
-            IHTB_CUDA(cudaMemcpyAsync(f->d_sel.p, &mine, sizeof(int64_t), cudaMemcpyHostToDevice, f->s));
+            copy_async(f->d_sel.p, &mine, sizeof(int64_t), cudaMemcpyHostToDevice, f->s);
             comm_allgather_i64(comm, f->d_sel.p, f->d_selall.p, 1, f->s);
             f->shard_j0.resize(nr);
-            IHTB_CUDA(cudaMemcpyAsync(f->shard_j0.data(), f->d_selall.p, nr * sizeof(int64_t), cudaMemcpyDeviceToHost,
-                                      f->s));
+            copy_async(f->shard_j0.data(), f->d_selall.p, nr * sizeof(int64_t), cudaMemcpyDeviceToHost,
+                                      f->s);
             IHTB_CUDA(cudaStreamSynchronize(f->s));
 
         }
@@ -1350,8 +1385,8 @@
                    "Only negative binomial regression currently supports nuisance parameter estimation");
         IHTB_CHECK(cfg->est_r >= 0 && cfg->est_r <= 2, IHTB_EINVAL, "Only support method is Newton or MM");
         if (cfg->est_r != 0) f->h_y.assign(y, y + n); else f->h_y.clear();
-        IHTB_CUDA(cudaMemcpyAsync(f->d_y.p, y, n * sizeof(double), cudaMemcpyHostToDevice, f->s));
-        IHTB_CUDA(cudaMemcpyAsync(f->d_z.p, z, n * q * sizeof(double), cudaMemcpyHostToDevice, f->s));
+        copy_async(f->d_y.p, y, n * sizeof(double), cudaMemcpyHostToDevice, f->s);
+        copy_async(f->d_z.p, z, n * q * sizeof(double), cudaMemcpyHostToDevice, f->s);
         f->d_xb.zero(f->s); f->d_zc.zero(f->s);
         f->glm = GlmCtx{n, q, f->d_z.p, f->d_y.p, f->d_w.p, f->d_xb.p, f->d_zc.p, f->d_mu.p, f->d_r.p, f->d_part.p,
                         f->d_scal.p, cfg->dist, cfg->link, cfg->nb_r};
@@ -1429,8 +1464,8 @@
             for (size_t t = 0; t < f->best_idx.size(); ++t) beta[f->best_idx[t]] = f->best_b[t];
         }
         if (c) std::copy(f->best_c.begin(), f->best_c.end(), c);
-        if (mu) IHTB_CUDA(cudaMemcpy(mu, f->d_mu.p, f->n * sizeof(double), cudaMemcpyDeviceToHost));
-        if (xb) IHTB_CUDA(cudaMemcpy(xb, f->d_xb.p, f->n * sizeof(double), cudaMemcpyDeviceToHost));
+        if (mu) IHTB_CUDA(cudaMemcpy(mu, f->glm.mu, f->n * sizeof(double), cudaMemcpyDeviceToHost));
+        if (xb) IHTB_CUDA(cudaMemcpy(xb, f->glm.xb, f->n * sizeof(double), cudaMemcpyDeviceToHost));
     });
 }
 
diff --git a/mendeliht.jl_b200/csrc/geno.cu b/mendeliht.jl_b200/csrc/geno.cu
--- a/mendeliht.jl_b200/csrc/geno.cu
+++ b/mendeliht.jl_b200/csrc/geno.cu
@@ -13,6 +13,10 @@
 void set_last_error(const std::string& m) { t_last_error = m; }
 const std::string& last_error() { return t_last_error; }
 LaunchCounter& launch_counter() {
+    static LaunchCounter c;
+    return c;
+}
+LaunchCounter& copy_counter() {
     static LaunchCounter c;
     return c;
 }
@@ -330,6 +334,13 @@
     });
 }
 
+int32_t ihtb_copy_count(int64_t* count) {
+    return guard([&] {
+        IHTB_CHECK(count, IHTB_EINVAL, "count is NULL");
+        *count = copy_counter();
+    });
+}
+
 static void upload_columns(ihtb_geno* g, const uint8_t* bed_cols, int64_t col_stride_bytes, int64_t j_dst, int64_t ncols) {
     const int64_t pitch = ceil_div(g->nbytes, 16) * 16;
     int64_t cols_per = (int64_t(64) << 20) / pitch;
diff --git a/mendeliht.jl_b200/csrc/support.cu b/mendeliht.jl_b200/csrc/support.cu
--- a/mendeliht.jl_b200/csrc/support.cu
+++ b/mendeliht.jl_b200/csrc/support.cu
@@ -8,23 +8,24 @@
 namespace ihtb {
 
 constexpr int XS_CHUNK = 32;
+constexpr int XS_THREADS = 256;
 
 template <int M, bool PUSH>
-__global__ void __launch_bounds__(256)
+__global__ void __launch_bounds__(XS_THREADS)
 k_x_support(GenoView gv, const int64_t* __restrict__ idx, int64_t k, const double* __restrict__ coef,
             double* __restrict__ out, P2PView pv, unsigned long long seq) {
-    const int64_t nbytes = gv.nbytes, n = gv.n;
+    const int64_t n = gv.n;
     const double* __restrict__ mu = gv.mu;
     const double* __restrict__ sinv = gv.sinv;
     const int impute = gv.impute;
     __shared__ double tab[XS_CHUNK][4][M];
     __shared__ int64_t cols[XS_CHUNK];
-    int64_t b = blockIdx.x * (int64_t)blockDim.x + threadIdx.x;
-    double acc[4][M];
-#pragma unroll
-    for (int s = 0; s < 4; ++s)
-#pragma unroll
-        for (int t = 0; t < M; ++t) acc[s][t] = 0.0;
+    const int64_t i = blockIdx.x * (int64_t)blockDim.x + threadIdx.x;
+    const int64_t b = i >> 2;
+    const int shift = 2 * (int)(i & 3);
+    double acc[M];
+#pragma unroll
+    for (int t = 0; t < M; ++t) acc[t] = 0.0;
 
     for (int64_t c0 = 0; c0 < k; c0 += XS_CHUNK) {
         int nc = (int)((k - c0 < XS_CHUNK) ? (k - c0) : XS_CHUNK);
@@ -39,59 +40,42 @@
             if (code == 0 && t == 0) cols[c] = j;
         }
         __syncthreads();
-        if (b < nbytes) {
-            for (int c = 0; c < nc; ++c) {
-                uint32_t byte = *gv_ptr(gv, cols[c], b);
-#pragma unroll
-                for (int s = 0; s < 4; ++s) {
-                    uint32_t code = (byte >> (2 * s)) & 3u;
-#pragma unroll
-                    for (int t = 0; t < M; ++t) acc[s][t] = __dadd_rn(acc[s][t], tab[c][code][t]);
+        if (i < n) {
+            uint32_t byte[XS_CHUNK];
+#pragma unroll
+            for (int c = 0; c < XS_CHUNK; ++c)
+                if (c < nc) byte[c] = *gv_ptr(gv, cols[c], b);
+#pragma unroll
+            for (int c = 0; c < XS_CHUNK; ++c)
+                if (c < nc) {
+                    const uint32_t code = (byte[c] >> shift) & 3u;
+#pragma unroll
+                    for (int t = 0; t < M; ++t) acc[t] = __dadd_rn(acc[t], tab[c][code][t]);
                 }
-            }
         }
     }
     if (PUSH) {
-        __shared__ double stage[PUSH ? 1024 : 1];
-        __syncthreads();
-#pragma unroll
-        for (int s = 0; s < 4; ++s) stage[4 * threadIdx.x + s] = acc[s][0];
-        __syncthreads();
-        const int64_t base = 1024 * (int64_t)blockIdx.x;
-        for (int e = 2 * threadIdx.x; e < 1024; e += 512) {
-            const int64_t i = base + e;
-            if (i + 1 < n) {
-                const double2 x = make_double2(stage[e], stage[e + 1]);
-                for (int r = 0; r < pv.nranks; ++r) *reinterpret_cast<double2*>(pv.push_slot[r] + i) = x;
-            } else if (i < n) {
-                for (int r = 0; r < pv.nranks; ++r) pv.push_slot[r][i] = stage[e];
-            }
-        }
+        if (i < n)
+            for (int r = 0; r < pv.nranks; ++r) pv.push_slot[r][i] = acc[0];
         p2p_publish(pv, seq);
         return;
     }
-    if (b < nbytes) {
-#pragma unroll
-        for (int s = 0; s < 4; ++s) {
-            int64_t i = 4 * b + s;
-            if (i < n)
-#pragma unroll
-                for (int t = 0; t < M; ++t) out[i + (int64_t)t * n] = acc[s][t];
-        }
-    }
+    if (i < n)
+#pragma unroll
+        for (int t = 0; t < M; ++t) out[i + (int64_t)t * n] = acc[t];
 }
 
 template <int M>
 static void launch_x_support(const ihtb_geno* g, const int64_t* d_idx, int64_t k, const double* d_coef, double* d_out,
                              cudaStream_t s) {
-    IHTB_LAUNCH((k_x_support<M, false>), (unsigned)ceil_div(g->nbytes, 256), 256, 0, s, geno_view(g), d_idx, k, d_coef,
-                d_out, P2PView{}, 0ull);
+    IHTB_LAUNCH((k_x_support<M, false>), (unsigned)ceil_div(g->n, XS_THREADS), XS_THREADS, 0, s, geno_view(g), d_idx, k,
+                d_coef, d_out, P2PView{}, 0ull);
 }
 
 void x_support_push(const ihtb_geno* g, const int64_t* d_idx, int64_t k, const double* d_coef, ihtb_comm* c,
                     cudaStream_t s) {
-    IHTB_LAUNCH((k_x_support<1, true>), (unsigned)ceil_div(g->nbytes, 256), 256, 0, s, geno_view(g), d_idx, k, d_coef,
-                (double*)nullptr, p2p_view(c), (unsigned long long)(c->seq[0] + 1));
+    IHTB_LAUNCH((k_x_support<1, true>), (unsigned)ceil_div(g->n, XS_THREADS), XS_THREADS, 0, s, geno_view(g), d_idx, k,
+                d_coef, (double*)nullptr, p2p_view(c), (unsigned long long)(c->seq[0] + 1));
 }
 
 void x_support(const ihtb_geno* g, const int64_t* d_idx, int64_t k, const double* d_coef, int64_t m, double* d_out,
```

Result: faster. 928.1, median of 6 (+1.3%).
